# BartvLaatum/GreenLight-Gym2

Hardware: AMD Instinct MI355X
Metric: TomatoEnv env-steps/sec (higher is better)
Workload: dtype f32

## Files before the change

### greenlight-gym2_amd/csrc/glgym.hip

```cpp
#include <hip/hip_runtime.h>

#include <cmath>
#include <cstdio>
#include <cstdlib>
#include <cstring>
#include <new>
#include <string>
#include <vector>

#include "glgym.h"
#include "gl_model.hpp"
#include "gl_model_quad.hpp"
#include "gl_reward.hpp"
#include "glgym_bdf.h"
#include "glgym_rng.h"
#include "glgym_plan.h"

using namespace glm;

namespace {

thread_local std::string g_err;

#define HIPCHK(expr)                                                                                   \
    do {                                                                                               \
        hipError_t e_ = (expr);                                                                        \
        if (e_ != hipSuccess) {                                                                        \
            g_err = std::string(#expr) + ": " + hipGetErrorString(e_);                                 \
            return GLGYM_EHIP;                                                                         \
        }                                                                                              \
    } while (0)

constexpr int WAVE = 64;

#include "gl_default_const.inc"
static_assert(sizeof(ModelConst<float>) == sizeof(kDefaultConstF32_image), "regenerate gl_default_const.inc");
static_assert(sizeof(ModelConst<double>) == sizeof(kDefaultConstF64_image), "regenerate gl_default_const.inc");
template <class T> struct DefaultConst;
template <> struct DefaultConst<float> {
    static constexpr ModelConst<float> value = __builtin_bit_cast(ModelConst<float>, kDefaultConstF32_bits);
};
template <> struct DefaultConst<double> {
    static constexpr ModelConst<double> value = __builtin_bit_cast(ModelConst<double>, kDefaultConstF64_bits);
};
__constant__ const ModelConst<float> g_default_f32 = __builtin_bit_cast(ModelConst<float>, kDefaultConstF32_bits);
__constant__ const ModelConst<double> g_default_f64 = __builtin_bit_cast(ModelConst<double>, kDefaultConstF64_bits);
template <class T> __device__ __forceinline__ const ModelConst<T>& device_default();
template <> __device__ __forceinline__ const ModelConst<float>& device_default<float>() { return g_default_f32; }
template <> __device__ __forceinline__ const ModelConst<double>& device_default<double>() { return g_default_f64; }

template <class T> struct RewardConst : RewardConstBase<T> {};

template <class T> struct StepArgsT {
    int B, ld;
    T* x; T* u;
    const float* action; const T* control;
    const T* weather; int weather_rows;
    const int* w_off; int* timestep;
    const T* crop_p;
    int N;
    T* reward; T* info; unsigned char* done; float* metrics; int* step_flags;
    T dt; int n_sub;
    T gasR, tCanMin;
    int nd;
    float du, u_min[NU], u_max[NU];
    int verify;
    int pipe;
    int window;
};

template <class T> __device__ __forceinline__ T wave_sum(T v)
{
#pragma unroll
    for (int o = 32; o > 0; o >>= 1) v += __shfl_xor(v, o, WAVE);
    return v;
}

constexpr int OBS_NCORE = 23;
__device__ __forceinline__ float obs_core_feature(int j, float prim, float aux, float sday, int ts, double doy_inc, double hod_inc)
{
#pragma clang fp contract(off)
    const float kPpm = (float)(8.3144598 / (101325.0 * 44.01e-3));
    const int k = ts > 0 ? ts - 1 : 0;
    const float sat = 610.78f * __builtin_amdgcn_exp2f(1.44269504f * 17.2694f * aux * __builtin_amdgcn_rcpf(aux + 238.3f));
    const float rh = fminf(fmaxf(100.0f * prim * __builtin_amdgcn_rcpf(sat), 0.0f), 100.0f);
    const float ppm = kPpm * (aux + 273.15f) * prim;
    const int c = j - 18;
    const double rev = (c <= 2) ? __builtin_fma((double)ts, doy_inc, (double)sday) * (1.0 / 365.0)
                                : (double)ts * hod_inc * (1.0 / 24.0);
    const float fr = (float)(rev - floor(rev));
    const float clk = (c == 1 || c == 3) ? __builtin_amdgcn_sinf(fr) : __builtin_amdgcn_cosf(fr);
    float v = prim;
    v = (j == 0 || j == 16) ? ppm : v;
    v = (j == 2 || j == 15) ? rh : v;
    v = (j == 18) ? (float)k : v;
    v = (j > 18) ? clk : v;
    return v;
}
__device__ __forceinline__ constexpr int obs_core_module(int j) { return j < 4 ? 0 : j < 7 ? 1 : j < 13 ? 2 : j < 18 ? 3 : 4; }
__device__ __forceinline__ constexpr int obs_core_col(int j) { return j < 4 ? j : j < 7 ? j - 4 : j < 13 ? j - 7 : j < 18 ? j - 13 : j - 18; }

#ifndef GL_OBS_ROWS
#define GL_OBS_ROWS 16
#endif
constexpr int OBS_ROWS = GL_OBS_ROWS, OBS_MAX_NP = 128;
struct StepObsArgs {
    float* obs; const float* start_day;
    double doy_inc, hod_inc;
    int Np, dim, moff[6];
};
constexpr int STEP_OBS_MAX_DIM_OCC2 = WAVE * ((2 * NX + GL_N_SLOW) | 1) / OBS_ROWS, STEP_OBS_MAX_DIM_OCC1 = 512;
struct StepNoObs {};
constexpr int GL_SCH_OBS = 8;
template <bool OBS> struct StepObsSel { using type = StepNoObs; };
template <> struct StepObsSel<true> { using type = StepObsArgs; };

#ifndef GL_STEP_WAVES_PER_SIMD
#define GL_STEP_WAVES_PER_SIMD 1
#endif
#ifndef GL_RK4_WIN_F32
#define GL_RK4_WIN_F32 4
#endif
#ifndef GL_RK4_WIN_F64
#define GL_RK4_WIN_F64 4
#endif
template <class T> struct RK4_WINDOW { static constexpr int value = sizeof(T) == 4 ? GL_RK4_WIN_F32 : GL_RK4_WIN_F64; };
constexpr int gl_order(int sch) { return sch == 0 ? 4 : sch == 1 ? 2 : sch == 2 ? 3 : 5; }
template <class T, int SCH> struct SchemeWin { static constexpr int value = SCH == 0 ? RK4_WINDOW<T>::value : SCH == 1 ? 4 : SCH == 2 ? 3 : 2; };

template <class T, bool PER_ENV_CROP, bool DEFAULT_P, bool PIPE = false, int SCHX = 0, int OCC = GL_STEP_WAVES_PER_SIMD>
__global__ __launch_bounds__(WAVE, OCC) void step_kernel(StepArgsT<T> a, ModelConst<T> m_arg, RewardConst<T> rw,
                                                         typename StepObsSel<(SCHX & GL_SCH_OBS) != 0>::type o)
{
    constexpr bool OBS = (SCHX & GL_SCH_OBS) != 0;
    constexpr int SCH = SCHX & (GL_SCH_OBS - 1);
    static_assert(!OBS || (sizeof(T) == 4 && !PIPE), "observation epilogue: fp32, default ODE");
    const ModelConst<T>& m = DEFAULT_P ? device_default<T>() : m_arg;
    constexpr bool WBUF = OCC == 2;
    constexpr int WSTRIDE = (2 * NX + GL_N_SLOW) | 1;
    alignas(16) __shared__ float sh_w[WBUF ? WAVE * WSTRIDE : WAVE * NU];
    float* sh_act = sh_w;
    const int lane = threadIdx.x;
    const int b0 = blockIdx.x * WAVE;
    const int b = b0 + lane;
    const bool live = b < a.B;
    const int bb = live ? b : a.B - 1;

    T u[NU];
    if (a.action) {
        const int n_tile = min(WAVE, a.B - b0) * NU;
        for (int i = lane; i < n_tile; i += WAVE) sh_act[i] = a.action[(size_t)b0 * NU + i];
        __syncthreads();
        const int l = live ? lane : (a.B - 1 - b0);
#pragma unroll
        for (int j = 0; j < NU; ++j) {
            const float inc = sh_act[l * NU + j] * a.du;
            const T v = a.u[(size_t)j * a.ld + bb] + T(inc);
            u[j] = Math<T>::min(Math<T>::max(v, T(a.u_min[j])), T(a.u_max[j]));
        }
    } else {
#pragma unroll
        for (int j = 0; j < NU; ++j) u[j] = a.control[(size_t)j * a.ld + bb];
    }

    T x0[NX];
#pragma unroll
    for (int i = 0; i < NX; ++i) x0[i] = a.x[(size_t)i * a.ld + bb];
    const int ts = a.timestep[bb];
    int row = a.w_off[bb] + ts;
    row = row < 0 ? 0 : (row >= a.weather_rows ? a.weather_rows - 1 : row);
    T d[7];
#pragma unroll
    for (int j = 0; j < 7; ++j) d[j] = a.weather[(size_t)row * a.nd + j];

    CropConst<T> crLocal;
    if (PER_ENV_CROP) {
        T pc[NCROP];
#pragma unroll
        for (int i = 0; i < NCROP; ++i) pc[i] = a.crop_p[(size_t)i * a.ld + bb];
        make_crop_const<T, T>(pc, a.gasR, a.tCanMin, crLocal);
    }
    const CropConst<T>& cr = PER_ENV_CROP ? crLocal : m.crop;
    StepCoef<T> s_reg;
    precompute(u, d, m, cr, s_reg);
    if (PIPE) {
        const T tPipe = a.weather[(size_t)row * a.nd + 10], swOff = a.weather[(size_t)row * a.nd + 12];
        s_reg.pipeTrack = ((tPipe < T(1)) || (swOff > T(0))) ? T(0) : T(1);
        s_reg.tPipeSet = tPipe;
    }
    const StepCoef<T>& s = s_reg;
    if (live) {
#pragma unroll
        for (int j = 0; j < NU; ++j) a.u[(size_t)j * a.ld + b] = u[j];
    }
    T del_reg[WBUF ? 1 : NX];
    T* wb = reinterpret_cast<T*>(sh_w) + (size_t)lane * WSTRIDE;
    T* del = WBUF ? wb + NX + GL_N_SLOW : del_reg;
    if (WBUF) {
        __syncthreads();
#pragma unroll
        for (int i = 0; i < NX; ++i) wb[i] = x0[i];
        wb[5] = x0[3] - x0[5]; wb[7] = x0[2] - x0[7]; wb[20] = x0[2] - x0[20]; wb[6] = x0[5] - x0[6];
    }
    bool bad;
    int extra_steps, first_flags = 0;
    const int retries = rk4_delta_guarded<T, PIPE, gl_order(SCH), SchemeWin<T, SCH>::value, WBUF>(x0, s, m, cr, a.dt, a.n_sub, del, &bad, &extra_steps, a.verify != 0, &first_flags, a.window, wb);
    const T uBoil = a.u[(size_t)0 * a.ld + bb], uCo2 = a.u[(size_t)1 * a.ld + bb], uLamp = a.u[(size_t)4 * a.ld + bb];
    if (WBUF) {
#pragma unroll
        for (int i = 0; i < NX; ++i) x0[i] = a.x[(size_t)i * a.ld + bb];
    }

    T x1[NX];
#pragma unroll
    for (int i = 0; i < NX; ++i) x1[i] = bad ? x0[i] : x0[i] + del[i];
    {
        const double per_step = (double)a.dt / 86400.0;
        double t_start = (double)x0[NX - 1] - (double)ts * per_step;
        if (fabs(t_start) < 5e-4) t_start = 0.0;
        if (!bad) x1[NX - 1] = T(t_start + ((double)ts + 1.0) * per_step);
    }

    const T co2ppm = rw.kPpm * (x1[2] + T(273.15)) * x1[0];
    const T rh = Math<T>::min(Math<T>::max(T(100) * x1[15] / sat_vp_exact(x1[2]), T(0)), T(100));
    const T o3[3] = {co2ppm, x1[2], rh};
    T viol[3], pen = T(0);
#pragma unroll
    for (int i = 0; i < 3; ++i) {
        viol[i] = Math<T>::max(rw.lo[i] - o3[i], T(0)) + Math<T>::max(o3[i] - rw.hi[i], T(0));
        pen += viol[i] * rw.invMaxViol[i];
    }
    const T heat = uBoil * rw.heatK, elec = uLamp * rw.elecK, co2c = uCo2 * rw.co2K;
    const T varc = heat + co2c + elec;
    const T gains = (bad ? T(0) : del[25]) * rw.gainK;
    const T profit = gains - varc;
    const T reward = (profit - rw.minProfit) * rw.invRange - pen;
    const bool term = bad || (ts >= a.N);

    if (live) {
#pragma unroll
        for (int i = 0; i < NX; ++i) a.x[(size_t)i * a.ld + b] = x1[i];
        a.timestep[b] = ts + 1;
        a.reward[b] = reward;
        a.done[b] = term ? 1 : 0;
        if (a.step_flags) a.step_flags[b] = first_flags | (retries << 8) | (bad ? GLGYM_SF_FAILED : 0) | (min(extra_steps, 32767) << 16);
        if (a.info) {
            const T inf[GLGYM_NINFO] = {profit, gains, varc, rw.fixedCosts, co2c, heat, elec, viol[1], viol[0], viol[2], T(0)};
#pragma unroll
            for (int i = 0; i < GLGYM_NINFO; ++i) a.info[(size_t)i * a.ld + b] = inf[i];
        }
    }
    if (a.metrics) {
        const float w = live ? 1.f : 0.f;
        float mv[GLGYM_NMETRIC] = {w * (float)reward, w * (float)profit, (live && term) ? 1.f : 0.f,
                                   (live && bad) ? 1.f : 0.f, w * (float)viol[0], w * (float)viol[1],
                                   w * (float)viol[2], w, w * (float)retries, w * (float)extra_steps,
                                   (live && (first_flags & SC_FLAG_ERR)) ? 1.f : 0.f, (live && (first_flags & SC_FLAG_BRANCH)) ? 1.f : 0.f,
                                   (live && (first_flags & (SC_FLAG_CAP | SC_FLAG_NONFINITE))) ? 1.f : 0.f,
                                   (live && (first_flags & 16)) ? 1.f : 0.f};
        float* mrep = a.metrics + (size_t)(blockIdx.x % GLGYM_METRIC_REPLICAS) * GLGYM_METRIC_STRIDE;
#pragma unroll
        for (int i = 0; i < GLGYM_NMETRIC; ++i) {
            const float sum = wave_sum(mv[i]);
            if (lane == 0) atomicAdd(mrep + i, sum);
        }
    }
    if constexpr (OBS) {
        typedef float v4f __attribute__((ext_vector_type(4)));
        float* span;
        if constexpr (WBUF) {
            span = sh_w;
        } else {
            __shared__ float4 sh_obs4[OBS_ROWS * STEP_OBS_MAX_DIM_OCC1 / 4];
            span = reinterpret_cast<float*>(sh_obs4);
        }
        const int dim = o.dim;
        const int ts1 = ts + 1;
        const int base = a.w_off[bb] + (ts1 > 0 ? ts1 - 1 : 0);
        const int basec = base >= a.weather_rows ? a.weather_rows - 1 : (base < 0 ? 0 : base);
        const T* wrow = a.weather + (size_t)basec * a.nd;
        float wv[5];
#pragma unroll
        for (int j = 0; j < 5; ++j) wv[j] = wrow[j];
        const float sday = o.start_day[bb];
        const float uo[NU] = {uBoil, uCo2, a.u[(size_t)2 * a.ld + bb], a.u[(size_t)3 * a.ld + bb], uLamp, a.u[(size_t)5 * a.ld + bb]};
        float f[OBS_NCORE];
#pragma unroll
        for (int j = 0; j < OBS_NCORE; ++j) {
            const int xi = j == 0 ? 0 : j == 1 ? 2 : j == 2 ? 15 : j == 3 ? 9 : j == 4 ? 21 : j == 5 ? 25 : 26;
            const float prim = j < 7 ? x1[xi] : (j < 13 ? uo[(j >= 7 && j < 13) ? j - 7 : 0] : wv[j < 18 ? j - 13 : 0]);
            const float aux = j < 13 ? x1[2] : wv[1];
            f[j] = obs_core_feature(j, prim, aux, sday, ts1, o.doy_inc, o.hod_inc);
        }
        const int n_live = min(WAVE, a.B - b0);
        const int nf = o.moff[5] >= 0 ? 5 * o.Np : 0;
        __syncthreads();
        for (int s0 = 0; s0 < n_live; s0 += OBS_ROWS) {
            const int nrows = min(OBS_ROWS, n_live - s0);
            const int r_me = lane - s0;
            if (r_me >= 0 && r_me < nrows) {
#pragma unroll
                for (int j = 0; j < OBS_NCORE; ++j) {
                    const int mo = o.moff[obs_core_module(j)];
                    if (mo >= 0) span[r_me * dim + mo + obs_core_col(j)] = f[j];
                }
            }
            int base_r[OBS_ROWS];
#pragma unroll
            for (int r = 0; r < OBS_ROWS; ++r) base_r[r] = __builtin_amdgcn_readlane(base, s0 + r);
            for (int q = lane; q < nf; q += WAVE) {
                const int i = q / 5, c = q - i * 5;
                float v[OBS_ROWS];
#pragma unroll
                for (int r = 0; r < OBS_ROWS; ++r) {
                    int row = base_r[r] + 1 + i;
                    row = row >= a.weather_rows ? a.weather_rows - 1 : (row < 0 ? 0 : row);
                    v[r] = (float)a.weather[(size_t)row * a.nd + c];
                }
#pragma unroll
                for (int r = 0; r < OBS_ROWS; ++r)
                    if (r < nrows) span[r * dim + o.moff[5] + q] = v[r];
            }
            __syncthreads();
            float* out = o.obs + (size_t)(b0 + s0) * dim;
            if (nrows == OBS_ROWS) {
                const int n4 = (OBS_ROWS * dim) >> 2;
                const v4f* src4 = reinterpret_cast<const v4f*>(span);
                v4f* dst4 = reinterpret_cast<v4f*>(out);
                for (int e = lane; e < n4; e += WAVE) __builtin_nontemporal_store(src4[e], &dst4[e]);
            } else {
                for (int r = 0; r < nrows; ++r)
                    for (int jj = lane; jj < dim; jj += WAVE) out[(size_t)r * dim + jj] = span[(size_t)r * dim + jj];
            }
            __syncthreads();
        }
    }
}


template <class T, bool DEFAULT_P, int SCH = 0, bool PIPE = false, bool CROP = false, bool PAIR = false>
__global__ __launch_bounds__(WAVE) void step_kernel_quad(StepArgsT<T> a, ModelConst<T> m_arg, RewardConst<T> rw)
{
    static_assert(!(PAIR && CROP), "the two-rungs ladder is instantiated for shared crop constants only");
    constexpr bool LDSM = sizeof(T) == 8 && !DEFAULT_P;
    __shared__ ModelConst<T> sh_m[1];
    if (LDSM) {
        static_assert(sizeof(ModelConst<T>) % 4 == 0, "word copy");
        const unsigned* src = reinterpret_cast<const unsigned*>(&m_arg);
        unsigned* dst = reinterpret_cast<unsigned*>(&sh_m[0]);
        for (int i = threadIdx.x; i < (int)(sizeof(ModelConst<T>) / 4); i += WAVE) dst[i] = src[i];
        __syncthreads();
    }
    const ModelConst<T>& m = LDSM ? sh_m[0] : DEFAULT_P ? device_default<T>() : m_arg;
    const int gl = blockIdx.x * WAVE + threadIdx.x, role = gl & 3;
    const int b = PAIR ? gl >> 3 : gl >> 2, half = PAIR ? (gl >> 2) & 1 : 0;
    const bool live = b < a.B;
    const int bb = live ? b : a.B - 1;
    T u[NU];
    if (a.action) {
#pragma unroll
        for (int j = 0; j < NU; ++j) {
            const float inc = a.action[(size_t)bb * NU + j] * a.du;
            const T v = a.u[(size_t)j * a.ld + bb] + T(inc);
            u[j] = Math<T>::min(Math<T>::max(v, T(a.u_min[j])), T(a.u_max[j]));
        }
    } else {
#pragma unroll
        for (int j = 0; j < NU; ++j) u[j] = a.control[(size_t)j * a.ld + bb];
    }
    const int ts = a.timestep[bb];
    int row = a.w_off[bb] + ts;
    row = row < 0 ? 0 : (row >= a.weather_rows ? a.weather_rows - 1 : row);
    T d[7];
#pragma unroll
    for (int j = 0; j < 7; ++j) d[j] = a.weather[(size_t)row * a.nd + j];
    constexpr bool LDSQ = sizeof(T) == 8;
    struct SRec { StepCoef<T> s; T pad[(sizeof(StepCoef<T>) / sizeof(T)) % 2 == 0 ? 1 : 2]; };
    struct KRec { LaneK<T> k; T pad[(sizeof(LaneK<T>) / sizeof(T)) % 2 == 0 ? 1 : 2]; };
    struct CRec { CropConst<T> c; T pad[(sizeof(CropConst<T>) / sizeof(T)) % 2 == 0 ? 1 : 2]; };
    __shared__ SRec sh_s[LDSQ ? WAVE / 4 : 1];
    __shared__ KRec sh_k[LDSQ ? WAVE : 1];
    __shared__ CRec sh_c[(LDSQ && CROP) ? WAVE / 4 : 1];
    StepCoef<T> s_reg;
    LaneK<T> k_reg;
    CropConst<T> cr_reg;
    if (CROP && (!LDSQ || role == 0)) {
        T pc[NCROP];
#pragma unroll
        for (int i = 0; i < NCROP; ++i) pc[i] = a.crop_p[(size_t)i * a.ld + bb];
        make_crop_const<T, T>(pc, a.gasR, a.tCanMin, cr_reg);
    }
    if (!LDSQ || role == 0) {
        precompute(u, d, m, CROP ? cr_reg : m.crop, s_reg);
        if (PIPE && a.pipe) {
            const T tPipe = a.weather[(size_t)row * a.nd + 10], swOff = a.weather[(size_t)row * a.nd + 12];
            s_reg.pipeTrack = ((tPipe < T(1)) || (swOff > T(0))) ? T(0) : T(1);
            s_reg.tPipeSet = tPipe;
            s_reg.pipeOde = T(1);
        }
    }
    if (LDSQ) {
        if (role == 0) { sh_s[threadIdx.x >> 2].s = s_reg; if (CROP) sh_c[threadIdx.x >> 2].c = cr_reg; }
        __syncthreads();
    }
    const CropConst<T>& cr = !CROP ? m.crop : LDSQ ? sh_c[threadIdx.x >> 2].c : cr_reg;
    const StepCoef<T>& s = LDSQ ? sh_s[threadIdx.x >> 2].s : s_reg;
    LaneK<T>& K = LDSQ ? sh_k[threadIdx.x].k : k_reg;
    auto X = [&](int i) { return a.x[(size_t)i * a.ld + bb]; };
    QVec<T> x0, z0, del;
#pragma unroll
    for (int i = 0; i < 6; ++i) x0.sh[i] = X(role == 0 ? gq_sh_ix(i) : role == 1 ? gq_sh_ix(i) : role == 2 ? gq_sh_ix(i) : gq_sh_ix(i));
    x0.p = gq_mk<T>(X(role == 0 ? 4 : role == 1 ? 8 : role == 2 ? 7 : 5), X(role == 0 ? 9 : role == 1 ? 17 : role == 2 ? 20 : 6));
#pragma unroll
    for (int j = 0; j < 4; ++j) {
        const int ix = role == 0 ? gq_other_ix(0, j) : role == 1 ? gq_other_ix(1, j) : role == 2 ? gq_other_ix(2, j) : gq_other_ix(3, j < 2 ? j : 1);
        x0.o[j] = X(ix);
    }
    z0 = x0;
    z0.p = gq_mk<T>(role == 2 ? x0.sh[2] - x0.p.x : role == 3 ? x0.sh[3] - x0.p.x : x0.p.x,
                    role == 2 ? x0.sh[2] - x0.p.y : role == 3 ? x0.p.x - x0.p.y : x0.p.y);
    if (live && role == 0 && half == 0) {
#pragma unroll
        for (int j = 0; j < NU; ++j) a.u[(size_t)j * a.ld + b] = u[j];
    }
    bool bad;
    int extra_steps = 0, first_flags = 0, retries = 0, mine = 1;
    constexpr bool HVU = sizeof(T) == 8 || DEFAULT_P;
    if (PAIR) {
        int bad_i;
        rk4_delta_guarded_quad_pair<T, gl_order(SCH), SchemeWin<T, SCH>::value, LDSQ, PIPE, false, true, HVU>(role, half, z0, s, K, m, cr, a.dt, a.n_sub, del, &bad_i, &mine,
                                                                                                         a.window, &retries, &extra_steps, &first_flags);
        asm volatile("" : "+v"(bad_i), "+v"(mine));
        bad = bad_i != 0;
    } else {
        retries = rk4_delta_guarded_quad<T, gl_order(SCH), SchemeWin<T, SCH>::value, LDSQ, PIPE, LDSQ && CROP, HVU>(role, z0, s, K, m, cr, a.dt, a.n_sub, del, &bad,
                                                                                                    &extra_steps, a.verify != 0, &first_flags, a.window);
    }
    P2<T> dP;
    gq_phys_pair<T>(role, del, dP);
    asm volatile("" ::: "memory");
    int gl2 = blockIdx.x * WAVE + threadIdx.x;
    asm volatile("" : "+v"(gl2));
    const int role2 = gl2 & 3, b2 = PAIR ? gl2 >> 3 : gl2 >> 2;
    const bool live2 = b2 < a.B && mine != 0;
    const int bb2 = (b2 < a.B) ? b2 : a.B - 1;
    const int ts2 = a.timestep[bb2];
    auto X2 = [&](int i) { return a.x[(size_t)i * a.ld + bb2]; };
#pragma unroll
    for (int i = 0; i < 6; ++i) x0.sh[i] = X2(gq_sh_ix(i));
    x0.p = gq_mk<T>(X2(role2 == 0 ? 4 : role2 == 1 ? 8 : role2 == 2 ? 7 : 5), X2(role2 == 0 ? 9 : role2 == 1 ? 17 : role2 == 2 ? 20 : 6));
#pragma unroll
    for (int j = 0; j < 4; ++j) {
        const int ix = role2 == 0 ? gq_other_ix(0, j) : role2 == 1 ? gq_other_ix(1, j) : role2 == 2 ? gq_other_ix(2, j) : gq_other_ix(3, j < 2 ? j : 1);
        x0.o[j] = X2(ix);
    }
#pragma unroll
    for (int j = 0; j < NU; ++j) u[j] = a.u[(size_t)j * a.ld + bb2];
    QVec<T> x1;
    x1.p = gq_mk<T>(bad ? x0.p.x : x0.p.x + dP.x, bad ? x0.p.y : x0.p.y + dP.y);
#pragma unroll
    for (int i = 0; i < 6; ++i) x1.sh[i] = bad ? x0.sh[i] : x0.sh[i] + del.sh[i];
#pragma unroll
    for (int j = 0; j < 4; ++j) x1.o[j] = bad ? x0.o[j] : x0.o[j] + del.o[j];
    if (role2 == 3) {
        const double per_step = (double)a.dt / 86400.0;
        double t_start = (double)x0.o[1] - (double)ts2 * per_step;
        if (fabs(t_start) < 5e-4) t_start = 0.0;
        if (!bad) x1.o[1] = T(t_start + ((double)ts2 + 1.0) * per_step);
    }
    const T dFruit = gq_bcast<2>(del.o[3]);
    const T co2ppm = rw.kPpm * (x1.sh[2] + T(273.15)) * x1.sh[0];
    const T rh = Math<T>::min(Math<T>::max(T(100) * x1.sh[4] / sat_vp_exact(x1.sh[2]), T(0)), T(100));
    const T o3[3] = {co2ppm, x1.sh[2], rh};
    T viol[3], pen = T(0);
#pragma unroll
    for (int i = 0; i < 3; ++i) {
        viol[i] = Math<T>::max(rw.lo[i] - o3[i], T(0)) + Math<T>::max(o3[i] - rw.hi[i], T(0));
        pen += viol[i] * rw.invMaxViol[i];
    }
    const T heat = u[0] * rw.heatK, elec = u[4] * rw.elecK, co2c = u[1] * rw.co2K;
    const T varc = heat + co2c + elec;
    const T gains = (bad ? T(0) : dFruit) * rw.gainK;
    const T profit = gains - varc;
    const T reward = (profit - rw.minProfit) * rw.invRange - pen;
    const bool term = bad || (ts2 >= a.N);
    if (live2) {
        auto W = [&](int i, T v) { a.x[(size_t)i * a.ld + b2] = v; };
        W(role2 == 0 ? 4 : role2 == 1 ? 8 : role2 == 2 ? 7 : 5, x1.p.x);
        W(role2 == 0 ? 9 : role2 == 1 ? 17 : role2 == 2 ? 20 : 6, x1.p.y);
#pragma unroll
        for (int j = 0; j < 4; ++j)
            if (role2 != 3 || j < 2) W(role2 == 0 ? gq_other_ix(0, j) : role2 == 1 ? gq_other_ix(1, j) : role2 == 2 ? gq_other_ix(2, j) : gq_other_ix(3, j < 2 ? j : 1), x1.o[j]);
        if (role2 == 0) {
#pragma unroll
            for (int i = 0; i < 6; ++i) W(gq_sh_ix(i), x1.sh[i]);
            a.timestep[b2] = ts2 + 1;
            a.reward[b2] = reward;
            a.done[b2] = term ? 1 : 0;
            if (a.step_flags) a.step_flags[b2] = first_flags | (retries << 8) | (bad ? GLGYM_SF_FAILED : 0) | (min(extra_steps, 32767) << 16);
            if (a.info) {
                const T inf[GLGYM_NINFO] = {profit, gains, varc, rw.fixedCosts, co2c, heat, elec, viol[1], viol[0], viol[2], T(0)};
#pragma unroll
                for (int i = 0; i < GLGYM_NINFO; ++i) a.info[(size_t)i * a.ld + b2] = inf[i];
            }
        }
    }
    if (a.metrics) {
        const bool cnt = live2 && role2 == 0;
        const float w = cnt ? 1.f : 0.f;
        float mv[GLGYM_NMETRIC] = {w * (float)reward, w * (float)profit, (cnt && term) ? 1.f : 0.f,
                                   (cnt && bad) ? 1.f : 0.f, w * (float)viol[0], w * (float)viol[1],
                                   w * (float)viol[2], w, w * (float)retries, w * (float)extra_steps,
                                   (cnt && (first_flags & SC_FLAG_ERR)) ? 1.f : 0.f, (cnt && (first_flags & SC_FLAG_BRANCH)) ? 1.f : 0.f,
                                   (cnt && (first_flags & (SC_FLAG_CAP | SC_FLAG_NONFINITE))) ? 1.f : 0.f,
                                   (cnt && (first_flags & 16)) ? 1.f : 0.f};
        float* mrep = a.metrics + (size_t)(blockIdx.x % GLGYM_METRIC_REPLICAS) * GLGYM_METRIC_STRIDE;
#pragma unroll
        for (int i = 0; i < GLGYM_NMETRIC; ++i) {
            const float sum = wave_sum(mv[i]);
            if (threadIdx.x == 0) atomicAdd(mrep + i, sum);
        }
    }
}

template <class T, int SCH, bool PIPE, bool CROP, bool PAIR = false>
__global__ __launch_bounds__(WAVE) void evalf_kernel_quad(const double* x, const double* u, const double* d, const double* crop, int B, T dt,
                                                          int n_sub, T gasR, T tCanMin, ModelConst<T> m_arg, double* x_next, int nd,
                                                          int* n_failed, int verify, int pipe, int window)
{
    constexpr bool LDSM = sizeof(T) == 8;
    __shared__ ModelConst<T> sh_m[1];
    if (LDSM) {
        const unsigned* src = reinterpret_cast<const unsigned*>(&m_arg);
        unsigned* dst = reinterpret_cast<unsigned*>(&sh_m[0]);
        for (int i = threadIdx.x; i < (int)(sizeof(ModelConst<T>) / 4); i += WAVE) dst[i] = src[i];
        __syncthreads();
    }
    const ModelConst<T>& m = LDSM ? sh_m[0] : m_arg;
    const int gl = blockIdx.x * WAVE + threadIdx.x, role = gl & 3, b = PAIR ? gl >> 3 : gl >> 2, half = PAIR ? (gl >> 2) & 1 : 0;
    const bool live = b < B;
    const int bb = live ? b : B - 1;
    T uu[NU], dd[7];
#pragma unroll
    for (int i = 0; i < NU; ++i) uu[i] = T(u[(size_t)bb * NU + i]);
#pragma unroll
    for (int i = 0; i < 7; ++i) dd[i] = T(d[(size_t)bb * nd + i]);
    constexpr bool LDSQ = sizeof(T) == 8;
    struct SRec { StepCoef<T> s; T pad[(sizeof(StepCoef<T>) / sizeof(T)) % 2 == 0 ? 1 : 2]; };
    struct KRec { LaneK<T> k; T pad[(sizeof(LaneK<T>) / sizeof(T)) % 2 == 0 ? 1 : 2]; };
    struct CRec { CropConst<T> c; T pad[(sizeof(CropConst<T>) / sizeof(T)) % 2 == 0 ? 1 : 2]; };
    __shared__ SRec sh_s[LDSQ ? WAVE / 4 : 1];
    __shared__ KRec sh_k[LDSQ ? WAVE : 1];
    __shared__ CRec sh_c[(LDSQ && CROP) ? WAVE / 4 : 1];
    StepCoef<T> s_reg;
    LaneK<T> k_reg;
    CropConst<T> cr_reg;
    if (CROP && (!LDSQ || role == 0)) {
        T pc[NCROP];
#pragma unroll
        for (int i = 0; i < NCROP; ++i) pc[i] = T(crop[(size_t)bb * NCROP + i]);
        make_crop_const<T, T>(pc, gasR, tCanMin, cr_reg);
    }
    if (!LDSQ || role == 0) {
        precompute(uu, dd, m, CROP ? cr_reg : m.crop, s_reg);
        if (PIPE && pipe) {
            const T tPipe = T(d[(size_t)bb * nd + 10]), swOff = T(d[(size_t)bb * nd + 12]);
            s_reg.pipeTrack = ((tPipe < T(1)) || (swOff > T(0))) ? T(0) : T(1);
            s_reg.tPipeSet = tPipe;
            s_reg.pipeOde = T(1);
        }
    }
    if (LDSQ) {
        if (role == 0) { sh_s[threadIdx.x >> 2].s = s_reg; if (CROP) sh_c[threadIdx.x >> 2].c = cr_reg; }
        __syncthreads();
    }
    const CropConst<T>& cr = !CROP ? m.crop : LDSQ ? sh_c[threadIdx.x >> 2].c : cr_reg;
    const StepCoef<T>& s = LDSQ ? sh_s[threadIdx.x >> 2].s : s_reg;
    LaneK<T>& K = LDSQ ? sh_k[threadIdx.x].k : k_reg;
    auto X = [&](int i) { return T(x[(size_t)bb * NX + i]); };
    QVec<T> x0, z0, del;
#pragma unroll
    for (int i = 0; i < 6; ++i) x0.sh[i] = X(gq_sh_ix(i));
    x0.p = gq_mk<T>(X(role == 0 ? 4 : role == 1 ? 8 : role == 2 ? 7 : 5), X(role == 0 ? 9 : role == 1 ? 17 : role == 2 ? 20 : 6));
#pragma unroll
    for (int j = 0; j < 4; ++j)
        x0.o[j] = X(role == 0 ? gq_other_ix(0, j) : role == 1 ? gq_other_ix(1, j) : role == 2 ? gq_other_ix(2, j) : gq_other_ix(3, j < 2 ? j : 1));
    z0 = x0;
    z0.p = gq_mk<T>(role == 2 ? x0.sh[2] - x0.p.x : role == 3 ? x0.sh[3] - x0.p.x : x0.p.x,
                    role == 2 ? x0.sh[2] - x0.p.y : role == 3 ? x0.p.x - x0.p.y : x0.p.y);
    bool bad;
    constexpr bool HVU = sizeof(T) == 8;
    int mine = 1;
    if (PAIR) {
        int bad_i;
        rk4_delta_guarded_quad_pair<T, gl_order(SCH), SchemeWin<T, SCH>::value, LDSQ, PIPE, LDSQ && CROP, false, HVU>(role, half, z0, s, K, m, cr, dt, n_sub, del, &bad_i, &mine, window);
        asm volatile("" : "+v"(bad_i), "+v"(mine));
        bad = bad_i != 0;
    } else {
        int extra_steps, first_flags = 0;
        rk4_delta_guarded_quad<T, gl_order(SCH), SchemeWin<T, SCH>::value, LDSQ, PIPE, LDSQ && CROP, HVU>(role, z0, s, K, m, cr, dt, n_sub, del, &bad, &extra_steps, verify != 0,
                                                                                      &first_flags, window);
    }
    P2<T> dP;
    gq_phys_pair<T>(role, del, dP);
    asm volatile("" ::: "memory");
    int gl2 = blockIdx.x * WAVE + threadIdx.x;
    asm volatile("" : "+v"(gl2));
    const int role2 = gl2 & 3, b2 = PAIR ? gl2 >> 3 : gl2 >> 2;
    if (b2 < B && mine != 0) {
        const double nan = __builtin_nan("");
        auto X2 = [&](int i) { return x[(size_t)b2 * NX + i]; };
        auto W = [&](int i, T dv) { x_next[(size_t)b2 * NX + i] = bad ? nan : X2(i) + (double)dv; };
        W(role2 == 0 ? 4 : role2 == 1 ? 8 : role2 == 2 ? 7 : 5, dP.x);
        W(role2 == 0 ? 9 : role2 == 1 ? 17 : role2 == 2 ? 20 : 6, dP.y);
#pragma unroll
        for (int j = 0; j < 4; ++j)
            if (role2 != 3 || j < 2)
                W(role2 == 0 ? gq_other_ix(0, j) : role2 == 1 ? gq_other_ix(1, j) : role2 == 2 ? gq_other_ix(2, j) : gq_other_ix(3, j < 2 ? j : 1), del.o[j]);
        if (role2 == 0) {
#pragma unroll
            for (int i = 0; i < 6; ++i) W(gq_sh_ix(i), del.sh[i]);
            if (bad) atomicAdd(n_failed, 1);
        }
    }
}

template <class T, bool PER_ENV_CROP, bool PIPE>
__global__ __launch_bounds__(WAVE) void rhs_kernel(const double* x, const double* u, const double* d, const double* crop, int B, T gasR,
                                                   T tCanMin, ModelConst<T> m, double* dx, int nd)
{
    const int b = blockIdx.x * WAVE + threadIdx.x;
    if (b >= B) return;
    T x0[NX], uu[NU], dd[7];
    for (int i = 0; i < NX; ++i) x0[i] = T(x[(size_t)b * NX + i]);
    for (int i = 0; i < NU; ++i) uu[i] = T(u[(size_t)b * NU + i]);
    for (int i = 0; i < 7; ++i) dd[i] = T(d[(size_t)b * nd + i]);
    CropConst<T> crLocal;
    if (PER_ENV_CROP) {
        T pc[NCROP];
        for (int i = 0; i < NCROP; ++i) pc[i] = T(crop[(size_t)b * NCROP + i]);
        make_crop_const<T, T>(pc, gasR, tCanMin, crLocal);
    }
    const CropConst<T>& cr = PER_ENV_CROP ? crLocal : m.crop;
    StepCoef<T> s;
    precompute(uu, dd, m, cr, s);
    if (PIPE) {
        const T tPipe = T(d[(size_t)b * nd + 10]), swOff = T(d[(size_t)b * nd + 12]);
        s.pipeTrack = ((tPipe < T(1)) || (swOff > T(0))) ? T(0) : T(1);
        s.tPipeSet = tPipe;
    }
    T k[NX];
    rhs<T, true, PIPE>(x0, s, m, cr, k);
    for (int i = 0; i < NX; ++i) dx[(size_t)b * NX + i] = (double)k[i];
}

template <class T, bool PER_ENV_CROP, bool PIPE = false, int SCH = 0>
__global__ __launch_bounds__(WAVE) void evalf_kernel(const double* x, const double* u, const double* d,
                                                     const double* crop, int B, T dt, int n_sub, T gasR, T tCanMin,
                                                     ModelConst<T> m, double* x_next, int rhs_only, int nd,
                                                     int* n_failed, int verify, int window)
{
    const int b = blockIdx.x * WAVE + threadIdx.x;
    if (b >= B) return;
    T x0[NX], uu[NU], dd[7];
    for (int i = 0; i < NX; ++i) x0[i] = T(x[(size_t)b * NX + i]);
    for (int i = 0; i < NU; ++i) uu[i] = T(u[(size_t)b * NU + i]);
    for (int i = 0; i < 7; ++i) dd[i] = T(d[(size_t)b * nd + i]);
    CropConst<T> crLocal;
    if (PER_ENV_CROP) {
        T pc[NCROP];
        for (int i = 0; i < NCROP; ++i) pc[i] = T(crop[(size_t)b * NCROP + i]);
        make_crop_const<T, T>(pc, gasR, tCanMin, crLocal);
    }
    const CropConst<T>& cr = PER_ENV_CROP ? crLocal : m.crop;
    StepCoef<T> s;
    precompute(uu, dd, m, cr, s);
    if (PIPE) {
        const T tPipe = T(d[(size_t)b * nd + 10]), swOff = T(d[(size_t)b * nd + 12]);
        s.pipeTrack = ((tPipe < T(1)) || (swOff > T(0))) ? T(0) : T(1);
        s.tPipeSet = tPipe;
    }
    if (rhs_only) {
        T k[NX];
        rhs<T, true, PIPE>(x0, s, m, cr, k);
        for (int i = 0; i < NX; ++i) x_next[(size_t)b * NX + i] = (double)k[i];
        return;
    }
    T del[NX];
    bool failed;
    rk4_delta_guarded<T, PIPE, gl_order(SCH), SchemeWin<T, SCH>::value>(x0, s, m, cr, dt, n_sub, del, &failed, nullptr, verify != 0, nullptr, window);
    for (int i = 0; i < NX; ++i)
        x_next[(size_t)b * NX + i] = failed ? __builtin_nan("") : (double)x0[i] + (double)del[i];
    if (failed) atomicAdd(n_failed, 1);
}

template <class T> struct ObsArgsT {
    int B, ld;
    const T* x; const T* u; const T* weather; int weather_rows;
    const int* w_off; const int* timestep; const float* start_day;
    int Np; float* obs; double doy_inc, hod_inc;
    const unsigned char* mask; float* term_obs;
    int nd;
    int moff[6], dim;
};

template <class T> __global__ __launch_bounds__(256) void obs_kernel(ObsArgsT<T> a)
{
    constexpr int ROWS = OBS_ROWS, NCORE = OBS_NCORE;
    extern __shared__ float4 span4[];
    float* span = reinterpret_cast<float*>(span4);
    const int tid = threadIdx.x;
    const int dim = a.dim;
    for (int rb = blockIdx.x * ROWS; rb < a.B; rb += gridDim.x * ROWS) {
        const int nrows = min(ROWS, a.B - rb);
        if (a.mask) {
            int any = 0;
            for (int r = 0; r < nrows; ++r) any |= a.mask[rb + r];
            if (!any) continue;
        }
        int base_r[ROWS];
#pragma unroll
        for (int r = 0; r < ROWS; ++r) {
            const int b = rb + (r < nrows ? r : 0);
            const int ts = a.timestep[b];
            base_r[r] = a.w_off[b] + (ts > 0 ? ts - 1 : 0);
        }
        for (int e = tid; e < ROWS * NCORE; e += 256) {
            const int r = e / NCORE, j = e - r * NCORE;
            const int b = rb + (r < nrows ? r : 0);
            const int ts = a.timestep[b];
            int base = 0;
#pragma unroll
            for (int rr = 0; rr < ROWS; ++rr) base = (rr == r) ? base_r[rr] : base;
            base = base >= a.weather_rows ? a.weather_rows - 1 : (base < 0 ? 0 : base);
            const T* wrow = a.weather + (size_t)base * a.nd;
            const int xi = j == 0 ? 0 : j == 1 ? 2 : j == 2 ? 15 : j == 3 ? 9 : j == 4 ? 21 : j == 5 ? 25 : 26;
            const T* p1 = j < 7 ? a.x + (size_t)xi * a.ld + b
                                : (j < 13 ? a.u + (size_t)(j - 7) * a.ld + b : wrow + (j < 18 ? j - 13 : 0));
            const T* p2 = j < 13 ? a.x + (size_t)2 * a.ld + b : wrow + 1;
            const float prim = (float)*p1, aux = (float)*p2, sday = a.start_day[b];
            const float v = obs_core_feature(j, prim, aux, sday, ts, a.doy_inc, a.hod_inc);
            const int mo = j < 4 ? a.moff[0] : j < 7 ? a.moff[1] : j < 13 ? a.moff[2] : j < 18 ? a.moff[3] : a.moff[4];
            const int jl = j < 4 ? j : j < 7 ? j - 4 : j < 13 ? j - 7 : j < 18 ? j - 13 : j - 18;
            if (r < nrows && mo >= 0) span[r * dim + mo + jl] = v;
        }
        const int nf = a.moff[5] >= 0 ? 5 * a.Np : 0;
        for (int q = tid; q < nf; q += 256) {
            const int i = q / 5, c = q - i * 5;
            float v[ROWS];
#pragma unroll
            for (int r = 0; r < ROWS; ++r) {
                int row = base_r[r] + 1 + i;
                row = row >= a.weather_rows ? a.weather_rows - 1 : (row < 0 ? 0 : row);
                v[r] = (float)a.weather[(size_t)row * a.nd + c];
            }
#pragma unroll
            for (int r = 0; r < ROWS; ++r)
                if (r < nrows) span[r * dim + a.moff[5] + q] = v[r];
        }
        __syncthreads();
        float* out = a.obs + (size_t)rb * dim;
        if (!a.mask && nrows == ROWS) {
            const int n4 = (ROWS * dim) >> 2;
            float4* out4 = reinterpret_cast<float4*>(out);
            typedef float v4f __attribute__((ext_vector_type(4)));
            const v4f* src4 = reinterpret_cast<const v4f*>(span4);
            v4f* dst4 = reinterpret_cast<v4f*>(out4);
            for (int e = tid; e < n4; e += 256) __builtin_nontemporal_store(src4[e], &dst4[e]);
        } else {
            for (int r = 0; r < nrows; ++r) {
                if (a.mask && !a.mask[rb + r]) continue;
                for (int jj = tid; jj < dim; jj += 256) {
                    const size_t e = (size_t)r * dim + jj;
                    if (a.mask && a.term_obs) a.term_obs[(size_t)rb * dim + e] = out[e];
                    out[e] = span[e];
                }
            }
        }
        __syncthreads();
    }
}

template <class T>
__global__ __launch_bounds__(256) void rule_based_kernel(glgym_rule_cfg c, int B, int ld, const T* __restrict__ x,
                                                         const T* __restrict__ weather, int weather_rows,
                                                         const int* __restrict__ w_off, const int* __restrict__ timestep,
                                                         const float* __restrict__ start_day, const double* hour,
                                                         const double* doy_in, double doy_inc, double hod_inc,
                                                         T* __restrict__ control, int nd)
{
    const int b = blockIdx.x * blockDim.x + threadIdx.x;
    if (b >= B) return;
    const int ts = timestep[b];
    int row = w_off[b] + ts;
    row = row >= weather_rows ? weather_rows - 1 : (row < 0 ? 0 : row);
    const T* w = weather + (size_t)row * nd;
    const double iGlob = (double)w[0], tOut = (double)w[1], dli = (double)w[7], isDay = (double)w[8],
                 isDaySmooth = (double)w[9];
    const double co2Air = (double)x[b], tAir = (double)x[(size_t)2 * ld + b], vpAir = (double)x[(size_t)15 * ld + b];
    const double hod = hour ? hour[b] : fmod((double)ts * hod_inc, 24.0);
    const double doy = doy_in ? doy_in[b] : (double)start_day[b] + (double)ts * doy_inc;
    auto pband = [](double v, double sp, double band, double lo, double hi) {
        return lo + (hi - lo) * (1.0 / (1.0 + exp(-2.0 / band * 4.605170185988092 * (v - sp - band * 0.5))));
    };
    const double tod = c.lamps_on <= c.lamps_off ? (double)(c.lamps_on < hod && hod < c.lamps_off)
                                                 : (double)(c.lamps_on < hod || hod < c.lamps_off);
    const double doy_ok = c.lamps_day_start <= c.lamps_day_stop
                              ? (double)(c.lamps_day_start < doy && doy < c.lamps_day_stop)
                              : (double)(c.lamps_day_start < doy || doy < c.lamps_day_stop);
    const double below_dli = (double)(dli < c.lamp_rad_sum_limit);
    const double lamp_no_cons = (double)(iGlob < c.lamps_off_sun) * below_dli * tod * doy_ok;
    const double sw_on = fmax(0.0, fmin(1.0, hod - c.lamps_on + 1.0));
    const double sw_off = fmax(0.0, fmin(1.0, c.lamps_off - hod + 1.0));
    const double both = c.lamps_on == c.lamps_off ? 0.0
                        : (c.lamps_on < c.lamps_off ? fmin(sw_on, sw_off) : fmax(sw_on, sw_off));
    const double smooth_lamp = both * below_dli * doy_ok;
    const double day_inside = fmax(smooth_lamp, isDay);
    const double heat_sp = day_inside * c.temp_setpoint_day + (1.0 - day_inside) * c.temp_setpoint_night +
                           c.heat_correction * lamp_no_cons;
    const double heat_max = heat_sp + c.heat_deadzone;
    const double co2_sp = day_inside * c.co2_day;
    const double co2_ppm = 1e6 * 8.3144598 * (tAir + 273.15) * (1e-6 * co2Air) / (101325.0 * 44.01e-3);
    const double rh_in = 100.0 * vpAir / (610.78 * exp(17.2694 * tAir / (tAir + 238.3)));
    const double vent_heat = pband(tAir, heat_max, c.vent_heat_Pband, 0, 1);
    const double vent_rh = pband(rh_in, c.rh_max + 0.0 * c.mech_dehumid_Pband, c.vent_rh_Pband, 0, 1);
    const double vent_cold = pband(tAir, heat_sp - c.t_vent_off, c.vent_cold_Pband, 1, 0);
    const double th_sp = isDay * c.thScrSpDay + (1.0 - isDay) * c.thScrSpNight;
    const double th_cold = pband(tOut, th_sp, c.thScrPband, 0, 1);
    const double th_heat = pband(tAir, heat_sp + c.thScrDeadZone, -c.thScrPband, 1, 0);
    const double th_rh = fmax(pband(rh_in, c.rhMax + c.thScrRh, c.thScrRhPband, 1, 0), 1.0 - vent_cold);
    const double lamp_on = lamp_no_cons * pband(tAir, heat_max + c.lampExtraHeat, -0.5, 0, 1) *
                           (isDaySmooth + (1.0 - isDaySmooth)) *
                           fmax(pband(rh_in, c.rhMax + c.blScrExtraRh, -0.5, 0, 1), 1.0 - vent_cold);
    control[b] = (T)pband(tAir, heat_sp, c.tHeatBand, 0, 1);
    control[(size_t)1 * ld + b] = (T)pband(co2_ppm, co2_sp, c.co2Band, 0, 1);
    control[(size_t)2 * ld + b] = (T)fmin(th_cold, fmax(th_heat, th_rh));
    control[(size_t)3 * ld + b] = (T)fmin(vent_cold, fmax(vent_heat, vent_rh));
    control[(size_t)4 * ld + b] = (T)lamp_on;
    control[(size_t)5 * ld + b] = (T)(c.useBlScr * (1.0 - isDaySmooth) * lamp_on);
}

__device__ __forceinline__ void philox4x32_10(unsigned c0, unsigned c1, unsigned c2, unsigned c3, unsigned k0,
                                              unsigned k1, unsigned* out)
{
#pragma unroll
    for (int r = 0; r < 10; ++r) {
        const unsigned long long p0 = 0xD2511F53ull * c0, p1 = 0xCD9E8D57ull * c2;
        const unsigned n0 = (unsigned)(p1 >> 32) ^ c1 ^ k0, n1 = (unsigned)p1;
        const unsigned n2 = (unsigned)(p0 >> 32) ^ c3 ^ k1, n3 = (unsigned)p0;
        c0 = n0; c1 = n1; c2 = n2; c3 = n3;
        k0 += 0x9E3779B9u; k1 += 0xBB67AE85u;
    }
    out[0] = c0; out[1] = c1; out[2] = c2; out[3] = c3;
}


template <class T>
__global__ void reset_kernel(int B, int ld, const unsigned char* mask, T* x, T* u, int* timestep, const T* weather,
                             int weather_rows, int* w_off, const int* start_rows, const float* start_days, int n_starts,
                             float* start_day, int* episode, unsigned long long seed, int nd)
{
    const int b = blockIdx.x * blockDim.x + threadIdx.x;
    if (b >= B || (mask && !mask[b])) return;
    if (start_rows && n_starts > 0) {
        const int ep = episode ? episode[b] : 0;
        unsigned rnd[4];
        philox4x32_10((unsigned)b, (unsigned)ep, 0x5eedu, 0u, (unsigned)seed, (unsigned)(seed >> 32), rnd);
        const int j = (int)(rnd[0] % (unsigned)n_starts);
        w_off[b] = start_rows[j];
        if (start_day && start_days) start_day[b] = start_days[j];
        if (episode) episode[b] = ep + 1;
    }
    int r = w_off[b];
    r = r < 0 ? 0 : (r >= weather_rows ? weather_rows - 1 : r);
    const double co2Out = (double)weather[(size_t)r * nd + 3], tSoOut = (double)weather[(size_t)r * nd + 6];
    const double tAir = 16.5;
    double xi[NX];
    xi[0] = xi[1] = co2Out;
    for (int i = 2; i <= 10; ++i) xi[i] = tAir;
    xi[4] = tAir + 4;
    xi[11] = 0.25 * (3.0 * tAir + tSoOut);
    xi[12] = 0.25 * (2.0 * tAir + 2 * tSoOut);
    xi[13] = 0.25 * (tAir + 3 * tSoOut);
    xi[14] = tSoOut;
    xi[15] = xi[16] = 90.0 / 100.0 * (610.78 * exp(17.2694 * tAir / (tAir + 238.3)));
    xi[17] = xi[18] = xi[19] = xi[20] = tAir;
    xi[21] = xi[4];
    xi[22] = 0.0; xi[23] = 9.5283e4; xi[24] = 2.5107e5; xi[25] = 5.5338e4; xi[26] = 3.0978e3; xi[27] = 0.0;
    for (int i = 0; i < NX; ++i) x[(size_t)i * ld + b] = T(xi[i]);
    for (int j = 0; j < NU; ++j) u[(size_t)j * ld + b] = T(0);
    timestep[b] = 0;
}

template <class T>
__global__ void crop_noise_kernel(T* crop_p, int B, int ld, const float* p0, float scale, unsigned long long seed,
                                  unsigned long long draw)
{
    const int b = blockIdx.x * blockDim.x + threadIdx.x;
    if (b >= B) return;
    float pn[NCROP + 2];
    for (int blk = 0; blk < 9; ++blk) {
        unsigned r[4];
        philox4x32_10((unsigned)b, (unsigned)draw, (unsigned)(draw >> 32), (unsigned)blk, (unsigned)seed,
                      (unsigned)(seed >> 32), r);
        for (int q = 0; q < 4; ++q) {
            const int i = blk * 4 + q;
            if (i < NCROP) {
                const float un = ((float)(r[q] >> 8) + 0.5f) * (1.0f / 16777216.0f);
                const float noise = (un - 0.5f) * scale;
                pn[i] = p0[i] + noise * p0[i];
            }
        }
    }
    pn[144 - CROP0] = pn[141 - CROP0] / pn[142 - CROP0];
    for (int i = 0; i < NCROP; ++i) crop_p[(size_t)i * ld + b] = T(pn[i]);
}


constexpr int VN_REP = 16;
__global__ __launch_bounds__(1024) void vecnorm_moments_kernel(const float* __restrict__ obs, int B, int dim,
                                                               double* __restrict__ acc_all)
{
    double* acc = acc_all + (size_t)(blockIdx.x % VN_REP) * 2 * dim;
    const int rows_per_block = (B + gridDim.x - 1) / gridDim.x;
    const int r0 = blockIdx.x * rows_per_block, r1 = min(B, r0 + rows_per_block);
    for (int c = threadIdx.x; c < dim; c += blockDim.x) {
        double s0 = 0.0, q0 = 0.0, s1 = 0.0, q1 = 0.0;
        int r = r0;
        for (; r + 7 < r1; r += 8) {
            float v[8];
#pragma unroll
            for (int j = 0; j < 8; ++j) v[j] = obs[(size_t)(r + j) * dim + c];
#pragma unroll
            for (int j = 0; j < 8; j += 2) {
                const double a = (double)v[j], b = (double)v[j + 1];
                s0 += a; q0 += a * a; s1 += b; q1 += b * b;
            }
        }
        for (; r < r1; ++r) { const double v = (double)obs[(size_t)r * dim + c]; s0 += v; q0 += v * v; }
        if (r1 > r0) { atomicAdd(acc + c, s0 + s1); atomicAdd(acc + dim + c, q0 + q1); }
    }
}

template <class T>
__global__ __launch_bounds__(256) void vecnorm_returns_kernel(const T* __restrict__ reward, double* __restrict__ returns,
                                                              int B, double gamma, double* __restrict__ acc2)
{
    const int b = blockIdx.x * blockDim.x + threadIdx.x;
    double v = 0.0;
    if (b < B) { v = returns[b] * gamma + (double)reward[b]; returns[b] = v; }
    double s = v, q = v * v;
#pragma unroll
    for (int o = 32; o > 0; o >>= 1) { s += __shfl_xor(s, o, WAVE); q += __shfl_xor(q, o, WAVE); }
    __shared__ double part[2][4];
    const int wv = threadIdx.x / WAVE;
    if ((threadIdx.x & (WAVE - 1)) == 0) { part[0][wv] = s; part[1][wv] = q; }
    __syncthreads();
    if (threadIdx.x == 0) {
        atomicAdd(acc2, part[0][0] + part[0][1] + part[0][2] + part[0][3]);
        atomicAdd(acc2 + 1, part[1][0] + part[1][1] + part[1][2] + part[1][3]);
    }
}

__global__ __launch_bounds__(1024) void vecnorm_merge_kernel(double* mean, double* var, double* count, const double* acc, int dim,
                                                            int B, double* ret_stats, const double* acc2, int do_obs,
                                                            int do_ret, double eps, double* scale)
{
    const double n = (double)B;
    const double cnt = *count;
    for (int c = threadIdx.x; c < dim; c += blockDim.x) {
        if (do_obs) {
            double sum = 0.0, sq = 0.0;
            for (int r = 0; r < VN_REP; ++r) { sum += acc[(size_t)r * 2 * dim + c]; sq += acc[(size_t)r * 2 * dim + dim + c]; }
            const double bm = sum / n, bv = fmax(sq / n - bm * bm, 0.0);
            const double tot = cnt + n, delta = bm - mean[c];
            const double m2 = var[c] * cnt + bv * n + delta * delta * cnt * n / tot;
            mean[c] += delta * n / tot;
            var[c] = m2 / tot;
        }
        if (scale) scale[c] = 1.0 / sqrt(var[c] + eps);
    }
    if (do_ret && threadIdx.x == 0) {
        const double bm = acc2[0] / n, bv = fmax(acc2[1] / n - bm * bm, 0.0);
        const double rc = ret_stats[2], tot = rc + n, delta = bm - ret_stats[0];
        const double m2 = ret_stats[1] * rc + bv * n + delta * delta * rc * n / tot;
        ret_stats[0] += delta * n / tot;
        ret_stats[1] = m2 / tot;
        ret_stats[2] = tot;
    }
    __syncthreads();
    if (do_obs && threadIdx.x == 0) *count = cnt + n;
}

__global__ __launch_bounds__(1024) void vecnorm_apply_kernel(const float* __restrict__ obs, float* __restrict__ out,
                                                            int B, int dim, const double* __restrict__ mean,
                                                            const double* __restrict__ scale, float clip)
{
    const int rows_per_block = (B + gridDim.x - 1) / gridDim.x;
    const int r0 = blockIdx.x * rows_per_block, r1 = min(B, r0 + rows_per_block);
    for (int c = threadIdx.x; c < dim; c += blockDim.x) {
        const double mu = mean[c], sc = scale[c];
        for (int r = r0; r < r1; ++r) {
            const size_t i = (size_t)r * dim + c;
            const float v = (float)(((double)obs[i] - mu) * sc);
            out[i] = fminf(fmaxf(v, -clip), clip);
        }
    }
}

template <class T>
__global__ void vecnorm_reward_kernel(const T* __restrict__ reward, float* __restrict__ out, double* __restrict__ returns,
                                      const unsigned char* __restrict__ done, int B, const double* ret_stats, double eps,
                                      float clip, int norm_reward)
{
    const int b = blockIdx.x * blockDim.x + threadIdx.x;
    if (b >= B) return;
    float r = (float)reward[b];
    if (norm_reward) r = fminf(fmaxf((float)((double)reward[b] / sqrt(ret_stats[1] + eps)), -clip), clip);
    out[b] = r;
    if (done && done[b]) returns[b] = 0.0;
}


__device__ __forceinline__ double w_sat_vp(double t) { return 610.78 * exp(17.2694 * t / (t + 238.3)); }

__global__ void weather_convert_kernel(int n, const double* __restrict__ time, const double* __restrict__ i_glob,
                                       const double* __restrict__ t_out, const double* __restrict__ rh,
                                       const double* __restrict__ wind, const double* __restrict__ t_sky, double co2_ppm,
                                       double* __restrict__ W)
{
    const int k = blockIdx.x * blockDim.x + threadIdx.x;
    if (k >= n) return;
    const double R = 8.3144598, C2K = 273.15, M_CO2 = 44.01e-3, M_H2O = 18.01528e-3, P_ATM = 101325.0;
    const double t = t_out[k];
    const double rho_v = (rh[k] / 100.0) * w_sat_vp(t) * M_H2O / (R * (t + C2K));
    const double rho_sat = (100.0 / 100.0) * w_sat_vp(t) * M_H2O / (R * (t + C2K));
    W[0 * (size_t)n + k] = i_glob[k];
    W[1 * (size_t)n + k] = t;
    W[2 * (size_t)n + k] = w_sat_vp(t) * (rho_v / rho_sat);
    W[3 * (size_t)n + k] = (P_ATM * 1e-6 * co2_ppm * M_CO2 / (R * (t + C2K))) * 1e6;
    W[4 * (size_t)n + k] = wind[k];
    W[5 * (size_t)n + k] = t_sky[k];
    const double year = 3600.0 * 24.0 * 365.0;
    W[6 * (size_t)n + k] = 10.0 + 5.0 * sin(2.0 * 3.14159265358979323846 * (time[k] + 0.625 * year) / year);
}

__global__ void weather_scan_kernel(int n, const double* __restrict__ time, double* __restrict__ W)
{
    if (blockIdx.x != 0 || threadIdx.x != 0 || n < 2) return;
    const double* rad = W;
    double* dli = W + 7 * (size_t)n;
    double* is_day = W + 8 * (size_t)n;
    double* smooth = W + 9 * (size_t)n;
    const double c = 86400.0, interval = time[1] - time[0];
    auto next_jump = [&](int from) {
        for (int k = from < 0 ? 0 : from; k + 1 < n; ++k)
            if (floor(time[k + 1] / c) - floor(time[k] / c) == 1.0) return k;
        return -1;
    };
    int before = 0, j = next_jump(0), after = j >= 0 ? j + 1 : n, i = 0;
    while (i < n) {
        const int seg_end = after < n ? after : n;
        double sum = 0.0;
        for (int k = before; k <= after && k < n; ++k) sum += rad[k];
        for (int k = i; k < seg_end; ++k) dli[k] = sum * interval * 1e-6;
        i = seg_end;
        if (i >= n) break;
        before = after;
        j = next_jump(before + 2);
        after = j >= 0 ? j : n;
    }
    double dt_mean = (time[n - 1] - time[0]) / (double)(n - 1);
    for (int k = 0; k < n; ++k) { is_day[k] = rad[k] > 0.0 ? 1.0 : 0.0; smooth[k] = is_day[k]; }
    const int n_tr = (int)(3600.0 / dt_mean), half = n_tr / 2;
    if (n_tr < 2) return;
    const double step = 1.0 / (double)(n_tr - 1);
    bool in_sunset = false;
    for (int k = n_tr; k < n - n_tr; ++k) {
        const double cur = is_day[k], nxt = is_day[k + 1];
        if (cur == 0.0) {
            in_sunset = false;
            if (nxt == 1.0)
                for (int q = 0; q < 2 * half && q < n_tr; ++q) {
                    const double r = (q == n_tr - 1) ? 1.0 : (double)q * step;
                    is_day[k - half + q] = r;
                    smooth[k - half + q] = 1.0 / (1.0 + exp(-10.0 * (r - 0.5)));
                }
        } else if (cur == 1.0 && nxt == 0.0 && !in_sunset) {
            for (int q = 0; q < 2 * half && q < n_tr; ++q) {
                const double r = (q == n_tr - 1) ? 1.0 : (double)q * step;
                is_day[k - half + q] = 1.0 - r;
                smooth[k - half + q] = 1.0 - 1.0 / (1.0 + exp(-10.0 * (r - 0.5)));
            }
            in_sunset = true;
        }
    }
}

__device__ __forceinline__ double w_sign(double v) { return v > 0.0 ? 1.0 : (v < 0.0 ? -1.0 : 0.0); }
__device__ __forceinline__ double pchip_edge(double h0, double h1, double m0, double m1)
{
    double d = ((2.0 * h0 + h1) * m0 - h0 * m1) / (h0 + h1);
    if (w_sign(d) != w_sign(m0)) d = 0.0;
    else if (w_sign(m0) != w_sign(m1) && fabs(d) > 3.0 * fabs(m0)) d = 3.0 * m0;
    return d;
}
__global__ void pchip_slopes_kernel(int n, int n_col, const double* __restrict__ x, const double* __restrict__ W,
                                    double* __restrict__ D)
{
    const int k = blockIdx.x * blockDim.x + threadIdx.x, col = blockIdx.y;
    if (k >= n || col >= n_col) return;
    const double* y = W + (size_t)col * n;
    auto h = [&](int i) { return x[i + 1] - x[i]; };
    auto m = [&](int i) { return (y[i + 1] - y[i]) / h(i); };
    double d;
    if (n == 2) d = m(0);
    else if (k == 0) d = pchip_edge(h(0), h(1), m(0), m(1));
    else if (k == n - 1) d = pchip_edge(h(n - 2), h(n - 3), m(n - 2), m(n - 3));
    else {
        const double m0 = m(k - 1), m1 = m(k), h0 = h(k - 1), h1 = h(k);
        if (w_sign(m0) != w_sign(m1) || m0 == 0.0 || m1 == 0.0) d = 0.0;
        else {
            const double w1 = 2.0 * h1 + h0, w2 = h1 + 2.0 * h0;
            d = 1.0 / ((w1 / m0 + w2 / m1) / (w1 + w2));
        }
    }
    D[(size_t)col * n + k] = d;
}

template <class T>
__global__ void pchip_eval_kernel(int n, int n_col, int n_out, int nd, const double* __restrict__ x,
                                  const double* __restrict__ W, const double* __restrict__ D, T* __restrict__ out)
{
    const int i = blockIdx.x * blockDim.x + threadIdx.x, col = blockIdx.y;
    if (i >= n_out || col >= n_col) return;
    const double start = x[0], stop = x[n - 1];
    const double stepo = n_out > 1 ? (stop - start) / (double)(n_out - 1) : 0.0;
    const double t = (i == n_out - 1 && n_out > 1) ? stop : (double)i * stepo + start;
    int lo = 0, hi = n - 1;
    while (hi - lo > 1) { const int mid = (lo + hi) >> 1; if (x[mid] <= t) lo = mid; else hi = mid; }
    const int k = lo > n - 2 ? n - 2 : lo;
    const double* y = W + (size_t)col * n;
    const double* d = D + (size_t)col * n;
    const double dx = x[k + 1] - x[k], slope = (y[k + 1] - y[k]) / dx;
    const double tt = (d[k] + d[k + 1] - 2.0 * slope) / dx;
    const double c0 = tt / dx, c1 = (slope - d[k]) / dx - tt, c2 = d[k], c3 = y[k];
    const double sdx = t - x[k];
    double res = 0.0, z = 1.0;
    res += c3 * z; z *= sdx;
    res += c2 * z; z *= sdx;
    res += c1 * z; z *= sdx;
    res += c0 * z;
    if (col == 0 && res < 1e-10) res = 0.0;
    out[(size_t)i * nd + col] = T(res);
}

}

struct glgym_handle_s {
    int device = 0;
    int dtype = GLGYM_F32;
    int n_sub = 256;
    double dt = 900.0;
    double p[NP];
    ModelConst<float> mf;
    ModelConst<double> md;
    glgym_reward_cfg rcfg;
    RewardConst<float> rf;
    RewardConst<double> rd;
    double max_profit = 0, min_profit = 0, fixed_costs = 0;
    float* p0_crop_dev = nullptr;
    int* fail_dev = nullptr;
    int nd = ND;
    int variant = GLGYM_ODE;
    int scheme = GLGYM_SCHEME_RK4;
    int verify_mode = GLGYM_VERIFY_AUTO;
    int use_specialised = 1;
    int window = 0;
    int layout = GLGYM_LAYOUT_AUTO;
    int occupancy = 0;
    int ladder_parallel = 1;
    int n_simd = 1024;
    float du = 0.1f, u_min[NU] = {0, 0, 0, 0, 0, 0}, u_max[NU] = {1, 1, 1, 1, 1, 1};
    int obs_modules[6] = {0, 1, 2, 3, 4, 5};
    int n_obs_modules = 6;
    hipEvent_t ev0 = nullptr, ev1 = nullptr;
    int integrator = GLGYM_INTEGRATOR_EXPLICIT;
    int step_integrator = GLGYM_INTEGRATOR_EXPLICIT;
    double rtol = 1e-6, atol = 1e-6;
    int max_steps = 10000;
    int32_t* stats_dev = nullptr;
    int stats_cap = 0;
    std::vector<int32_t> stats;
    int stats_rows = 0;
// ... 170 lines not shown
{
    if (!h || waves_per_simd < 0 || waves_per_simd > 2) { g_err = "glgym_set_occupancy: 0 (by batch size), 1 or 2 waves per SIMD"; return GLGYM_EINVAL; }
    h->occupancy = waves_per_simd;
    return GLGYM_OK;
}

int glgym_set_ladder_parallel(glgym_handle h, int on)
{
    if (!h || (on != 0 && on != 1)) { g_err = "glgym_set_ladder_parallel: 0 or 1"; return GLGYM_EINVAL; }
    h->ladder_parallel = on;
    return GLGYM_OK;
}

int glgym_set_control_limits(glgym_handle h, const double* u_min, const double* u_max, double delta_u_max)
{
    if (!h || !u_min || !u_max || !(delta_u_max >= 0)) { g_err = "glgym_set_control_limits: bad arguments"; return GLGYM_EINVAL; }
    for (int j = 0; j < NU; ++j)
        if (!(u_min[j] <= u_max[j])) { g_err = "glgym_set_control_limits: u_min > u_max"; return GLGYM_EINVAL; }
    for (int j = 0; j < NU; ++j) { h->u_min[j] = (float)u_min[j]; h->u_max[j] = (float)u_max[j]; }
    h->du = (float)delta_u_max;
    return GLGYM_OK;
}

int glgym_set_integrator(glgym_handle h, int integrator)
{
    if (!h || (integrator != GLGYM_INTEGRATOR_EXPLICIT && integrator != GLGYM_INTEGRATOR_BDF)) {
        g_err = "glgym_set_integrator: GLGYM_INTEGRATOR_EXPLICIT or GLGYM_INTEGRATOR_BDF";
        return GLGYM_EINVAL;
    }
    h->integrator = integrator;
    return GLGYM_OK;
}

int glgym_set_step_integrator(glgym_handle h, int integrator)
{
    if (!h || (integrator != GLGYM_INTEGRATOR_EXPLICIT && integrator != GLGYM_INTEGRATOR_BDF)) {
        g_err = "glgym_set_step_integrator: GLGYM_INTEGRATOR_EXPLICIT or GLGYM_INTEGRATOR_BDF";
        return GLGYM_EINVAL;
    }
    h->step_integrator = integrator;
    return GLGYM_OK;
}

int glgym_set_tolerances(glgym_handle h, double rtol, double atol, int max_steps)
{
    if (!h || !(rtol > 0.0) || !(atol > 0.0) || !std::isfinite(rtol) || !std::isfinite(atol) || max_steps < 1) {
        g_err = "glgym_set_tolerances: rtol > 0, atol > 0 (finite), max_steps >= 1";
        return GLGYM_EINVAL;
    }
    h->rtol = rtol; h->atol = atol; h->max_steps = max_steps;
    return GLGYM_OK;
}

int glgym_get_solver_stats(glgym_handle h, int B, int32_t* stats)
{
    if (!h || !stats || B < 1 || B != h->stats_rows) {
        g_err = "glgym_get_solver_stats: B must be the batch size of the last glgym_evalF with GLGYM_INTEGRATOR_BDF";
        return GLGYM_EINVAL;
    }
    std::memcpy(stats, h->stats.data(), (size_t)B * GLGYM_NSOLVER_STAT * sizeof(int32_t));
    return GLGYM_OK;
}

int glgym_set_verify(glgym_handle h, int mode)
{
    if (!h || (mode != GLGYM_VERIFY_AUTO && mode != GLGYM_VERIFY_ALWAYS && mode != GLGYM_VERIFY_NEVER)) {
        g_err = "glgym_set_verify: GLGYM_VERIFY_AUTO, GLGYM_VERIFY_ALWAYS or GLGYM_VERIFY_NEVER";
        return GLGYM_EINVAL;
    }
    h->verify_mode = mode;
    return GLGYM_OK;
}

int glgym_set_n_sub(glgym_handle h, int n_sub)
{
    if (!h || n_sub < 1) return GLGYM_EINVAL;
    h->n_sub = n_sub;
    return GLGYM_OK;
}

int glgym_set_reward(glgym_handle h, const glgym_reward_cfg* cfg)
{
    if (!h || !cfg) return GLGYM_EINVAL;
    h->rcfg = *cfg;
    return refresh(h);
}

int glgym_get_reward_scale(glgym_handle h, double* max_profit, double* min_profit, double* fixed_costs)
{
    if (!h) return GLGYM_EINVAL;
    if (max_profit) *max_profit = h->max_profit;
    if (min_profit) *min_profit = h->min_profit;
    if (fixed_costs) *fixed_costs = h->fixed_costs;
    return GLGYM_OK;
}

}

static int ensure_scratch(glgym_handle h, size_t elems)
{
    if (h->scratch_elems >= elems) return GLGYM_OK;
    if (h->scratch) (void)hipFree(h->scratch);
    h->scratch = nullptr; h->scratch_elems = 0;
    HIPCHK(hipMalloc(&h->scratch, elems * sizeof(double)));
    h->scratch_elems = elems;
    return GLGYM_OK;
}

template <class T, int SCH>
static void launch_evalf_sch(glgym_handle h, const ModelConst<T>& m, const double* p_used, const double* dx, const double* du,
                             const double* dd, const double* dcrop, int B, double* dout, dim3 grid, dim3 block)
{
    const int verify = h->verify_mode != GLGYM_VERIFY_NEVER;
    const bool pair = verify && h->ladder_parallel && !dcrop && (size_t)8 * B <= (size_t)WAVE * h->n_simd &&
                      (sizeof(T) == 8 || h->layout != GLGYM_LAYOUT_ONE);
    if constexpr (sizeof(T) == 8) {
        const dim3 qgrid((4 * B + WAVE - 1) / WAVE), pgrid((8 * B + WAVE - 1) / WAVE);
        const int pipe = h->variant == GLGYM_ODE_PIPE ? 1 : 0;
        if (pair) hipLaunchKernelGGL((evalf_kernel_quad<T, SCH, true, false, true>), pgrid, block, 0, (hipStream_t)0, dx, du, dd, dcrop, B, T(h->dt), h->n_sub,
                                     T(p_used[39]), T(p_used[162]), m, dout, h->nd, h->fail_dev, verify, pipe, h->window);
        else if (dcrop) hipLaunchKernelGGL((evalf_kernel_quad<T, SCH, true, true>), qgrid, block, 0, (hipStream_t)0, dx, du, dd, dcrop, B, T(h->dt), h->n_sub,
                                      T(p_used[39]), T(p_used[162]), m, dout, h->nd, h->fail_dev, verify, pipe, h->window);
        else hipLaunchKernelGGL((evalf_kernel_quad<T, SCH, true, false>), qgrid, block, 0, (hipStream_t)0, dx, du, dd, dcrop, B, T(h->dt), h->n_sub,
                                T(p_used[39]), T(p_used[162]), m, dout, h->nd, h->fail_dev, verify, pipe, h->window);
    } else {
        const dim3 pgrid((8 * B + WAVE - 1) / WAVE);
        if (pair) hipLaunchKernelGGL((evalf_kernel_quad<T, SCH, false, false, true>), pgrid, block, 0, (hipStream_t)0, dx, du, dd, dcrop, B, T(h->dt), h->n_sub,
                                     T(p_used[39]), T(p_used[162]), m, dout, h->nd, h->fail_dev, verify, 0, h->window);
        else if (!dcrop && (h->layout == GLGYM_LAYOUT_QUAD || (h->layout == GLGYM_LAYOUT_AUTO && B <= 4 * h->n_simd * 4)))
            hipLaunchKernelGGL((evalf_kernel_quad<T, SCH, false, false, false>), dim3((4 * B + WAVE - 1) / WAVE), block, 0, (hipStream_t)0, dx, du, dd, dcrop, B,
                               T(h->dt), h->n_sub, T(p_used[39]), T(p_used[162]), m, dout, h->nd, h->fail_dev, verify, 0, h->window);
        else if (dcrop) hipLaunchKernelGGL((evalf_kernel<T, true, false, SCH>), grid, block, 0, (hipStream_t)0, dx, du, dd, dcrop, B, T(h->dt), h->n_sub,
                                      T(p_used[39]), T(p_used[162]), m, dout, 0, h->nd, h->fail_dev, verify, h->window);
        else hipLaunchKernelGGL((evalf_kernel<T, false, false, SCH>), grid, block, 0, (hipStream_t)0, dx, du, dd, dcrop, B, T(h->dt), h->n_sub,
                                T(p_used[39]), T(p_used[162]), m, dout, 0, h->nd, h->fail_dev, verify, h->window);
    }
}

template <class T>
static int run_evalf(glgym_handle h, const ModelConst<T>& m, const double* p_used, const double* dx, const double* du,
                     const double* dd, const double* dcrop, int B, double* dout, int rhs_only)
{
    const dim3 grid((B + WAVE - 1) / WAVE), block(WAVE);
    const bool pipe = h->variant == GLGYM_ODE_PIPE;
    if (rhs_only) {
        if (pipe) hipLaunchKernelGGL((rhs_kernel<T, false, true>), grid, block, 0, (hipStream_t)0, dx, du, dd, dcrop, B, T(p_used[39]), T(p_used[162]), m, dout, h->nd);
        else if (dcrop) hipLaunchKernelGGL((rhs_kernel<T, true, false>), grid, block, 0, (hipStream_t)0, dx, du, dd, dcrop, B, T(p_used[39]), T(p_used[162]), m, dout, h->nd);
        else hipLaunchKernelGGL((rhs_kernel<T, false, false>), grid, block, 0, (hipStream_t)0, dx, du, dd, dcrop, B, T(p_used[39]), T(p_used[162]), m, dout, h->nd);
        HIPCHK(hipGetLastError());
        return GLGYM_OK;
    }
    if (pipe) {
        if (dcrop || h->scheme != GLGYM_SCHEME_RK4) {
            g_err = "glgym_evalF: GLGYM_ODE_PIPE supports neither per-row parameter blocks nor schemes other than GLGYM_SCHEME_RK4";
            return GLGYM_EINVAL;
        }
        if constexpr (sizeof(T) == 8) {
            launch_evalf_sch<T, GLGYM_SCHEME_RK4>(h, m, p_used, dx, du, dd, dcrop, B, dout, grid, block);
        } else {
            const int verify = h->verify_mode != GLGYM_VERIFY_NEVER;
            hipLaunchKernelGGL((evalf_kernel<T, false, true>), grid, block, 0, (hipStream_t)0, dx, du, dd, dcrop, B, T(h->dt), h->n_sub,
                               T(p_used[39]), T(p_used[162]), m, dout, 0, h->nd, h->fail_dev, verify, h->window);
        }
    } else if (h->scheme == GLGYM_SCHEME_RK2) {
        launch_evalf_sch<T, GLGYM_SCHEME_RK2>(h, m, p_used, dx, du, dd, dcrop, B, dout, grid, block);
    } else if (h->scheme == GLGYM_SCHEME_RK3) {
        launch_evalf_sch<T, GLGYM_SCHEME_RK3>(h, m, p_used, dx, du, dd, dcrop, B, dout, grid, block);
    } else if (h->scheme == GLGYM_SCHEME_LS5) {
        launch_evalf_sch<T, GLGYM_SCHEME_LS5>(h, m, p_used, dx, du, dd, dcrop, B, dout, grid, block);
    } else {
        launch_evalf_sch<T, GLGYM_SCHEME_RK4>(h, m, p_used, dx, du, dd, dcrop, B, dout, grid, block);
    }
    HIPCHK(hipGetLastError());
    return GLGYM_OK;
}

static int evalf_impl(glgym_handle h, const double* x, const double* u, const double* d, const double* p, int p_rows,
                      int B, double* out, int rhs_only)
{
    if (!h || !x || !u || !d || !out || B < 1 || (p && p_rows != 1 && p_rows != B)) {
        g_err = "glgym_evalF: bad arguments";
        return GLGYM_EINVAL;
    }
    HIPCHK(hipSetDevice(h->device));
    const bool bdf = !rhs_only && h->integrator == GLGYM_INTEGRATOR_BDF;
    if (bdf && h->variant == GLGYM_ODE_PIPE) {
        g_err = "glgym_evalF: GLGYM_INTEGRATOR_BDF does not support GLGYM_ODE_PIPE";
        return GLGYM_EINVAL;
    }
    const double* p_used = p ? p : h->p;
    bool per_row = p && p_rows == B && B > 1;
    if (per_row) {
        for (int b = 1; b < B && per_row; ++b)
            for (int i = 0; i < NP; ++i)
                if ((i < CROP0 || i >= CROP0 + NCROP) && p[(size_t)b * NP + i] != p[i]) {
                    std::vector<int32_t> st(bdf ? (size_t)B * GLGYM_NSOLVER_STAT : 0);
                    for (int r = 0; r < B; ++r) {
                        const int rc = evalf_impl(h, x + (size_t)r * NX, u + (size_t)r * NU, d + (size_t)r * h->nd,
                                                  p + (size_t)r * NP, 1, 1, out + (size_t)r * NX, rhs_only);
                        if (bdf && h->stats_rows == 1)
                            std::memcpy(&st[(size_t)r * GLGYM_NSOLVER_STAT], h->stats.data(), sizeof(int32_t) * GLGYM_NSOLVER_STAT);
                        if (rc != GLGYM_OK) return rc;
                    }
                    if (bdf) { h->stats = st; h->stats_rows = B; }
                    return GLGYM_OK;
                }
    }
    const size_t n_in = (size_t)B * (NX + NU + h->nd + (per_row ? NCROP : 0));
    int rc = ensure_scratch(h, n_in + (size_t)B * NX);
    if (rc != GLGYM_OK) return rc;
    double* dx = h->scratch; double* du = dx + (size_t)B * NX; double* dd = du + (size_t)B * NU;
    double* dcrop = per_row ? dd + (size_t)B * h->nd : nullptr;
    double* dout = h->scratch + n_in;
    HIPCHK(hipMemcpy(dx, x, (size_t)B * NX * sizeof(double), hipMemcpyHostToDevice));
    HIPCHK(hipMemcpy(du, u, (size_t)B * NU * sizeof(double), hipMemcpyHostToDevice));
    HIPCHK(hipMemcpy(dd, d, (size_t)B * h->nd * sizeof(double), hipMemcpyHostToDevice));
    if (per_row) {
        std::vector<double> crop((size_t)B * NCROP);
        for (int b = 0; b < B; ++b)
            for (int i = 0; i < NCROP; ++i) crop[(size_t)b * NCROP + i] = p[(size_t)b * NP + CROP0 + i];
        HIPCHK(hipMemcpy(dcrop, crop.data(), crop.size() * sizeof(double), hipMemcpyHostToDevice));
    }
    HIPCHK(hipMemset(h->fail_dev, 0, sizeof(int)));
    HIPCHK(hipMemset(dout, 0xFF, (size_t)B * NX * sizeof(double)));
    if (bdf) {
        if (h->stats_cap < B) {
            if (h->stats_dev) (void)hipFree(h->stats_dev);
            h->stats_dev = nullptr; h->stats_cap = 0;
            HIPCHK(hipMalloc(&h->stats_dev, (size_t)B * GLGYM_NSOLVER_STAT * sizeof(int32_t)));
            h->stats_cap = B;
        }
        h->stats_rows = 0;
        ModelConst<double> m = h->md;
        if (p) make_model_const<double>(p_used, m);
        HIPCHK(bdf_launch(dx, du, dd, dcrop, B, h->nd, h->dt, h->rtol, h->atol, h->max_steps, m, p_used[39], p_used[162], dout,
                          h->stats_dev, h->fail_dev));
        h->stats.resize((size_t)B * GLGYM_NSOLVER_STAT);
        HIPCHK(hipMemcpy(h->stats.data(), h->stats_dev, h->stats.size() * sizeof(int32_t), hipMemcpyDeviceToHost));
        h->stats_rows = B;
    } else if (h->dtype == GLGYM_F32) {
        ModelConst<float> m = h->mf;
        if (p) make_model_const<float>(p_used, m);
        rc = run_evalf<float>(h, m, p_used, dx, du, dd, dcrop, B, dout, rhs_only);
    } else {
        ModelConst<double> m = h->md;
        if (p) make_model_const<double>(p_used, m);
        rc = run_evalf<double>(h, m, p_used, dx, du, dd, dcrop, B, dout, rhs_only);
    }
    if (rc != GLGYM_OK) return rc;
    HIPCHK(hipMemcpy(out, dout, (size_t)B * NX * sizeof(double), hipMemcpyDeviceToHost));
    int n_failed = 0;
    HIPCHK(hipMemcpy(&n_failed, h->fail_dev, sizeof(int), hipMemcpyDeviceToHost));
    if (n_failed > 0) {
        g_err = "glgym_evalF: the integration failed for " + std::to_string(n_failed) + " of " + std::to_string(B) +
                (bdf ? " rows (BDF: step limit, right-hand-side limit, step-size underflow or a non-finite value)"
                     : " rows (no two consecutive attempts of the n_sub, 2x, 4x, 8x ladder agreed)") + "; their rows of x_next are NaN";
        return GLGYM_EODE;
    }
    if (!rhs_only) {
        for (int b = 0; b < B; ++b)
            for (int i = 0; i < NX; ++i)
                if (std::isnan(out[(size_t)b * NX + i])) {
                    g_err = "glgym_evalF: row " + std::to_string(b) + " of " + std::to_string(B) + " came back unwritten (state " + std::to_string(i) +
                            " is NaN although no integration was reported as failed): internal error of the kernel's row-writing lane selection";
                    return GLGYM_EHIP;
                }
    }
    return GLGYM_OK;
}

extern "C" {

int glgym_evalF(glgym_handle h, const double* x, const double* u, const double* d, const double* p, int p_rows, int B,
                double* x_next)
{
    return evalf_impl(h, x, u, d, p, p_rows, B, x_next, 0);
}

int glgym_rhs(glgym_handle h, const double* x, const double* u, const double* d, int B, double* dx)
{
    return evalf_impl(h, x, u, d, nullptr, 1, B, dx, 1);
}

}

static const int OBS_MODULE_SIZE[6] = {4, 3, 6, 5, 5, 0};
static void obs_layout(glgym_handle h, int Np, int moff[6], int* dim)
{
    for (int m = 0; m < 6; ++m) moff[m] = -1;
    *dim = 0;
    for (int i = 0; i < h->n_obs_modules; ++i) {
        const int m = h->obs_modules[i];
        moff[m] = *dim;
        *dim += m == GLGYM_OBS_FORECAST ? 5 * Np : OBS_MODULE_SIZE[m];
    }
}
static void obs_clock_increments(glgym_handle h, double* doy_inc, double* hod_inc)
{
    *doy_inc = std::fmod(h->dt / 86400.0, 365.0);
    *hod_inc = h->dt / 3600.0;
}
template <int SCH>
static void launch_step_sch(const glgym_step_args* a, const StepArgsT<float>& k, const ModelConst<float>& m, const RewardConst<float>& rw,
                            dim3 grid, dim3 block, hipStream_t st, bool def, bool occ2, const StepObsArgs* o)
{
    using T = float;
    const StepNoObs no;
    constexpr int SCHO = SCH | GL_SCH_OBS;
    if (o) {
        if (occ2) hipLaunchKernelGGL((step_kernel<T, false, true, false, SCHO, 2>), grid, block, 0, st, k, m, rw, *o);
        else if (a->crop_p && def) hipLaunchKernelGGL((step_kernel<T, true, true, false, SCHO>), grid, block, 0, st, k, m, rw, *o);
        else if (a->crop_p) hipLaunchKernelGGL((step_kernel<T, true, false, false, SCHO>), grid, block, 0, st, k, m, rw, *o);
        else if (def) hipLaunchKernelGGL((step_kernel<T, false, true, false, SCHO>), grid, block, 0, st, k, m, rw, *o);
        else hipLaunchKernelGGL((step_kernel<T, false, false, false, SCHO>), grid, block, 0, st, k, m, rw, *o);
        return;
    }
    if (occ2) {
        hipLaunchKernelGGL((step_kernel<T, false, true, false, SCH, 2>), grid, block, 0, st, k, m, rw, no);
        return;
    }
    if (a->crop_p) {
        if (def) hipLaunchKernelGGL((step_kernel<T, true, true, false, SCH>), grid, block, 0, st, k, m, rw, no);
        else hipLaunchKernelGGL((step_kernel<T, true, false, false, SCH>), grid, block, 0, st, k, m, rw, no);
    } else {
        if (def) hipLaunchKernelGGL((step_kernel<T, false, true, false, SCH>), grid, block, 0, st, k, m, rw, no);
        else hipLaunchKernelGGL((step_kernel<T, false, false, false, SCH>), grid, block, 0, st, k, m, rw, no);
    }
}

template <class T, int SCH>
static void launch_quad_sch(const glgym_step_args* a, const StepArgsT<T>& k, const ModelConst<T>& m, const RewardConst<T>& rw,
                            dim3 qgrid, dim3 block, hipStream_t st, bool def, bool pair)
{
    const dim3 pgrid((8 * (size_t)a->B + WAVE - 1) / WAVE);
    if constexpr (sizeof(T) == 8) {
        if (pair) hipLaunchKernelGGL((step_kernel_quad<T, false, SCH, true, false, true>), pgrid, block, 0, st, k, m, rw);
        else if (a->crop_p) hipLaunchKernelGGL((step_kernel_quad<T, false, SCH, true, true>), qgrid, block, 0, st, k, m, rw);
        else hipLaunchKernelGGL((step_kernel_quad<T, false, SCH, true, false>), qgrid, block, 0, st, k, m, rw);
    } else {
        if (pair && def) hipLaunchKernelGGL((step_kernel_quad<T, true, SCH, false, false, true>), pgrid, block, 0, st, k, m, rw);
        else if (pair) hipLaunchKernelGGL((step_kernel_quad<T, false, SCH, false, false, true>), pgrid, block, 0, st, k, m, rw);
        else if (def) hipLaunchKernelGGL((step_kernel_quad<T, true, SCH, false, false>), qgrid, block, 0, st, k, m, rw);
        else hipLaunchKernelGGL((step_kernel_quad<T, false, SCH, false, false>), qgrid, block, 0, st, k, m, rw);
    }
}

template <class T>
static int launch_step(glgym_handle h, const glgym_step_args* a, const ModelConst<T>& m, const RewardConst<T>& rw,
                       hipStream_t st, const glgym_obs_args* oa = nullptr, bool* fused = nullptr)
{
    StepArgsT<T> k;
    k.B = a->B; k.ld = a->ld;
    k.x = (T*)a->x; k.u = (T*)a->u; k.action = a->action; k.control = (const T*)a->control;
    k.weather = (const T*)a->weather; k.weather_rows = a->weather_rows;
    k.w_off = a->w_off; k.timestep = a->timestep; k.crop_p = (const T*)a->crop_p; k.N = a->N;
    k.reward = (T*)a->reward; k.info = (T*)a->info; k.done = a->done; k.metrics = a->metrics; k.step_flags = a->step_flags;
    k.dt = T(h->dt); k.n_sub = h->n_sub; k.gasR = T(h->p[39]); k.tCanMin = T(h->p[162]); k.nd = h->nd;
    k.du = h->du;
    for (int j = 0; j < NU; ++j) { k.u_min[j] = h->u_min[j]; k.u_max[j] = h->u_max[j]; }
    k.pipe = h->variant == GLGYM_ODE_PIPE ? 1 : 0;
    k.window = h->window;
    k.verify = h->verify_mode == GLGYM_VERIFY_ALWAYS || (h->verify_mode == GLGYM_VERIFY_AUTO && (!a->action || h->du > 0.1001f));
    const dim3 grid((a->B + WAVE - 1) / WAVE), block(WAVE), qgrid((4 * a->B + WAVE - 1) / WAVE);
    const bool pipe = h->variant == GLGYM_ODE_PIPE;
    if (pipe && (a->crop_p || h->scheme != GLGYM_SCHEME_RK4)) {
        g_err = "glgym_step: GLGYM_ODE_PIPE supports neither per-env crop parameters nor schemes other than GLGYM_SCHEME_RK4";
        return GLGYM_EINVAL;
    }
    const bool def = h->use_specialised && std::memcmp(&m, &DefaultConst<T>::value, sizeof m) == 0;
    const bool pair = k.verify && h->ladder_parallel && !a->crop_p && (size_t)8 * a->B <= (size_t)WAVE * h->n_simd;
    if constexpr (sizeof(T) == 8) {
        if (h->scheme == GLGYM_SCHEME_RK2) launch_quad_sch<T, GLGYM_SCHEME_RK2>(a, k, m, rw, qgrid, block, st, def, pair);
        else if (h->scheme == GLGYM_SCHEME_RK3) launch_quad_sch<T, GLGYM_SCHEME_RK3>(a, k, m, rw, qgrid, block, st, def, pair);
        else if (h->scheme == GLGYM_SCHEME_LS5) launch_quad_sch<T, GLGYM_SCHEME_LS5>(a, k, m, rw, qgrid, block, st, def, pair);
        else launch_quad_sch<T, GLGYM_SCHEME_RK4>(a, k, m, rw, qgrid, block, st, def, pair);
        HIPCHK(hipGetLastError());
        return GLGYM_OK;
    } else {
        const int layout_env = h->layout;
        const bool quad_ok = !pipe && !a->crop_p;
        const int b_small = 4 * h->n_simd * 4;
        if (quad_ok && (layout_env == 2 || (layout_env == 0 && a->B <= b_small))) {
            if (h->scheme == GLGYM_SCHEME_RK2) launch_quad_sch<T, GLGYM_SCHEME_RK2>(a, k, m, rw, qgrid, block, st, def, pair);
            else if (h->scheme == GLGYM_SCHEME_RK3) launch_quad_sch<T, GLGYM_SCHEME_RK3>(a, k, m, rw, qgrid, block, st, def, pair);
            else if (h->scheme == GLGYM_SCHEME_LS5) launch_quad_sch<T, GLGYM_SCHEME_LS5>(a, k, m, rw, qgrid, block, st, def, pair);
            else launch_quad_sch<T, GLGYM_SCHEME_RK4>(a, k, m, rw, qgrid, block, st, def, pair);
            HIPCHK(hipGetLastError());
            return GLGYM_OK;
        }
        if (pipe) {
            hipLaunchKernelGGL((step_kernel<T, false, false, true>), grid, block, 0, st, k, m, rw, StepNoObs{});
            HIPCHK(hipGetLastError());
            return GLGYM_OK;
        }
        const bool occ2 = def && !a->crop_p && (h->occupancy == 2 || (h->occupancy == 0 && (size_t)a->B >= (size_t)2 * WAVE * h->n_simd));
        StepObsArgs ob;
        const StepObsArgs* o = nullptr;
        if (oa && !oa->mask && oa->B == a->B && oa->ld == a->ld && oa->x == a->x && oa->u == a->u && oa->weather == a->weather &&
            oa->weather_rows == a->weather_rows && oa->w_off == a->w_off && oa->timestep == a->timestep &&
            ((uintptr_t)oa->obs & 15) == 0) {
            ob.obs = oa->obs; ob.start_day = oa->start_day; ob.Np = oa->Np;
            obs_clock_increments(h, &ob.doy_inc, &ob.hod_inc);
            obs_layout(h, oa->Np, ob.moff, &ob.dim);
            if (ob.dim > 0 && ob.dim <= (occ2 ? STEP_OBS_MAX_DIM_OCC2 : STEP_OBS_MAX_DIM_OCC1)) o = &ob;
        }
        if (h->scheme == GLGYM_SCHEME_RK2) launch_step_sch<GLGYM_SCHEME_RK2>(a, k, m, rw, grid, block, st, def, occ2, o);
        else if (h->scheme == GLGYM_SCHEME_RK3) launch_step_sch<GLGYM_SCHEME_RK3>(a, k, m, rw, grid, block, st, def, occ2, o);
        else if (h->scheme == GLGYM_SCHEME_LS5) launch_step_sch<GLGYM_SCHEME_LS5>(a, k, m, rw, grid, block, st, def, occ2, o);
        else launch_step_sch<GLGYM_SCHEME_RK4>(a, k, m, rw, grid, block, st, def, occ2, o);
        HIPCHK(hipGetLastError());
        if (o && fused) *fused = true;
        return GLGYM_OK;
    }
}

template <class T>
static int launch_step_bdf(glgym_handle h, const glgym_step_args* a, const RewardConst<T>& rw, hipStream_t st)
{
    if (h->variant == GLGYM_ODE_PIPE) {
        g_err = "glgym_step: GLGYM_INTEGRATOR_BDF does not support GLGYM_ODE_PIPE";
        return GLGYM_EINVAL;
    }
    glbdf::BdfEnvArgs<T> k;
    k.ld = a->ld;
    k.x = (T*)a->x; k.u = (T*)a->u; k.action = a->action; k.control = (const T*)a->control;
    k.weather = (const T*)a->weather; k.weather_rows = a->weather_rows; k.nd = h->nd;
    k.w_off = a->w_off; k.timestep = a->timestep; k.crop_p = (const T*)a->crop_p; k.N = a->N;
    k.reward = (T*)a->reward; k.info = (T*)a->info; k.done = a->done; k.step_flags = a->step_flags;
    k.dt = h->dt; k.rtol = h->rtol; k.atol = h->atol; k.max_steps = h->max_steps;
    k.gasR = h->p[39]; k.tCanMin = h->p[162];
    k.du = h->du;
    for (int j = 0; j < NU; ++j) { k.u_min[j] = h->u_min[j]; k.u_max[j] = h->u_max[j]; }
    HIPCHK(bdf_env_launch<T>(k, a->B, h->md, rw, a->metrics, st));
    return GLGYM_OK;
}

static int step_impl(glgym_handle h, const glgym_step_args* a, void* stream, const glgym_obs_args* oa, bool* fused)
{
    if (!h || !a) { g_err = "glgym_step: null handle / arguments"; return GLGYM_EINVAL; }
    if (a->struct_size != (int32_t)sizeof(glgym_step_args)) {
        g_err = "glgym_step: glgym_step_args.struct_size is " + std::to_string(a->struct_size) + ", this library expects " +
                std::to_string(sizeof(glgym_step_args)) + " (ABI " + std::to_string(GLGYM_ABI_VERSION) + "): rebuild against include/glgym.h";
        return GLGYM_EINVAL;
    }
    if (a->B < 1 || a->ld < a->B || !a->x || !a->u || !a->weather || !a->w_off || !a->timestep ||
        !a->reward || !a->done || (!a->action) == (!a->control) || a->weather_rows < 1) {
        g_err = "glgym_step: bad arguments (exactly one of action/control, ld >= B, non-null state/outputs)";
        return GLGYM_EINVAL;
    }
    if (h->step_integrator == GLGYM_INTEGRATOR_BDF) {
        DeviceGuard dev_guard(h);
        return h->dtype == GLGYM_F32 ? launch_step_bdf<float>(h, a, h->rf, (hipStream_t)stream)
                                     : launch_step_bdf<double>(h, a, h->rd, (hipStream_t)stream);
    }
    if (h->integrator != GLGYM_INTEGRATOR_EXPLICIT) {
        g_err = "glgym_step: GLGYM_INTEGRATOR_BDF is available to glgym_evalF only; set GLGYM_INTEGRATOR_EXPLICIT for env-steps";
        return GLGYM_EINVAL;
    }
    DeviceGuard dev_guard(h);
    hipStream_t st = (hipStream_t)stream;
    return h->dtype == GLGYM_F32 ? launch_step<float>(h, a, h->mf, h->rf, st, oa, fused)
                                 : launch_step<double>(h, a, h->md, h->rd, st);
}

extern "C" int glgym_step(glgym_handle h, const glgym_step_args* a, void* stream)
{
    return step_impl(h, a, stream, nullptr, nullptr);
}

template <class T> static int launch_obs(glgym_handle h, const glgym_obs_args* a, hipStream_t st)
{
    ObsArgsT<T> k;
    k.B = a->B; k.ld = a->ld; k.x = (const T*)a->x; k.u = (const T*)a->u; k.weather = (const T*)a->weather;
    k.weather_rows = a->weather_rows; k.w_off = a->w_off; k.timestep = a->timestep; k.start_day = a->start_day;
    k.Np = a->Np; k.obs = a->obs; k.mask = a->mask; k.term_obs = a->term_obs; k.nd = h->nd;
    obs_clock_increments(h, &k.doy_inc, &k.hod_inc);
    int blocks = (a->B + OBS_ROWS - 1) / OBS_ROWS;
    static const int cap = [] { const char* e = std::getenv("GLGYM_OBS_BLOCKS"); return e ? std::atoi(e) : 4096; }();
    if (blocks > cap) blocks = cap;
    obs_layout(h, a->Np, k.moff, &k.dim);
    const size_t lds = (size_t)OBS_ROWS * k.dim * sizeof(float);
    hipLaunchKernelGGL((obs_kernel<T>), dim3(blocks), dim3(256), lds, st, k);
    HIPCHK(hipGetLastError());
    return GLGYM_OK;
}



extern "C" int glgym_weather(glgym_handle h, const glgym_weather_args* a, void* stream)
{
    DeviceGuard dev_guard(h);
    if (!h || !a || a->n_raw < 3 || a->n_out < 1 || a->nd < ND || !a->time || !a->i_glob || !a->t_out || !a->rh || !a->wind ||
        !a->t_sky || !a->out || !a->workspace) {
        g_err = "glgym_weather: bad arguments (>= 3 raw samples, nd >= 10, non-null device pointers)";
        return GLGYM_EINVAL;
    }
    hipStream_t st = (hipStream_t)stream;
    const int n = a->n_raw;
    double* W = a->workspace;
    double* D = a->workspace + (size_t)10 * n;
    hipLaunchKernelGGL(weather_convert_kernel, dim3((n + 255) / 256), dim3(256), 0, st, n, a->time, a->i_glob, a->t_out,
                       a->rh, a->wind, a->t_sky, a->co2_ppm, W);
    hipLaunchKernelGGL(weather_scan_kernel, dim3(1), dim3(64), 0, st, n, a->time, W);
    hipLaunchKernelGGL(pchip_slopes_kernel, dim3((n + 255) / 256, 10), dim3(256), 0, st, n, 10, a->time, W, D);
    if (a->nd > ND) {
        HIPCHK(hipMemsetAsync(a->out, 0, (size_t)a->n_out * a->nd * (h->dtype == GLGYM_F32 ? 4 : 8), st));
    }
    const dim3 grid((a->n_out + 255) / 256, 10);
    if (h->dtype == GLGYM_F32)
        hipLaunchKernelGGL((pchip_eval_kernel<float>), grid, dim3(256), 0, st, n, 10, a->n_out, a->nd, a->time, W, D,
                           (float*)a->out);
    else
        hipLaunchKernelGGL((pchip_eval_kernel<double>), grid, dim3(256), 0, st, n, 10, a->n_out, a->nd, a->time, W, D,
                           (double*)a->out);
    HIPCHK(hipGetLastError());
    return GLGYM_OK;
}

extern "C" int glgym_vecnorm(glgym_handle h, const glgym_vecnorm_args* a, void* stream)
{
    DeviceGuard dev_guard(h);
    if (!h || !a || a->B < 1 || a->dim < 1 || !a->obs || !a->obs_out || !a->obs_mean || !a->obs_var || !a->obs_count ||
        !a->workspace || (a->reward && (!a->reward_out || !a->ret_stats || !a->returns))) {
        g_err = "glgym_vecnorm: bad arguments";
        return GLGYM_EINVAL;
    }
    hipStream_t st = (hipStream_t)stream;
    const int B = a->B, dim = a->dim;
    double* acc = a->workspace;
    double* acc2 = a->workspace + (size_t)VN_REP * 2 * dim;
    HIPCHK(hipMemsetAsync(a->workspace, 0, ((size_t)VN_REP * 2 * dim + 2) * sizeof(double), st));
    const int do_obs = a->training && a->norm_obs, do_ret = a->training && a->reward != nullptr;
    int col_threads = (dim + WAVE - 1) / WAVE * WAVE;
    if (col_threads > 1024) col_threads = 1024;
    if (do_obs) {
        int blocks = (B + 63) / 64;
        if (blocks > 1024) blocks = 1024;
        hipLaunchKernelGGL(vecnorm_moments_kernel, dim3(blocks), dim3(col_threads), 0, st, a->obs, B, dim, acc);
    }
    if (do_ret) {
        if (h->dtype == GLGYM_F32)
            hipLaunchKernelGGL((vecnorm_returns_kernel<float>), dim3((B + 255) / 256), dim3(256), 0, st,
                               (const float*)a->reward, a->returns, B, a->gamma, acc2);
        else
            hipLaunchKernelGGL((vecnorm_returns_kernel<double>), dim3((B + 255) / 256), dim3(256), 0, st,
                               (const double*)a->reward, a->returns, B, a->gamma, acc2);
    }
    double* scale = acc;
    if (do_obs || do_ret || a->norm_obs)
        hipLaunchKernelGGL(vecnorm_merge_kernel, dim3(1), dim3(1024), 0, st, a->obs_mean, a->obs_var, a->obs_count, acc, dim, B,
                           a->ret_stats, acc2, do_obs, do_ret, a->epsilon, a->norm_obs ? scale : nullptr);
    const size_t total = (size_t)B * dim;
    if (a->norm_obs) {
        int blocks = (B + 15) / 16;
        if (blocks > 8192) blocks = 8192;
        hipLaunchKernelGGL(vecnorm_apply_kernel, dim3(blocks), dim3(col_threads), 0, st, a->obs, a->obs_out, B, dim,
                           a->obs_mean, scale, a->clip_obs);
    } else if (a->obs_out != a->obs) {
        HIPCHK(hipMemcpyAsync(a->obs_out, a->obs, total * sizeof(float), hipMemcpyDeviceToDevice, st));
    }
    if (a->reward) {
        if (h->dtype == GLGYM_F32)
            hipLaunchKernelGGL((vecnorm_reward_kernel<float>), dim3((B + 255) / 256), dim3(256), 0, st,
                               (const float*)a->reward, a->reward_out, a->returns, a->done, B, a->ret_stats, a->epsilon,
                               a->clip_reward, a->norm_reward);
        else
            hipLaunchKernelGGL((vecnorm_reward_kernel<double>), dim3((B + 255) / 256), dim3(256), 0, st,
                               (const double*)a->reward, a->reward_out, a->returns, a->done, B, a->ret_stats, a->epsilon,
                               a->clip_reward, a->norm_reward);
    }
    HIPCHK(hipGetLastError());
    return GLGYM_OK;
}

extern "C" {

static bool obs_args_ok(glgym_handle h, const glgym_obs_args* a)
{
    return h && a && a->B >= 1 && a->ld >= a->B && a->x && a->u && a->weather && a->w_off && a->timestep && a->start_day && a->obs &&
           a->Np >= 0 && a->Np <= OBS_MAX_NP;
}

int glgym_obs(glgym_handle h, const glgym_obs_args* a, void* stream)
{
    DeviceGuard dev_guard(h);
    if (!obs_args_ok(h, a)) {
        g_err = "glgym_obs: bad arguments (null pointer, ld < B, or Np outside 0..128)";
        return GLGYM_EINVAL;
    }
    hipStream_t st = (hipStream_t)stream;
    return h->dtype == GLGYM_F32 ? launch_obs<float>(h, a, st) : launch_obs<double>(h, a, st);
}

int glgym_step_obs(glgym_handle h, const glgym_step_args* a, const glgym_obs_args* oa, void* stream)
{
    if (!h || !a || !oa) { g_err = "glgym_step_obs: null handle / arguments"; return GLGYM_EINVAL; }
    if (oa->mask) { g_err = "glgym_step_obs: full-mode observations only (glgym_obs_args.mask must be NULL)"; return GLGYM_EINVAL; }
    if (!obs_args_ok(h, oa)) {
        g_err = "glgym_step_obs: bad observation arguments (null pointer, ld < B, or Np outside 0..128)";
        return GLGYM_EINVAL;
    }
    bool fused = false;
    const int rc = step_impl(h, a, stream, oa, &fused);
    if (rc != GLGYM_OK || fused) return rc;
    return glgym_obs(h, oa, stream);
}

int glgym_set_obs_modules(glgym_handle h, const int32_t* modules, int n)
{
    if (!h || !modules || n < 1 || n > 6) { g_err = "glgym_set_obs_modules: 1..6 module ids expected"; return GLGYM_EINVAL; }
    int seen = 0;
    for (int i = 0; i < n; ++i) {
        if (modules[i] < 0 || modules[i] > 5 || (seen >> modules[i] & 1)) {
            g_err = "glgym_set_obs_modules: ids must be distinct GLGYM_OBS_* values";
            return GLGYM_EINVAL;
        }
        seen |= 1 << modules[i];
    }
    for (int i = 0; i < n; ++i) h->obs_modules[i] = modules[i];
    h->n_obs_modules = n;
    return GLGYM_OK;
}

int glgym_obs_dim(glgym_handle h, int Np)
{
    if (!h || Np < 0 || Np > OBS_MAX_NP) return GLGYM_EINVAL;
    int dim = 0;
    for (int i = 0; i < h->n_obs_modules; ++i)
        dim += h->obs_modules[i] == GLGYM_OBS_FORECAST ? 5 * Np : OBS_MODULE_SIZE[h->obs_modules[i]];
    return dim;
}

int glgym_reset(glgym_handle h, const glgym_reset_args* a, void* stream)
{
    DeviceGuard dev_guard(h);
    if (!h || !a || a->B < 1 || a->ld < a->B || !a->x || !a->u || !a->timestep || !a->weather || !a->w_off) {
        g_err = "glgym_reset: bad arguments";
        return GLGYM_EINVAL;
    }
    hipStream_t st = (hipStream_t)stream;
    const dim3 grid((a->B + 255) / 256), block(256);
    if (h->dtype == GLGYM_F32)
        hipLaunchKernelGGL((reset_kernel<float>), grid, block, 0, st, a->B, a->ld, a->mask, (float*)a->x, (float*)a->u,
                           a->timestep, (const float*)a->weather, a->weather_rows, a->w_off, a->start_rows, a->start_days,
                           a->n_starts, a->start_day, a->episode, (unsigned long long)a->seed, h->nd);
    else
        hipLaunchKernelGGL((reset_kernel<double>), grid, block, 0, st, a->B, a->ld, a->mask, (double*)a->x,
                           (double*)a->u, a->timestep, (const double*)a->weather, a->weather_rows, a->w_off,
                           a->start_rows, a->start_days, a->n_starts, a->start_day, a->episode,
                           (unsigned long long)a->seed, h->nd);
    HIPCHK(hipGetLastError());
    return GLGYM_OK;
}

int glgym_crop_noise(glgym_handle h, void* crop_p, int B, int ld, double scale, uint64_t seed, uint64_t draw_index,
                     void* stream)
{
    DeviceGuard dev_guard(h);
    if (!h || !crop_p || B < 1 || ld < B) return GLGYM_EINVAL;
    hipStream_t st = (hipStream_t)stream;
    const dim3 grid((B + 255) / 256), block(256);
    if (h->dtype == GLGYM_F32)
        hipLaunchKernelGGL((crop_noise_kernel<float>), grid, block, 0, st, (float*)crop_p, B, ld, h->p0_crop_dev,
                           (float)scale, (unsigned long long)seed, (unsigned long long)draw_index);
    else
        hipLaunchKernelGGL((crop_noise_kernel<double>), grid, block, 0, st, (double*)crop_p, B, ld, h->p0_crop_dev,
                           (float)scale, (unsigned long long)seed, (unsigned long long)draw_index);
    HIPCHK(hipGetLastError());
    return GLGYM_OK;
}

int glgym_rng_crop_noise(glgym_handle h, void* crop_p, int B, int ld, double scale, uint64_t* rng_state, void* stream)
{
    DeviceGuard dev_guard(h);
    if (!h || !rng_state || B < 1 || ld < B || !(scale >= 0.0)) {
        g_err = "glgym_rng_crop_noise: bad arguments (null handle or stream buffer, ld < B, or a negative scale)";
        return GLGYM_EINVAL;
    }
    hipStream_t st = (hipStream_t)stream;
    if (h->dtype == GLGYM_F32) HIPCHK(rng_crop_noise_launch<float>((float*)crop_p, B, ld, h->p0_crop_dev, scale, rng_state, st));
    else HIPCHK(rng_crop_noise_launch<double>((double*)crop_p, B, ld, h->p0_crop_dev, scale, rng_state, st));
    return GLGYM_OK;
}

int glgym_rng_reset_draw(glgym_handle h, int B, int ld, const unsigned char* mask, uint64_t* rng_state, int n_years, int n_days,
                         const int32_t* start_rows, const float* start_days, int32_t* w_off, float* start_day, void* stream)
{
    DeviceGuard dev_guard(h);
    if (!h || !rng_state || B < 1 || ld < B || n_years < 1 || n_days < 1 || !start_rows || !w_off) {
        g_err = "glgym_rng_reset_draw: bad arguments (null pointer, ld < B, or an empty start grid)";
        return GLGYM_EINVAL;
    }
    HIPCHK(rng_reset_draw_launch(B, ld, mask, rng_state, n_years, n_days, start_rows, start_days, w_off, start_day, (hipStream_t)stream));
    return GLGYM_OK;
}

static bool plan_size_ok(const char* who, int32_t got, size_t want)
{
    if (got == (int32_t)want) return true;
    g_err = std::string(who) + ": struct_size is " + std::to_string(got) + ", this library expects " + std::to_string(want) +
            " (ABI " + std::to_string(GLGYM_ABI_VERSION) + "): rebuild against include/glgym.h";
    return false;
}

int glgym_plan_fork(glgym_handle h, const glgym_plan_fork_args* a, void* stream)
{
    if (!h || !a) { g_err = "glgym_plan_fork: null handle / arguments"; return GLGYM_EINVAL; }
    if (!plan_size_ok("glgym_plan_fork", a->struct_size, sizeof *a)) return GLGYM_EINVAL;
    if (a->n_children < 1 || a->n_parents < 1 || a->ld_parent < a->n_parents || a->ld_child < a->n_children ||
        (!a->parent && (a->K < 1 || (int64_t)a->n_parents * a->K < a->n_children)) ||
        !a->x_parent || !a->u_parent || !a->timestep_parent || !a->w_off_parent || !a->x || !a->u || !a->timestep || !a->w_off ||
        !a->ret || !a->viol || !a->n_steps || !a->alive || !a->failed) {
        g_err = "glgym_plan_fork: bad arguments (null pointer, ld < batch, or without a parent table K < 1 or fewer than C = P * K slots)";
        return GLGYM_EINVAL;
    }
    DeviceGuard dev_guard(h);
    hipStream_t st = (hipStream_t)stream;
    if (h->dtype == GLGYM_F32) HIPCHK(plan_fork_launch<float>(*a, st));
    else HIPCHK(plan_fork_launch<double>(*a, st));
    return GLGYM_OK;
}

int glgym_plan_accumulate(glgym_handle h, const glgym_plan_accumulate_args* a, void* stream)
{
    if (!h || !a) { g_err = "glgym_plan_accumulate: null handle / arguments"; return GLGYM_EINVAL; }
    if (!plan_size_ok("glgym_plan_accumulate", a->struct_size, sizeof *a)) return GLGYM_EINVAL;
    if (a->B < 1 || a->ld < a->B || !a->reward || !a->info || !a->done || !a->ret || !a->viol || !a->n_steps || !a->alive || !a->failed) {
        g_err = "glgym_plan_accumulate: bad arguments (null pointer or ld < B)";
        return GLGYM_EINVAL;
    }
    DeviceGuard dev_guard(h);
    hipStream_t st = (hipStream_t)stream;
    if (h->dtype == GLGYM_F32) HIPCHK(plan_accumulate_launch<float>(*a, st));
    else HIPCHK(plan_accumulate_launch<double>(*a, st));
    return GLGYM_OK;
}

int glgym_plan_rollout(glgym_handle h, const glgym_plan_rollout_args* a, void* stream)
{
    if (!h || !a) { g_err = "glgym_plan_rollout: null handle / arguments"; return GLGYM_EINVAL; }
    if (!plan_size_ok("glgym_plan_rollout", a->struct_size, sizeof *a)) return GLGYM_EINVAL;
    if (a->H < 1 || !(a->gamma >= 0.0) || !std::isfinite(a->gamma) || (!a->actions) == (!a->controls) || a->step.B < 1 ||
        a->step.ld < a->step.B || !a->step.reward || !a->step.info || !a->step.done || !a->ret || !a->viol || !a->n_steps ||
        !a->alive || !a->failed) {
        g_err = "glgym_plan_rollout: bad arguments (H < 1, gamma, exactly one of actions / controls, ld >= B, non-null reward / info / done / accumulators)";
        return GLGYM_EINVAL;
    }
    glgym_step_args s = a->step;
    s.metrics = nullptr;
    glgym_plan_accumulate_args acc;
    acc.struct_size = (int32_t)sizeof acc;
    acc.B = s.B; acc.ld = s.ld; acc.reward = s.reward; acc.info = s.info; acc.done = s.done; acc.step_flags = s.step_flags;
    acc.ret = a->ret; acc.viol = a->viol; acc.n_steps = a->n_steps; acc.alive = a->alive; acc.failed = a->failed;
    const size_t plane = (size_t)NU * (size_t)s.ld * (h->dtype == GLGYM_F32 ? sizeof(float) : sizeof(double));
    double w = 1.0;
    for (int k = 0; k < a->H; ++k) {
        s.action = a->actions ? a->actions + (size_t)k * (size_t)s.B * NU : nullptr;
        s.control = a->controls ? (const void*)((const char*)a->controls + (size_t)k * plane) : nullptr;
        const int rc = glgym_step(h, &s, stream);
        if (rc != GLGYM_OK) return rc;
        acc.w = w;
        const int ra = glgym_plan_accumulate(h, &acc, stream);
        if (ra != GLGYM_OK) return ra;
        w = w * a->gamma;
    }
    return GLGYM_OK;
}

int glgym_plan_select(glgym_handle h, const glgym_plan_select_args* a, void* stream)
{
    if (!h || !a) { g_err = "glgym_plan_select: null handle / arguments"; return GLGYM_EINVAL; }
    if (!plan_size_ok("glgym_plan_select", a->struct_size, sizeof *a)) return GLGYM_EINVAL;
    const bool wants_actions = a->best_action || a->best_sequence || a->mean_sequence;
    if (a->P < 1 || a->K < 1 || a->H < 1 || a->H > 65535 || (int64_t)a->P * a->K > INT32_MAX || !a->ret || !a->failed || !a->best_k ||
        !a->best_ret || (wants_actions && !a->actions) || (a->mean_sequence && !(a->temperature > 0.0 && std::isfinite(a->temperature)))) {
        g_err = "glgym_plan_select: bad arguments (P, K, H < 1, H > 65 535, null pointer, action outputs without actions, or mean_sequence "
                "without a finite temperature > 0)";
        return GLGYM_EINVAL;
    }
    DeviceGuard dev_guard(h);
    HIPCHK(plan_select_launch(*a, (hipStream_t)stream));
    return GLGYM_OK;
}

int glgym_rule_based(glgym_handle h, const glgym_rule_cfg* cfg, const glgym_rule_args* a, void* stream)
{
    DeviceGuard dev_guard(h);
    if (!h || !cfg || !a || a->B < 1 || a->ld < a->B || !a->x || !a->weather || !a->w_off || !a->timestep || !a->control ||
        a->weather_rows < 1 || (!a->start_day && !a->doy) || cfg->vent_heat_Pband == 0 || cfg->vent_rh_Pband == 0 ||
        cfg->vent_cold_Pband == 0 || cfg->thScrPband == 0 || cfg->thScrRhPband == 0 || cfg->tHeatBand == 0 ||
        cfg->co2Band == 0) {
        g_err = "glgym_rule_based: bad arguments (null pointer, ld < B, or a zero proportional band)";
        return GLGYM_EINVAL;
    }
    hipStream_t st = (hipStream_t)stream;
    const dim3 grid((a->B + 255) / 256), block(256);
    const double doy_inc = std::fmod(h->dt / 86400.0, 365.0), hod_inc = h->dt / 3600.0;
    if (h->dtype == GLGYM_F32)
        hipLaunchKernelGGL((rule_based_kernel<float>), grid, block, 0, st, *cfg, a->B, a->ld, (const float*)a->x,
                           (const float*)a->weather, a->weather_rows, a->w_off, a->timestep, a->start_day, a->hour, a->doy,
                           doy_inc, hod_inc, (float*)a->control, h->nd);
    else
        hipLaunchKernelGGL((rule_based_kernel<double>), grid, block, 0, st, *cfg, a->B, a->ld, (const double*)a->x,
                           (const double*)a->weather, a->weather_rows, a->w_off, a->timestep, a->start_day, a->hour,
                           a->doy, doy_inc, hod_inc, (double*)a->control, h->nd);
    HIPCHK(hipGetLastError());
    return GLGYM_OK;
}

int glgym_timer_start(glgym_handle h, void* stream)
{
    DeviceGuard dev_guard(h);
    if (!h) return GLGYM_EINVAL;
    HIPCHK(hipEventRecord(h->ev0, (hipStream_t)stream));
    return GLGYM_OK;
}

int glgym_timer_stop(glgym_handle h, void* stream, float* elapsed_ms)
{
    DeviceGuard dev_guard(h);
    if (!h || !elapsed_ms) return GLGYM_EINVAL;
    HIPCHK(hipEventRecord(h->ev1, (hipStream_t)stream));
    HIPCHK(hipEventSynchronize(h->ev1));
    HIPCHK(hipEventElapsedTime(elapsed_ms, h->ev0, h->ev1));
    return GLGYM_OK;
}

}
```

### greenlight-gym2_amd/gl_gym_amd/_lib.py

```python
from __future__ import annotations

import ctypes as C
import os
from pathlib import Path

_HERE = Path(__file__).resolve().parent
LIB_PATH = Path(os.environ.get("GLGYM_LIB", _HERE / "libglgym.so"))

NX, NU, ND, NP, NCROP, NINFO, NMETRIC = 28, 6, 10, 208, 34, 11, 14
METRIC_REPLICAS, METRIC_STRIDE = 64, 32
F32, F64 = 0, 1
ODE, ODE_PIPE = 0, 1
SCHEME_RK4, SCHEME_RK2 = 0, 1
SCHEME_RK3 = 2
SCHEME_LS5 = 3
SCHEMES = {"rk4": SCHEME_RK4, "rk2": SCHEME_RK2, "rk3": SCHEME_RK3, "ls5": SCHEME_LS5}
ABI_VERSION = 7
INTEGRATORS = {"explicit": 0, "bdf": 1}
NSOLVER_STAT = 5
SOLVER_STAT_KEYS = ("steps", "rhs_evals", "jacobians", "factorisations", "order")
LAYOUTS = {"auto": 0, "one": 1, "quad": 2}
DEFAULT_N_SUB = {"rk4": 240, "rk2": 336, "rk3": 270, "ls5": 128}
DEFAULT_SCHEME = "ls5"
VERIFY_MODES = {"auto": 0, "always": 1, "never": 2}
N_SUB_MULTIPLE = {"rk4": 4, "rk2": 4, "rk3": 3, "ls5": 2}
PRESETS = {"throughput": {k: (v, 0) for k, v in DEFAULT_N_SUB.items()},
           "parity": {"ls5": (192, 1), "rk4": (640, 0), "rk3": (720, 0), "rk2": (896, 0)}}


def preset_n_sub(scheme: str, dt: float, preset: str = "throughput"):
    n0, window = PRESETS[preset][scheme]
    n = n0 * float(dt) / 900.0
    mult = window if window > 0 else N_SUB_MULTIPLE[scheme]
    return max(mult, int(-(-n // mult) * mult)), window


def resolve_scheme(scheme, variant: str = "ode") -> str:
    if variant not in ("ode", "ode_pipe"):
        raise ValueError("variant must be 'ode' or 'ode_pipe'")
    if scheme is None:
        return "rk4" if variant == "ode_pipe" else DEFAULT_SCHEME
    if scheme not in SCHEMES:
        raise ValueError("scheme must be 'ls5', 'rk4', 'rk3' or 'rk2'")
    if variant == "ode_pipe" and scheme != "rk4":
        raise ValueError(f"variant 'ode_pipe' is built for scheme 'rk4' only (got {scheme!r}): leave scheme unset or pass scheme='rk4'")
    return scheme


def default_n_sub(scheme: str, dt: float) -> int:
    return preset_n_sub(scheme, dt, "throughput")[0]
OK, EINVAL, ENODEV, EHIP, ENOMEM, EODE = 0, -1, -2, -3, -4, -5

INFO_KEYS = ("EPI", "revenue", "variable_costs", "fixed_costs", "co2_cost", "heat_cost", "elec_cost",
             "temp_violation", "co2_violation", "rh_violation", "lamp_violation")
METRIC_KEYS = ("sum_reward", "sum_EPI", "n_done", "n_ode_fail", "sum_co2_violation", "sum_temp_violation",
               "sum_rh_violation", "n_env_steps", "n_guard_retries", "n_refined_substeps", "n_flag_err", "n_flag_branch",
               "n_flag_cap", "n_flag_heavy")


class GlgymError(RuntimeError):
    pass


class GlgymOdeError(GlgymError):
    """glgym_evalF: the integration failed for at least one row (GLGYM_EODE) -- the counterpart of the RuntimeError the
    reference's evalF raises when CVODES fails (greenlight_model.cpp:110, caught at tomato_env.py:119-123)."""


class RewardCfg(C.Structure):
    _fields_ = [(n, C.c_double) for n in (
        "elec_price", "heating_price", "co2_price", "fruit_price", "dmfm", "fixed_greenhouse_cost", "fixed_co2_cost",
        "fixed_lamp_cost", "fixed_screen_cost", "pen_lamp", "co2_min", "co2_max", "temp_min", "temp_max", "rh_min",
        "rh_max")]


class StepArgs(C.Structure):
    _fields_ = [("struct_size", C.c_int32), ("B", C.c_int32), ("ld", C.c_int32), ("x", C.c_void_p), ("u", C.c_void_p), ("action", C.c_void_p),
                ("control", C.c_void_p), ("weather", C.c_void_p), ("weather_rows", C.c_int32), ("w_off", C.c_void_p),
                ("timestep", C.c_void_p), ("crop_p", C.c_void_p), ("N", C.c_int32), ("reward", C.c_void_p),
                ("info", C.c_void_p), ("done", C.c_void_p), ("metrics", C.c_void_p), ("step_flags", C.c_void_p)]


def make_step_args(*args, **kw):
    return StepArgs(C.sizeof(StepArgs), *args, **kw)


SF_FIRST_MASK, SF_ACCEPT_AGREE_FLAGGED, SF_ACCEPT_LAST_ALONE, SF_FAILED = 31, 32, 64, 128
SF_BDF = 2048
METRIC_BDF = 14
BDF_METRIC_KEYS = ("bdf_steps", "bdf_rhs_evals", "bdf_jacobians", "bdf_factorisations")


class ObsArgs(C.Structure):
    _fields_ = [("B", C.c_int32), ("ld", C.c_int32), ("x", C.c_void_p), ("u", C.c_void_p), ("weather", C.c_void_p),
                ("weather_rows", C.c_int32), ("w_off", C.c_void_p), ("timestep", C.c_void_p), ("start_day", C.c_void_p),
                ("Np", C.c_int32), ("obs", C.c_void_p), ("mask", C.c_void_p), ("term_obs", C.c_void_p)]


class ResetArgs(C.Structure):
    _fields_ = [("B", C.c_int32), ("ld", C.c_int32), ("mask", C.c_void_p), ("x", C.c_void_p), ("u", C.c_void_p),
                ("timestep", C.c_void_p), ("weather", C.c_void_p), ("weather_rows", C.c_int32), ("w_off", C.c_void_p),
                ("start_rows", C.c_void_p), ("start_days", C.c_void_p), ("n_starts", C.c_int32),
                ("start_day", C.c_void_p), ("episode", C.c_void_p), ("seed", C.c_uint64)]


class VecNormArgs(C.Structure):
    _fields_ = [("B", C.c_int32), ("dim", C.c_int32), ("obs", C.c_void_p), ("obs_out", C.c_void_p),
                ("reward", C.c_void_p), ("reward_out", C.c_void_p), ("done", C.c_void_p), ("obs_mean", C.c_void_p),
                ("obs_var", C.c_void_p), ("obs_count", C.c_void_p), ("ret_stats", C.c_void_p), ("returns", C.c_void_p),
                ("workspace", C.c_void_p), ("gamma", C.c_double), ("epsilon", C.c_double), ("clip_obs", C.c_float),
                ("clip_reward", C.c_float), ("training", C.c_int32), ("norm_obs", C.c_int32),
                ("norm_reward", C.c_int32)]


class PlanForkArgs(C.Structure):
    _fields_ = [("struct_size", C.c_int32), ("n_children", C.c_int32), ("n_parents", C.c_int32), ("K", C.c_int32),
                ("ld_parent", C.c_int32), ("ld_child", C.c_int32), ("parent", C.c_void_p), ("x_parent", C.c_void_p),
                ("u_parent", C.c_void_p), ("timestep_parent", C.c_void_p), ("w_off_parent", C.c_void_p),
                ("start_day_parent", C.c_void_p), ("crop_parent", C.c_void_p), ("x", C.c_void_p), ("u", C.c_void_p),
                ("timestep", C.c_void_p), ("w_off", C.c_void_p), ("start_day", C.c_void_p), ("crop", C.c_void_p),
                ("ret", C.c_void_p), ("viol", C.c_void_p), ("n_steps", C.c_void_p), ("alive", C.c_void_p), ("failed", C.c_void_p)]


class PlanAccumulateArgs(C.Structure):
    _fields_ = [("struct_size", C.c_int32), ("B", C.c_int32), ("ld", C.c_int32), ("w", C.c_double), ("reward", C.c_void_p),
                ("info", C.c_void_p), ("done", C.c_void_p), ("step_flags", C.c_void_p), ("ret", C.c_void_p), ("viol", C.c_void_p),
                ("n_steps", C.c_void_p), ("alive", C.c_void_p), ("failed", C.c_void_p)]


class PlanRolloutArgs(C.Structure):
    _fields_ = [("struct_size", C.c_int32), ("H", C.c_int32), ("gamma", C.c_double), ("step", StepArgs), ("actions", C.c_void_p),
                ("controls", C.c_void_p), ("ret", C.c_void_p), ("viol", C.c_void_p), ("n_steps", C.c_void_p), ("alive", C.c_void_p),
                ("failed", C.c_void_p)]


class PlanSelectArgs(C.Structure):
    _fields_ = [("struct_size", C.c_int32), ("P", C.c_int32), ("K", C.c_int32), ("H", C.c_int32), ("ret", C.c_void_p),
                ("failed", C.c_void_p), ("actions", C.c_void_p), ("best_k", C.c_void_p), ("best_ret", C.c_void_p),
                ("best_action", C.c_void_p), ("best_sequence", C.c_void_p), ("temperature", C.c_double),
                ("mean_sequence", C.c_void_p)]


def make_plan_args(cls, *args, **kw):
    return cls(C.sizeof(cls), *args, **kw)


RULE_FIELDS = ("lamps_on", "lamps_off", "lamps_day_start", "lamps_day_stop", "lamps_off_sun", "lamp_rad_sum_limit",
               "temp_setpoint_day", "temp_setpoint_night", "heat_correction", "heat_deadzone", "co2_day",
               "vent_heat_Pband", "rh_max", "mech_dehumid_Pband", "vent_rh_Pband", "t_vent_off", "vent_cold_Pband",
               "thScrSpDay", "thScrSpNight", "thScrPband", "thScrDeadZone", "thScrRh", "thScrRhPband", "lampExtraHeat",
               "blScrExtraRh", "rhMax", "tHeatBand", "co2Band", "useBlScr")


class RuleCfg(C.Structure):
    _fields_ = [(n, C.c_double) for n in RULE_FIELDS]


class RuleArgs(C.Structure):
    _fields_ = [("B", C.c_int32), ("ld", C.c_int32), ("x", C.c_void_p), ("weather", C.c_void_p),
                ("weather_rows", C.c_int32), ("w_off", C.c_void_p), ("timestep", C.c_void_p), ("start_day", C.c_void_p),
                ("hour", C.c_void_p), ("doy", C.c_void_p), ("control", C.c_void_p)]


class WeatherArgs(C.Structure):
    _fields_ = [("n_raw", C.c_int32), ("time", C.c_void_p), ("i_glob", C.c_void_p), ("t_out", C.c_void_p),
                ("rh", C.c_void_p), ("wind", C.c_void_p), ("t_sky", C.c_void_p), ("co2_ppm", C.c_double),
                ("n_out", C.c_int32), ("nd", C.c_int32), ("out", C.c_void_p), ("workspace", C.c_void_p)]


_DP = C.POINTER(C.c_double)
PROTOTYPES = {
    "glgym_version": (C.c_char_p, []),
    "glgym_abi_version": (C.c_int, []),
    "glgym_set_window": (C.c_int, [C.c_void_p, C.c_int]),
    "glgym_set_layout": (C.c_int, [C.c_void_p, C.c_int]),
    "glgym_set_occupancy": (C.c_int, [C.c_void_p, C.c_int]),
    "glgym_set_ladder_parallel": (C.c_int, [C.c_void_p, C.c_int]),
    "glgym_last_error": (C.c_char_p, []),
    "glgym_create": (C.c_int, [C.c_int, C.c_int, C.c_int, C.c_int, C.c_double, _DP, C.c_int, C.c_int, C.c_int,
                               C.POINTER(C.c_void_p)]),
    "glgym_destroy": (C.c_int, [C.c_void_p]),
    "glgym_set_params": (C.c_int, [C.c_void_p, _DP]),
    "glgym_set_params_keep_reward_scale": (C.c_int, [C.c_void_p, _DP]),
    "glgym_set_n_sub": (C.c_int, [C.c_void_p, C.c_int]),
    "glgym_set_model_variant": (C.c_int, [C.c_void_p, C.c_int]),
    "glgym_set_scheme": (C.c_int, [C.c_void_p, C.c_int]),
    "glgym_set_verify": (C.c_int, [C.c_void_p, C.c_int]),
    "glgym_set_reward": (C.c_int, [C.c_void_p, C.POINTER(RewardCfg)]),
    "glgym_get_reward_scale": (C.c_int, [C.c_void_p, _DP, _DP, _DP]),
    "glgym_evalF": (C.c_int, [C.c_void_p, _DP, _DP, _DP, _DP, C.c_int, C.c_int, _DP]),
    "glgym_rhs": (C.c_int, [C.c_void_p, _DP, _DP, _DP, C.c_int, _DP]),
    "glgym_set_integrator": (C.c_int, [C.c_void_p, C.c_int]),
    "glgym_set_tolerances": (C.c_int, [C.c_void_p, C.c_double, C.c_double, C.c_int]),
    "glgym_get_solver_stats": (C.c_int, [C.c_void_p, C.c_int, C.POINTER(C.c_int32)]),
    "glgym_set_step_integrator": (C.c_int, [C.c_void_p, C.c_int]),
    "glgym_step": (C.c_int, [C.c_void_p, C.POINTER(StepArgs), C.c_void_p]),
    "glgym_obs": (C.c_int, [C.c_void_p, C.POINTER(ObsArgs), C.c_void_p]),
    "glgym_step_obs": (C.c_int, [C.c_void_p, C.POINTER(StepArgs), C.POINTER(ObsArgs), C.c_void_p]),
    "glgym_set_obs_modules": (C.c_int, [C.c_void_p, C.POINTER(C.c_int32), C.c_int]),
    "glgym_obs_dim": (C.c_int, [C.c_void_p, C.c_int]),
    "glgym_set_control_limits": (C.c_int, [C.c_void_p, _DP, _DP, C.c_double]),
    "glgym_reset": (C.c_int, [C.c_void_p, C.POINTER(ResetArgs), C.c_void_p]),
    "glgym_crop_noise": (C.c_int, [C.c_void_p, C.c_void_p, C.c_int, C.c_int, C.c_double, C.c_uint64, C.c_uint64,
                                   C.c_void_p]),
    "glgym_rng_crop_noise": (C.c_int, [C.c_void_p, C.c_void_p, C.c_int, C.c_int, C.c_double, C.c_void_p, C.c_void_p]),
    "glgym_rng_reset_draw": (C.c_int, [C.c_void_p, C.c_int, C.c_int, C.c_void_p, C.c_void_p, C.c_int, C.c_int, C.c_void_p,
                                       C.c_void_p, C.c_void_p, C.c_void_p, C.c_void_p]),
    "glgym_plan_fork": (C.c_int, [C.c_void_p, C.POINTER(PlanForkArgs), C.c_void_p]),
    "glgym_plan_accumulate": (C.c_int, [C.c_void_p, C.POINTER(PlanAccumulateArgs), C.c_void_p]),
    "glgym_plan_rollout": (C.c_int, [C.c_void_p, C.POINTER(PlanRolloutArgs), C.c_void_p]),
    "glgym_plan_select": (C.c_int, [C.c_void_p, C.POINTER(PlanSelectArgs), C.c_void_p]),
    "glgym_rule_based": (C.c_int, [C.c_void_p, C.POINTER(RuleCfg), C.POINTER(RuleArgs), C.c_void_p]),
    "glgym_vecnorm": (C.c_int, [C.c_void_p, C.POINTER(VecNormArgs), C.c_void_p]),
    "glgym_weather": (C.c_int, [C.c_void_p, C.POINTER(WeatherArgs), C.c_void_p]),
    "glgym_timer_start": (C.c_int, [C.c_void_p, C.c_void_p]),
    "glgym_timer_stop": (C.c_int, [C.c_void_p, C.c_void_p, C.POINTER(C.c_float)]),
}

_lib = None


def load():
    global _lib
    if _lib is None:
        if not LIB_PATH.exists():
            raise GlgymError(f"{LIB_PATH} not found: build it with `python -c 'import __graft_entry__ as g; g.build()'` "
                             "(hipcc --offload-arch=gfx950).  There is no CPU fallback.")
        try:
            import torch
        except Exception:
            pass
        lib = C.CDLL(str(LIB_PATH))
        for name, (res, args) in PROTOTYPES.items():
            fn = getattr(lib, name)
            fn.restype, fn.argtypes = res, args
        if lib.glgym_abi_version() != ABI_VERSION:
            raise GlgymError(f"{LIB_PATH} has ABI {lib.glgym_abi_version()}, this binding expects {ABI_VERSION}: rebuild the library")
        _lib = lib
    return _lib


def check(rc: int, what: str = "glgym"):
    if rc != OK:
        msg = load().glgym_last_error().decode() or {EINVAL: "invalid argument", ENODEV: "no HIP device",
                                                       EHIP: "HIP error", ENOMEM: "out of memory"}.get(rc, "")
        raise (GlgymOdeError if rc == EODE else GlgymError)(f"{what} failed (status {rc}): {msg}")
```

### greenlight-gym2_amd/gl_gym_amd/tomato_env.py

```python
from __future__ import annotations

import ctypes as C
import os
from typing import Any, Dict, List, Optional, Sequence

import numpy as np

from . import _lib as L
from . import np_stream
from .greenlight_model import _check_integrator, _check_tolerances
from .parameters import init_default_params
from .utils import synthetic_weather

try:
    from gymnasium import spaces as _spaces

    def _box(low, high, shape, dtype=np.float32):
        return _spaces.Box(low=low, high=high, shape=shape, dtype=dtype)
except Exception:
    class _Box:
        def __init__(self, low, high, shape, dtype):
            self.low = np.broadcast_to(np.asarray(low, dtype=dtype), shape).copy()
            self.high = np.broadcast_to(np.asarray(high, dtype=dtype), shape).copy()
            self.shape, self.dtype = tuple(shape), np.dtype(dtype)
            self._rng = np.random.default_rng()

        def seed(self, seed=None):
            self._rng = np.random.default_rng(seed)

        def sample(self):
            return self._rng.uniform(self.low, self.high).astype(self.dtype)

        def contains(self, v):
            v = np.asarray(v)
            return v.shape == self.shape and bool(np.all(v >= self.low) and np.all(v <= self.high))

    def _box(low, high, shape, dtype=np.float32):
        return _Box(low, high, shape, dtype)

DEFAULT_REWARD = dict(fixed_greenhouse_cost=15., fixed_co2_cost=0.015, fixed_lamp_cost=0.07, fixed_screen_cost=2.,
                      elec_price=0.3, heating_price=0.09, co2_price=0.3, fruit_price=1.6, dmfm=0.065,
                      pen_weights=[4.e-4, 5.e-3, 7.e-4], pen_lamp=0.1)
DEFAULT_CONSTRAINTS = dict(co2_min=300., co2_max=1600., temp_min=15., temp_max=34., rh_min=50., rh_max=85.)


def _torch():
    import torch
    return torch


RNGS = ("philox", "numpy")


def _check_rng(rng, start_grid, n_starts):
    if rng not in RNGS:
        raise ValueError("rng must be 'philox' or 'numpy'")
    if start_grid is None:
        return rng, ((1, int(n_starts)) if rng == "numpy" else None)
    grid = tuple(int(v) for v in start_grid)
    if len(grid) != 2 or grid[0] < 1 or grid[1] < 1 or grid[0] * grid[1] != int(n_starts):
        raise ValueError(f"start_grid must be (n_years, n_days) with n_years * n_days = len(start_rows) = {n_starts}, got {start_grid!r}")
    return rng, grid


def _observation_modules(Np, names):
    return observation_modules(Np, names)


class ObservationModule:

    def __init__(self, name, obs_names, low=-1e-4, high=1e4):
        self.name, self.obs_names, self.n_obs, self.low, self.high = name, list(obs_names), len(obs_names), low, high

    def __repr__(self):
        return f"{self.name}({self.n_obs})"


OBSERVATION_MODULE_IDS = {"IndoorClimateObservations": 0, "BasicCropObservations": 1, "ControlObservations": 2,
                          "WeatherObservations": 3, "TimeObservations": 4, "WeatherForecastObservations": 5}
DEFAULT_OBSERVATION_MODULES = ["IndoorClimateObservations", "BasicCropObservations", "ControlObservations",
                               "WeatherObservations", "TimeObservations", "WeatherForecastObservations"]


def observation_modules(Np: int, names: Optional[Sequence[str]] = None):
    wx = ["glob_rad", "temp_out", "rh_out", "co2_out", "wind_speed"]
    table = {"IndoorClimateObservations": (["co2_air", "temp_air", "rh_air", "pipe_temp"],),
             "BasicCropObservations": (["24CanTemp", "cFruit", "tSum"],),
             "ControlObservations": (["uBoil", "uCo2", "uThScr", "uVent", "uLamp", "uBlScr"], 0.0, 1.0),
             "WeatherObservations": (wx,),
             "TimeObservations": (["timestep", "day of year sin", "day of year cos", "hour of day sin",
                                   "hour of day cos"],),
             "WeatherForecastObservations": (wx * Np,)}
    names = DEFAULT_OBSERVATION_MODULES if names is None else list(names)
    for n in names:
        if n == "StateObservations":
            raise NotImplementedError("StateObservations cannot be built by the reference's TomatoEnv either "
                                      "(observations.py:42: __init__ takes no env) and returns random numbers (:57)")
        if n not in table:
            raise KeyError(f"unknown observation module {n!r}; known: {sorted(table)}")
    if len(set(names)) != len(names) or not names:
        raise ValueError("observation_modules must be a non-empty list without repeats")
    return [ObservationModule(n, *table[n]) for n in names]


class LazyInfos:

    def __init__(self, keys, info_rows, controls, dones, term_obs, step_flags=None):
        self._keys, self._rows, self._ctrl, self._dones, self._term = keys, info_rows, controls, dones, term_obs
        self._flags = step_flags
        self._cache = {}

    def __len__(self):
        return len(self._rows)

    def _make(self, b):
        d = dict(zip(self._keys, self._rows[b].tolist()))
        d["controls"] = self._ctrl[b]
        d["TimeLimit.truncated"] = False
        if self._flags is not None:
            d["integration"] = int(self._flags[b])
        if self._term is not None and self._dones[b]:
            d["terminal_observation"] = self._term[b]
        return d

    def __getitem__(self, b):
        if isinstance(b, slice):
            return [self[i] for i in range(*b.indices(len(self)))]
        b = int(b)
        if b < 0:
            b += len(self)
        if b not in self._cache:
            self._cache[b] = self._make(b)
        return self._cache[b]

    def __setitem__(self, b, value):
        self._cache[int(b)] = value

    def __iter__(self):
        return (self[i] for i in range(len(self)))


class _EpochLib:

    def __init__(self, lib, env):
        self.__dict__["_lib"], self.__dict__["_env"] = lib, env

    def __getattr__(self, name):
        fn, env = getattr(self._lib, name), self._env

        def call(*args):
            env._epoch += 1
            return fn(*args)
        self.__dict__[name] = call
        return call


class TomatoVecEnv:
    def __init__(self, num_envs: int, weather: Optional[np.ndarray] = None, params: Optional[np.ndarray] = None,
                 dt: float = 900.0, season_length: float = 60, pred_horizon: float = 0.5, dtype: str = "float32",
                 n_sub: Optional[int] = None, device: str = "cuda:0", seed: int = 0, uncertainty_scale: float = 0.0,
                 start_rows: Optional[Sequence[int]] = None, start_days: Optional[Sequence[float]] = None,
                 reward_params: Optional[Dict[str, Any]] = None, constraints: Optional[Dict[str, float]] = None,
                 auto_reset: bool = True, collect_metrics: bool = True, lazy_infos: Optional[bool] = None,
                 model_variant: str = "ode", scheme: Optional[str] = None, window: Optional[int] = None,
                 preset: Optional[str] = None,
                 observation_modules: Optional[Sequence[str]] = None, u_min: Optional[Sequence[float]] = None,
                 u_max: Optional[Sequence[float]] = None, delta_u_max: float = 0.1, integration_info: bool = True,
                 integrator: str = "explicit", rtol: float = 1e-6, atol: float = 1e-6, max_steps: int = 10000,
                 rng: str = "philox", start_grid: Optional[Sequence[int]] = None, env_index_offset: int = 0):
        _check_integrator(integrator, model_variant)
        _check_tolerances(rtol, atol, max_steps)
        _check_rng(rng, start_grid, 1 if start_rows is None else len(start_rows))
        torch = _torch()
        if not torch.cuda.is_available():
            raise L.GlgymError("TomatoVecEnv needs a HIP device (torch.cuda.is_available() is False); "
                               "there is no CPU fallback")
        self._epoch = 0
        self._obs_token = None
        self._obs_followed = False
        self._stepped = False
        self.n_fused_steps = 0
        self.n_obs_elided = 0
        self._lib = _EpochLib(L.load(), self)
        self.torch = torch
        self.device = torch.device(device)
        torch.cuda.set_device(self.device)
        self.num_envs = self.B = int(num_envs)
        self.ld = (self.B + 63) // 64 * 64
        self.dt = float(dt)
        self.c = 86400
        self.nx, self.nu, self.num_params = L.NX, L.NU, L.NP
        weather_is_tensor = weather is not None and hasattr(weather, "data_ptr")
        self.nd = L.ND if weather is None else int(np.shape(weather)[1])
        if model_variant not in ("ode", "ode_pipe"):
            raise ValueError("model_variant must be 'ode' or 'ode_pipe'")
        self.model_variant = model_variant
        self.season_length = season_length
        self.N = int(season_length * self.c / self.dt)
        self.Np = int(pred_horizon * self.c / self.dt)
        self.observation_modules = _observation_modules(self.Np, observation_modules)
        if self.observation_modules[0].name != "IndoorClimateObservations":
            raise NotImplementedError("observation_modules must start with IndoorClimateObservations: the reference's "
                                      "GreenhouseReward takes co2 / temperature / humidity from obs[0:3]")
        self.obs_dim = sum(m.n_obs for m in self.observation_modules)
        self.f64 = str(dtype) in ("float64", "f64", "double")
        self.tdtype = torch.float64 if self.f64 else torch.float32
        scheme = L.resolve_scheme(scheme, model_variant)
        self.preset = ("parity" if self.f64 else "throughput") if preset is None else preset
        if self.preset not in L.PRESETS:
            raise ValueError("preset must be 'throughput' or 'parity'")
        self.scheme = scheme
        n_def, w_def = L.preset_n_sub(scheme, self.dt, self.preset)
        self.n_sub = int(n_def if n_sub is None else n_sub)
        self.window = int((w_def if n_sub is None else 0) if window is None else window)
        self.uncertainty_scale = float(uncertainty_scale)
        self.auto_reset = auto_reset
        self.lazy_infos = (int(num_envs) > 4096) if lazy_infos is None else bool(lazy_infos)
        self.integration_info = bool(integration_info)
        self.seed_value = int(seed)

        self._p = np.asarray(init_default_params(L.NP) if params is None else params, dtype=np.float32)
        self._h = C.c_void_p()
        p64 = np.ascontiguousarray(self.p, dtype=np.float64)
        L.check(self._lib.glgym_create(L.NX, L.NU, self.nd, L.NP, self.dt, p64.ctypes.data_as(L._DP),
                                       L.F64 if self.f64 else L.F32, self.n_sub, self.device.index or 0,
                                       C.byref(self._h)), "glgym_create")
        self._env_at_create = tuple(os.environ.get(k) for k in ("GLGYM_LAYOUT", "GLGYM_OCC", "GLGYM_VERIFY"))
        if model_variant == "ode_pipe":
            L.check(self._lib.glgym_set_model_variant(self._h, L.ODE_PIPE), "glgym_set_model_variant")
        L.check(self._lib.glgym_set_scheme(self._h, L.SCHEMES[scheme]), "glgym_set_scheme")
        L.check(self._lib.glgym_set_window(self._h, self.window), "glgym_set_window")
        self.rtol, self.atol, self.max_steps = float(rtol), float(atol), int(max_steps)
        self.set_integrator(integrator)
        self.u_min = np.asarray([0.0] * L.NU if u_min is None else u_min, dtype=np.float32)
        self.u_max = np.asarray([1.0] * L.NU if u_max is None else u_max, dtype=np.float32)
        self.delta_u_max = np.ones(L.NU, dtype=np.float32) * np.float32(delta_u_max)
        if self.u_min.shape != (L.NU,) or self.u_max.shape != (L.NU,):
            raise ValueError("u_min / u_max must have 6 entries")
        lo64, hi64 = self.u_min.astype(np.float64), self.u_max.astype(np.float64)
        L.check(self._lib.glgym_set_control_limits(self._h, lo64.ctypes.data_as(L._DP), hi64.ctypes.data_as(L._DP),
                                                   float(delta_u_max)), "glgym_set_control_limits")
        ids = (C.c_int32 * len(self.observation_modules))(*[OBSERVATION_MODULE_IDS[m.name] for m in self.observation_modules])
        L.check(self._lib.glgym_set_obs_modules(self._h, ids, len(ids)), "glgym_set_obs_modules")
        assert self._lib.glgym_obs_dim(self._h, self.Np) == self.obs_dim
        rp = dict(DEFAULT_REWARD, **(reward_params or {}))
        cs = dict(DEFAULT_CONSTRAINTS, **(constraints or {}))
        self.reward_params, self.constraints = rp, cs
        cfg = L.RewardCfg(rp["elec_price"], rp["heating_price"], rp["co2_price"], rp["fruit_price"], rp["dmfm"],
                          rp["fixed_greenhouse_cost"], rp["fixed_co2_cost"], rp["fixed_lamp_cost"],
                          rp["fixed_screen_cost"], rp["pen_lamp"], cs["co2_min"], cs["co2_max"], cs["temp_min"],
                          cs["temp_max"], cs["rh_min"], cs["rh_max"])
        L.check(self._lib.glgym_set_reward(self._h, C.byref(cfg)), "glgym_set_reward")
        mx, mn, fx = C.c_double(), C.c_double(), C.c_double()
        L.check(self._lib.glgym_get_reward_scale(self._h, C.byref(mx), C.byref(mn), C.byref(fx)))
        self.max_profit, self.min_profit, self.fixed_costs = mx.value, mn.value, fx.value

        if weather is None:
            weather = synthetic_weather(dt=self.dt)
        self._weather_data = (weather.detach().double().cpu().numpy() if weather_is_tensor
                              else np.ascontiguousarray(weather, dtype=np.float64))
        self.weather_rows = int(self._weather_data.shape[0])
        need = self.N + 1 + self.Np + 1
        if self.weather_rows < need:
            raise ValueError(f"weather tensor has {self.weather_rows} rows, an episode needs {need}")
        if start_rows is None:
            start_rows = [0]
        self.start_rows = np.asarray(start_rows, dtype=np.int64)
        if np.any(self.start_rows + need > self.weather_rows) or np.any(self.start_rows < 0):
            raise ValueError("start_rows + episode length exceeds the weather tensor")
        self.start_days = np.asarray(start_days if start_days is not None
                                     else self.start_rows * self.dt / self.c, dtype=np.float32)
        self.rng, self.start_grid = _check_rng(rng, start_grid, len(self.start_rows))
        self.env_index_offset = int(env_index_offset)

        dev, T = self.device, self.tdtype
        z = lambda *s, dtype=T: torch.zeros(*s, dtype=dtype, device=dev)
        self.weather_t = (weather.to(device=dev, dtype=T).contiguous() if weather_is_tensor
                          else torch.as_tensor(self.weather_data, dtype=T, device=dev).contiguous())
        self.x_T, self.u_T = z(L.NX, self.ld), z(L.NU, self.ld)
        self.ctrl_T = z(L.NU, self.ld)
        self.info_T = z(L.NINFO, self.ld)
        self.reward_t = z(self.ld)
        self.done_t = z(self.B, dtype=torch.uint8)
        self.timestep_t = z(self.B, dtype=torch.int32)
        self.w_off_t = z(self.B, dtype=torch.int32)
        self.start_day_t = z(self.B, dtype=torch.float32)
        self.action_t = z(self.B, L.NU, dtype=torch.float32)
        self.obs_t = z(self.B, self.obs_dim, dtype=torch.float32)
        self.term_obs_t = z(self.B, self.obs_dim, dtype=torch.float32)
        self.metrics_t = z(L.METRIC_REPLICAS, L.METRIC_STRIDE, dtype=torch.float32) if collect_metrics else None
        self.step_flags_t = z(self.B, dtype=torch.int32)
        self.crop_T = z(L.NCROP, self.ld) if self.uncertainty_scale > 0 else None
        self._start_rows_t = torch.as_tensor(self.start_rows, dtype=torch.int32, device=dev)
        self._start_days_t = torch.as_tensor(self.start_days, dtype=torch.float32, device=dev)
        self.episode_t = z(self.B, dtype=torch.int32)
        self._draw = 0
        self.rng_state_t = z(np_stream.NWORD, self.ld, dtype=torch.int64) if self.rng == "numpy" else None
        if self.rng == "numpy":
            self._seed_streams(self.seed_value)
        self.x, self.u = self.x_T[:, :self.B].t(), self.u_T[:, :self.B].t()

        lo = np.concatenate([np.full(m.n_obs, m.low, np.float32) for m in self.observation_modules])
        hi = np.concatenate([np.full(m.n_obs, m.high, np.float32) for m in self.observation_modules])
        self.observation_space = _box(lo, hi, (self.obs_dim,), np.float32)
        self.action_space = _box(-1.0, 1.0, (L.NU,), np.float32)
        self._actions = None
        self._keep_applied_u, self._u_applied_T = False, None
        self.reset_infos: List[dict] = [{} for _ in range(self.B)]
        self._obs_host = [torch.empty(self.B, self.obs_dim, dtype=torch.float32).pin_memory() for _ in range(2)]
        self._obs_flip = 0

    def _obs_to_host(self, obs_t):
        buf = self._obs_host[self._obs_flip]
        self._obs_flip ^= 1
        buf.copy_(obs_t, non_blocking=True)
        self.torch.cuda.current_stream(self.device).synchronize()
        return buf.numpy()

    def _stream(self):
        return C.c_void_p(self.torch.cuda.current_stream(self.device).cuda_stream)

    def _seed_streams(self, seed: int):
        first = int(seed) + self.env_index_offset
        self.set_rng_state(np_stream.seed_states(range(first, first + self.B)))

    def get_rng_state(self) -> List[dict]:
        if self.rng_state_t is None:
            raise L.GlgymError("get_rng_state: this environment was built with rng='philox' (stateless, keyed by seed and counters)")
        return np_stream.unpack_states(self.rng_state_t[:, :self.B].cpu().numpy().view(np.uint64))

    def set_rng_state(self, states):
        if self.rng_state_t is None:
            raise L.GlgymError("set_rng_state: this environment was built with rng='philox'")
        words = states if isinstance(states, np.ndarray) else np_stream.pack_states(states)
        if words.shape != (np_stream.NWORD, self.B):
            raise ValueError(f"set_rng_state: expected {self.B} states, got an array of shape {words.shape}")
        self.rng_state_t[:, :self.B].copy_(self.torch.as_tensor(np.ascontiguousarray(words, dtype=np.uint64).view(np.int64)))

    _STATE_TENSORS = ("x_T", "u_T", "timestep_t", "w_off_t", "start_day_t", "episode_t", "crop_T", "rng_state_t", "obs_t", "done_t")

    def get_state(self) -> Dict[str, Any]:
        state: Dict[str, Any] = {k: (None if getattr(self, k) is None else getattr(self, k).clone()) for k in self._STATE_TENSORS}
        state.update(_draw=int(self._draw), seed_value=int(self.seed_value), num_envs=self.B, dtype=str(self.tdtype), rng=self.rng)
        return state

    def set_state(self, state: Dict[str, Any]):
        missing = [k for k in self._STATE_TENSORS + ("_draw", "seed_value", "num_envs", "dtype", "rng") if k not in state]
        if missing:
            raise ValueError(f"set_state: not a get_state() snapshot (missing {missing})")
        if state["num_envs"] != self.B or state["dtype"] != str(self.tdtype) or state["rng"] != self.rng:
            raise ValueError(f"set_state: snapshot of {state['num_envs']} envs, {state['dtype']}, rng={state['rng']!r} does not fit "
                             f"this environment ({self.B} envs, {self.tdtype}, rng={self.rng!r})")
        for k in self._STATE_TENSORS:
            mine, theirs = getattr(self, k), state[k]
            if (mine is None) != (theirs is None) or (mine is not None and (mine.shape != theirs.shape or mine.dtype != theirs.dtype)):
                raise ValueError(f"set_state: {k} of the snapshot does not fit this environment")
        for k in self._STATE_TENSORS:
            if getattr(self, k) is not None:
                getattr(self, k).copy_(state[k])
        self._draw, self.seed_value = int(state["_draw"]), int(state["seed_value"])

    def planner(self, n_candidates: int, horizon: int, gamma: float = 1.0, crop: str = "nominal"):
        from .planner import Planner
        return Planner(self, n_candidates, horizon, gamma=gamma, crop=crop)

    def _launch_reset(self, mask_t):
        mask_ptr = mask_t.data_ptr() if mask_t is not None else None
        if self.rng == "numpy":
            L.check(self._lib.glgym_rng_reset_draw(self._h, self.B, self.ld, mask_ptr, self.rng_state_t.data_ptr(), self.start_grid[0],
                                                   self.start_grid[1], self._start_rows_t.data_ptr(), self._start_days_t.data_ptr(),
                                                   self.w_off_t.data_ptr(), self.start_day_t.data_ptr(), self._stream()),
                    "glgym_rng_reset_draw")
            a = L.ResetArgs(self.B, self.ld, mask_ptr, self.x_T.data_ptr(), self.u_T.data_ptr(), self.timestep_t.data_ptr(),
                            self.weather_t.data_ptr(), self.weather_rows, self.w_off_t.data_ptr(), None, None, 0,
                            self.start_day_t.data_ptr(), self.episode_t.data_ptr(), self.seed_value)
            L.check(self._lib.glgym_reset(self._h, C.byref(a), self._stream()), "glgym_reset")
            return
        a = L.ResetArgs(self.B, self.ld, mask_t.data_ptr() if mask_t is not None else None, self.x_T.data_ptr(),
                        self.u_T.data_ptr(), self.timestep_t.data_ptr(), self.weather_t.data_ptr(), self.weather_rows,
                        self.w_off_t.data_ptr(), self._start_rows_t.data_ptr(), self._start_days_t.data_ptr(),
                        len(self.start_rows), self.start_day_t.data_ptr(), self.episode_t.data_ptr(), self.seed_value)
        L.check(self._lib.glgym_reset(self._h, C.byref(a), self._stream()), "glgym_reset")

    def _obs_args(self, out_t, mask_t=None, term_t=None):
        return L.ObsArgs(self.B, self.ld, self.x_T.data_ptr(), self.u_T.data_ptr(), self.weather_t.data_ptr(),
                         self.weather_rows, self.w_off_t.data_ptr(), self.timestep_t.data_ptr(),
                         self.start_day_t.data_ptr(), self.Np, out_t.data_ptr(),
                         mask_t.data_ptr() if mask_t is not None else None,
                         term_t.data_ptr() if term_t is not None else None)

    def _obs_deps(self):
        return tuple((t.data_ptr(), t._version) for t in (self.x_T, self.u_T, self.timestep_t, self.w_off_t, self.start_day_t,
                                                          self.weather_t, self.obs_t))

    def _launch_obs(self, out_t, mask_t=None, term_t=None):
        if mask_t is None:
            token, self._obs_token = self._obs_token, None
            if out_t is self.obs_t:
                self._obs_followed = self._stepped
                if token is not None and token == (id(out_t), self._epoch, self._obs_deps()):
                    self.n_obs_elided += 1
                    return
        L.check(self._lib.glgym_obs(self._h, C.byref(self._obs_args(out_t, mask_t, term_t)), self._stream()), "glgym_obs")

    def _launch_step(self, raw_control: bool, want_obs: Optional[bool] = None):
        if self._env_at_create is not None and tuple(os.environ.get(k) for k in ("GLGYM_LAYOUT", "GLGYM_OCC", "GLGYM_VERIFY")) != self._env_at_create:
            import warnings
            warnings.warn("GLGYM_LAYOUT / GLGYM_OCC / GLGYM_VERIFY changed after this TomatoVecEnv was created: they are read once, at glgym_create, "
                          "and have no effect on an existing handle -- use set_layout() / set_occupancy() / set_verify()", RuntimeWarning, stacklevel=3)
            self._env_at_create = None
        fuse = self._obs_followed if want_obs is None else bool(want_obs)
        self._obs_followed, self._obs_token, self._stepped = False, None, True
        if self.rng == "numpy":
            if not getattr(self, "freeze_crop_noise", False):
                L.check(self._lib.glgym_rng_crop_noise(self._h, self.crop_T.data_ptr() if self.crop_T is not None else None, self.B, self.ld,
                                                       self.uncertainty_scale, self.rng_state_t.data_ptr(), self._stream()),
                        "glgym_rng_crop_noise")
        elif self.crop_T is not None and not getattr(self, "freeze_crop_noise", False):
            L.check(self._lib.glgym_crop_noise(self._h, self.crop_T.data_ptr(), self.B, self.ld,
                                               self.uncertainty_scale, self.seed_value, self._draw, self._stream()),
                    "glgym_crop_noise")
            self._draw += 1
        a = L.make_step_args(self.B, self.ld, self.x_T.data_ptr(), self.u_T.data_ptr(),
                       None if raw_control else getattr(self, "_action_src", self.action_t).data_ptr(),
                       self.ctrl_T.data_ptr() if raw_control else None, self.weather_t.data_ptr(), self.weather_rows,
                       self.w_off_t.data_ptr(), self.timestep_t.data_ptr(),
                       self.crop_T.data_ptr() if self.crop_T is not None else None, self.N,
                       self.reward_t.data_ptr(), self.info_T.data_ptr(), self.done_t.data_ptr(),
                       self.metrics_t.data_ptr() if self.metrics_t is not None else None, self.step_flags_t.data_ptr())
        if not fuse:
            L.check(self._lib.glgym_step(self._h, C.byref(a), self._stream()), "glgym_step")
            return
        L.check(self._lib.glgym_step_obs(self._h, C.byref(a), C.byref(self._obs_args(self.obs_t)), self._stream()), "glgym_step_obs")
        self.n_fused_steps += 1
        self._obs_token = (id(self.obs_t), self._epoch, self._obs_deps())

    def reset_tensor(self, seed: Optional[int] = None):
        if seed is not None:
            self.seed_value = int(seed)
            self.episode_t.zero_()
            if self.rng == "numpy":
                self._seed_streams(self.seed_value)
        self._launch_reset(None)
        self._launch_obs(self.obs_t)
        return self.obs_t

    def _launch_rule_based(self, controller, hour_t=None, doy_t=None):
        cfg = L.RuleCfg(*[float(getattr(controller, n)) for n in L.RULE_FIELDS])
        if hour_t is None and (self.dt / 3600) * 8 != round((self.dt / 3600) * 8):
            hour_t = self.hour_of_day()
        a = L.RuleArgs(self.B, self.ld, self.x_T.data_ptr(), self.weather_t.data_ptr(), self.weather_rows,
                       self.w_off_t.data_ptr(), self.timestep_t.data_ptr(), self.start_day_t.data_ptr(),
                       hour_t.data_ptr() if hour_t is not None else None,
                       doy_t.data_ptr() if doy_t is not None else None, self.ctrl_T.data_ptr())
        L.check(self._lib.glgym_rule_based(self._h, C.byref(cfg), C.byref(a), self._stream()), "glgym_rule_based")

    def step_tensor(self, actions_t=None, controls_t=None, want_obs: bool = True, controller=None):
        if (actions_t is not None) + (controls_t is not None) + (controller is not None) != 1:
            raise ValueError("give exactly one of actions_t / controls_t / controller")
        self._action_src = self.action_t
        if actions_t is not None:
            if (actions_t.dtype == self.torch.float32 and actions_t.is_cuda and actions_t.device == self.device and
                    actions_t.is_contiguous() and actions_t.numel() == self.B * L.NU):
                self._action_src = actions_t
            else:
                self.action_t.copy_(actions_t.reshape(self.B, L.NU))
        elif controls_t is not None:
            self.ctrl_T[:, :self.B].copy_(controls_t.reshape(self.B, L.NU).t())
        else:
            self._launch_rule_based(controller)
        self._launch_step(raw_control=actions_t is None, want_obs=want_obs)
        if want_obs:
            self._launch_obs(self.obs_t)
        if self.auto_reset:
            if self._keep_applied_u:
                if self._u_applied_T is None:
                    self._u_applied_T = self.torch.empty_like(self.u_T)
                self._u_applied_T.copy_(self.u_T)
                self._u_applied_valid = True
            else:
                self._u_applied_valid = False
            self._launch_reset(self.done_t)
            if want_obs:
                self._launch_obs(self.obs_t, self.done_t, self.term_obs_t)
        return self.obs_t, self.reward_t[:self.B], self.done_t, self.info_T[:, :self.B]

    def reset(self):
        return self._obs_to_host(self.reset_tensor())

    def seed(self, seed: Optional[int] = None):
        if seed is not None:
            self.seed_value = int(seed)
            if self.rng == "numpy":
                self._seed_streams(self.seed_value)
        return [seed] * self.B

    def step_async(self, actions):
        self._actions = np.asarray(actions, dtype=np.float32)

    def step_wait(self):
        self._keep_applied_u = True
        try:
            return self._host_result(self.step_tensor(self.torch.as_tensor(self._actions, device=self.device)))
        finally:
            self._keep_applied_u = False

    def _host_result(self, out):
        obs_t, r_t, d_t, info_T = out
        obs, rew = self._obs_to_host(obs_t), r_t.float().cpu().numpy()
        dones, infos = self.host_infos(d_t, info_T)
        return obs, rew, dones, infos

    def host_infos(self, d_t, info_T, term_obs=None):
        dones = d_t.cpu().numpy().astype(bool)
        rows = info_T.double().t().cpu().numpy()
        applied = self._u_applied_T if (self.auto_reset and getattr(self, "_u_applied_valid", False)) else self.u_T
        ctrl = applied[:, :self.B].t().double().cpu().numpy()
        term = None
        if self.auto_reset and dones.any():
            term = self.term_obs_t.cpu().numpy() if term_obs is None else term_obs
        flags = self.step_flags_t.cpu().numpy() if self.integration_info else None
        if self.lazy_infos:
            infos = LazyInfos(L.INFO_KEYS, rows, ctrl, dones, term, flags)
        else:
            infos = [dict(zip(L.INFO_KEYS, row), controls=c) for row, c in zip(rows.tolist(), ctrl)]
            for d in infos:
                d["TimeLimit.truncated"] = False
            if flags is not None:
                for d, f in zip(infos, flags.tolist()):
                    d["integration"] = f
            if term is not None:
                for b in np.nonzero(dones)[0]:
                    infos[b]["terminal_observation"] = term[b]
        return dones, infos

    def step(self, actions):
        self.step_async(actions)
        return self.step_wait()

    def step_raw_control(self, controls):
        torch = self.torch
        obs_t, r_t, d_t, info_T = self.step_tensor(controls_t=torch.as_tensor(np.asarray(controls), dtype=self.tdtype,
                                                                              device=self.device))
        return self._obs_to_host(obs_t), r_t.float().cpu().numpy(), d_t.cpu().numpy().astype(bool), info_T.cpu().numpy()

    def step_raw_control_pipeinput(self, controls):
        torch = self.torch
        _, _, d_t, _ = self.step_tensor(controls_t=torch.as_tensor(np.asarray(controls), dtype=self.tdtype,
                                                                   device=self.device), want_obs=False)
        return self.x.double().cpu().numpy(), d_t.cpu().numpy().astype(bool)

    def _indices(self, indices):
        if indices is None:
            return list(range(self.B))
        return [indices] if isinstance(indices, int) else list(indices)

    def get_attr(self, attr_name: str, indices=None):
        idx = self._indices(indices)
        per_env = {"x": lambda b: self.x[b].double().cpu().numpy(), "u": lambda b: self.u[b].double().cpu().numpy(),
                   "timestep": lambda b: int(self.timestep_t[b]), "start_day": lambda b: float(self.start_day_t[b]),
                   "w_off": lambda b: int(self.w_off_t[b])}
        if attr_name == "growth_year" and getattr(self, "start_years", None) is not None:
            w_off = self.w_off_t.cpu().numpy()
            return [int(self.start_years[int(np.searchsorted(self.start_rows, w_off[b], side="right")) - 1]) for b in idx]
        if attr_name in per_env:
            return [per_env[attr_name](b) for b in idx]
        return [getattr(self, attr_name) for _ in idx]

    def set_attr(self, attr_name: str, value, indices=None):
        setattr(self, attr_name, value)

    def env_method(self, method_name: str, *args, indices=None, **kwargs):
        return [getattr(self, method_name)(*args, **kwargs) for _ in self._indices(indices)]

    def env_is_wrapped(self, wrapper_class, indices=None):
        return [False for _ in self._indices(indices)]

    def get_obs_names(self):
        return [n for m in self.observation_modules for n in m.obs_names]

    def set_seed(self, seed: int):
        self.seed_value = int(seed)
        self.episode_t.zero_()
        if self.rng == "numpy":
            self._seed_streams(self.seed_value)

    def current_weather(self):
        idx = (self.w_off_t + self.timestep_t).long().clamp_(0, self.weather_rows - 1)
        return self.weather_t[idx]

    @property
    def weather_data(self):
        return self._weather_data

    @weather_data.setter
    def weather_data(self, table):
        torch = self.torch
        table = np.ascontiguousarray(table.detach().double().cpu().numpy() if hasattr(table, "detach") else table, dtype=np.float64)
        if table.ndim != 2 or table.shape[1] != self._weather_data.shape[1]:
            raise ValueError(f"weather_data: expected [rows, {self._weather_data.shape[1]}] like the table this env was built with, got {table.shape}")
        need = self.N + 1 + self.Np + 1
        if table.shape[0] < need:
            raise ValueError(f"weather_data has {table.shape[0]} rows, an episode needs {need}")
        self._weather_data = table
        self.weather_rows = int(table.shape[0])
        self._epoch += 1
        self.weather_t = torch.as_tensor(table, dtype=self.tdtype, device=self.device).contiguous()
        self.start_rows = np.zeros(1, dtype=np.int64)
        self.start_days = np.asarray(self.start_days[:1], dtype=np.float32)
        self._start_rows_t = torch.as_tensor(self.start_rows, dtype=torch.int32, device=self.device)
        self._start_days_t = torch.as_tensor(self.start_days, dtype=torch.float32, device=self.device)
        if self.rng == "numpy":
            self.start_grid = (1, 1)
        self.w_off_t.zero_()

    @property
    def p(self):
        return self._p

    @p.setter
    def p(self, value):
        value = np.asarray(value, dtype=np.float32)
        if value.shape != (L.NP,):
            raise ValueError(f"p: expected {L.NP} parameters, got an array of shape {value.shape}")
        p64 = np.ascontiguousarray(value, dtype=np.float64)
        L.check(self._lib.glgym_set_params_keep_reward_scale(self._h, p64.ctypes.data_as(L._DP)), "glgym_set_params_keep_reward_scale")
        self._p = value

    def _hod_table(self):
        if getattr(self, "_hod_table_t", None) is None:
            t = np.empty(self.N + 4, dtype=np.float64)
            h = 0.0
            for k in range(len(t)):
                t[k] = h
                h = (h + self.dt / 3600) % 24
            self._hod_table_t = self.torch.as_tensor(t, device=self.device)
        return self._hod_table_t

    def hour_of_day(self):
        return self._hod_table()[self.timestep_t.long().clamp_(0, self.N + 3)]

    def day_of_year(self):
        return self.start_day_t.double() + self.timestep_t.double() * ((self.dt / self.c) % 365)

    def rule_based_controls(self, controller):
        self._launch_rule_based(controller)
        return self.ctrl_T[:, :self.B].t().clone()

    def step_rule_based(self, controller):
        return self._host_result(self.step_tensor(controller=controller))

    def metrics(self) -> Dict[str, float]:
        if self.metrics_t is None:
            return {}
        v = self.metrics_t.double().sum(dim=0)[:L.NMETRIC].cpu().numpy()
        return {k: float(v[i]) for i, k in enumerate(L.METRIC_KEYS)}

    def capture_step_graph(self, want_obs: bool = True):
        if self.crop_T is not None and self.rng != "numpy":
            raise L.GlgymError("capture_step_graph: per-step crop noise carries a host-side draw counter; use step_tensor")
        torch = self.torch
        static_a = torch.zeros(self.B, L.NU, dtype=torch.float32, device=self.device)

        def seq():
            self.action_t.copy_(static_a)
            self._action_src = self.action_t
            self._launch_step(raw_control=False, want_obs=want_obs)
            if want_obs:
                self._launch_obs(self.obs_t)
            if self.auto_reset:
                self._launch_reset(self.done_t)
                if want_obs:
                    self._launch_obs(self.obs_t, self.done_t, self.term_obs_t)

        state = [self.x_T, self.u_T, self.timestep_t, self.w_off_t, self.start_day_t, self.episode_t, self.obs_t]
        if self.rng == "numpy":
            state += [self.rng_state_t] + ([self.crop_T] if self.crop_T is not None else [])
        keep = [b.clone() for b in state]
        metrics = None if self.metrics_t is None else self.metrics_t.clone()
        side = torch.cuda.Stream(device=self.device)
        side.wait_stream(torch.cuda.current_stream(self.device))
        with torch.cuda.stream(side):
            seq()
        torch.cuda.current_stream(self.device).wait_stream(side)
        for b, k in zip(state, keep):
            b.copy_(k)
        if metrics is not None:
            self.metrics_t.copy_(metrics)
        graph = torch.cuda.CUDAGraph()
        with torch.cuda.graph(graph):
            seq()
        for b, k in zip(state, keep):
            b.copy_(k)
        if metrics is not None:
            self.metrics_t.copy_(metrics)

        def replay(actions_t):
            static_a.copy_(actions_t.reshape(self.B, L.NU))
            graph.replay()
            return self.obs_t, self.reward_t[:self.B], self.done_t, self.info_T[:, :self.B]
        replay.graph = graph
        return replay

    def set_scheme(self, scheme: str, n_sub: Optional[int] = None, window: Optional[int] = None):
        if scheme not in L.SCHEMES:
            raise ValueError("scheme must be 'ls5', 'rk4', 'rk3' or 'rk2'")
        L.check(self._lib.glgym_set_scheme(self._h, L.SCHEMES[scheme]), "glgym_set_scheme")
        self.scheme = scheme
        n_def, w_def = L.preset_n_sub(scheme, self.dt, self.preset)
        self.set_n_sub(n_def if n_sub is None else n_sub)
        self.set_window((w_def if n_sub is None else 0) if window is None else window)

    def set_integrator(self, name: str, rtol: Optional[float] = None, atol: Optional[float] = None,
                       max_steps: Optional[int] = None):
        rtol = self.rtol if rtol is None else rtol
        atol = self.atol if atol is None else atol
        max_steps = self.max_steps if max_steps is None else max_steps
        _check_integrator(name, self.model_variant)
        _check_tolerances(rtol, atol, max_steps)
        L.check(self._lib.glgym_set_tolerances(self._h, float(rtol), float(atol), int(max_steps)), "glgym_set_tolerances")
        L.check(self._lib.glgym_set_step_integrator(self._h, L.INTEGRATORS[name]), "glgym_set_step_integrator")
        self.integrator, self.rtol, self.atol, self.max_steps = name, float(rtol), float(atol), int(max_steps)

    def solver_metrics(self) -> Dict[str, float]:
        if self.metrics_t is None:
            return {}
        v = self.metrics_t.double().sum(dim=0)[L.METRIC_BDF:L.METRIC_BDF + len(L.BDF_METRIC_KEYS)].cpu().numpy()
        return {k: float(v[i]) for i, k in enumerate(L.BDF_METRIC_KEYS)}

    def set_window(self, window: int):
        self.window = int(window)
        L.check(self._lib.glgym_set_window(self._h, self.window), "glgym_set_window")

    def set_layout(self, layout: str):
        L.check(self._lib.glgym_set_layout(self._h, L.LAYOUTS[layout]), "glgym_set_layout")

    def set_occupancy(self, waves_per_simd: int):
        L.check(self._lib.glgym_set_occupancy(self._h, int(waves_per_simd)), "glgym_set_occupancy")

    def set_ladder_parallel(self, on: bool):
        L.check(self._lib.glgym_set_ladder_parallel(self._h, int(bool(on))), "glgym_set_ladder_parallel")

    def set_n_sub(self, n_sub: int):
        self.n_sub = int(n_sub)
        L.check(self._lib.glgym_set_n_sub(self._h, self.n_sub), "glgym_set_n_sub")

    def set_verify(self, mode: str):
        L.check(self._lib.glgym_set_verify(self._h, L.VERIFY_MODES[mode]), "glgym_set_verify")

    def timer_start(self):
        L.check(self._lib.glgym_timer_start(self._h, self._stream()))

    def timer_stop(self) -> float:
        ms = C.c_float()
        L.check(self._lib.glgym_timer_stop(self._h, self._stream(), C.byref(ms)))
        return float(ms.value)

    def close(self):
        if getattr(self, "_h", None) is not None and self._h.value:
            self.torch.cuda.synchronize(self.device)
            self._lib.glgym_destroy(self._h)
            self._h = C.c_void_p()

    def __del__(self):
        try:
            self.close()
        except Exception:
            pass


class TomatoEnv:

    def __init__(self, weather=None, params=None, dt=900.0, season_length=60, pred_horizon=0.5, dtype="float64",
                 n_sub=None, device="cuda:0", uncertainty_scale=0.0, start_day=0.0, growth_year=2010,
                 reward_params=None, constraints=None, location="synthetic", training=True, model_variant="ode",
                 scheme="rk4", observation_modules=None, u_min=None, u_max=None, delta_u_max=0.1, integrator="explicit", rtol=1e-6,
                 atol=1e-6, max_steps=10000, rng="philox"):
        self.vec = TomatoVecEnv(1, rng=rng, model_variant=model_variant, scheme=scheme, observation_modules=observation_modules,
                                u_min=u_min, u_max=u_max, delta_u_max=delta_u_max, integrator=integrator, rtol=rtol, atol=atol,
                                max_steps=max_steps,
                                weather=weather, params=params, dt=dt, season_length=season_length,
                                pred_horizon=pred_horizon, dtype=dtype, n_sub=n_sub, device=device,
                                uncertainty_scale=uncertainty_scale, start_rows=[0], start_days=[start_day],
                                reward_params=reward_params, constraints=constraints, auto_reset=False)
        v = self.vec
        self.nx, self.nu, self.nd, self.num_params, self.dt, self.c = v.nx, v.nu, v.nd, v.num_params, v.dt, v.c
        self.N, self.Np = v.N, v.Np
        self.observation_space, self.action_space = v.observation_space, v.action_space
        self.start_day, self.growth_year, self.location, self.training = start_day, growth_year, location, training
        self.u_min, self.u_max, self.delta_u_max = v.u_min, v.u_max, v.delta_u_max
        self.terminated = False

    def _set_x(self, value):
        value = np.asarray(value, dtype=np.float64).reshape(L.NX)
        self.vec.x_T[:, 0] = self.vec.torch.as_tensor(value, dtype=self.vec.tdtype, device=self.vec.device)

    x = property(lambda self: self.vec.x[0].double().cpu().numpy(), _set_x)
    weather_data = property(lambda self: self.vec.weather_data, lambda self, table: setattr(self.vec, "weather_data", table))
    u = property(lambda self: self.vec.u[0].double().cpu().numpy())
    p = property(lambda self: self.vec.p, lambda self, value: setattr(self.vec, "p", value))
    timestep = property(lambda self: int(self.vec.timestep_t[0]))
    day_of_year = property(lambda self: self.start_day + self.timestep * ((self.dt / self.c) % 365))
    hour_of_day = property(lambda self: float(self.vec.hour_of_day()[0]))

    def reset(self, seed: Optional[int] = None):
        obs = self.vec.reset_tensor(seed)
        self.terminated = False
        return obs[0].double().cpu().numpy(), {}

    def action_to_control(self, action):
        return np.clip(self.u + np.asarray(action) * self.delta_u_max, self.u_min, self.u_max)

    def _finish(self, out):
        obs_t, r_t, d_t, info_T = out
        info = {k: float(info_T[i, 0]) for i, k in enumerate(L.INFO_KEYS)}
        info["controls"] = self.u
        self.terminated = bool(d_t[0])
        return obs_t[0].double().cpu().numpy(), float(r_t[0]), self.terminated, False, info

    def step(self, action):
        t = self.vec.torch
        return self._finish(self.vec.step_tensor(t.as_tensor(np.asarray(action, dtype=np.float32).reshape(1, 6),
                                                             device=self.vec.device)))

    def step_raw_control(self, control):
        t = self.vec.torch
        return self._finish(self.vec.step_tensor(controls_t=t.as_tensor(np.asarray(control).reshape(1, 6),
                                                                        dtype=self.vec.tdtype, device=self.vec.device)))

    def step_raw_control_pipeinput(self, control):
        x, term = self.vec.step_raw_control_pipeinput(np.asarray(control).reshape(1, 6))
        self.terminated = bool(term[0])
        return x[0], self.terminated

    def set_crop_state(self, cBuf, cLeaf, cStem, cFruit, tCanSum):
        for i, v in zip((22, 23, 24, 25, 26), (cBuf, cLeaf, cStem, cFruit, tCanSum)):
            self.vec.x_T[i, 0] = v

    def get_state(self):
        return dict(self.vec.get_state(), terminated=self.terminated)

    def set_state(self, state):
        self.vec.set_state(state)
        self.terminated = bool(state.get("terminated", False))

    def get_obs_names(self):
        return self.vec.get_obs_names()

    def close(self):
        self.vec.close()
```

### include/glgym.h

```cpp
#ifndef GLGYM_H
#define GLGYM_H

#include <stddef.h>
#include <stdint.h>

#ifdef __cplusplus
extern "C" {
#endif

#define GLGYM_NX 28
#define GLGYM_NU 6
#define GLGYM_ND 10
#define GLGYM_NP 208
#define GLGYM_NCROP 34
#define GLGYM_NINFO 11
#define GLGYM_NMETRIC 14
#define GLGYM_METRIC_BDF 14
#define GLGYM_METRIC_REPLICAS 64
#define GLGYM_METRIC_STRIDE 32

typedef struct glgym_handle_s* glgym_handle;

typedef enum { GLGYM_F32 = 0, GLGYM_F64 = 1 } glgym_dtype;

typedef enum { GLGYM_ODE = 0, GLGYM_ODE_PIPE = 1 } glgym_variant;

typedef enum { GLGYM_SCHEME_RK4 = 0, GLGYM_SCHEME_RK2 = 1, GLGYM_SCHEME_RK3 = 2, GLGYM_SCHEME_LS5 = 3 } glgym_scheme;

typedef enum { GLGYM_VERIFY_AUTO = 0, GLGYM_VERIFY_ALWAYS = 1, GLGYM_VERIFY_NEVER = 2 } glgym_verify;

typedef enum {
    GLGYM_OK = 0,
    GLGYM_EINVAL = -1,
    GLGYM_ENODEV = -2,
    GLGYM_EHIP = -3,
    GLGYM_ENOMEM = -4,
    GLGYM_EODE = -5
} glgym_status;

typedef struct {
    double elec_price, heating_price, co2_price, fruit_price, dmfm;
    double fixed_greenhouse_cost, fixed_co2_cost, fixed_lamp_cost, fixed_screen_cost;
    double pen_lamp;
    double co2_min, co2_max, temp_min, temp_max, rh_min, rh_max;
} glgym_reward_cfg;

#define GLGYM_ABI_VERSION 7

typedef struct {
    int32_t struct_size;
    int32_t B;
    int32_t ld;
    void* x;
    void* u;
    const float* action;
    const void* control;
    const void* weather;
    int32_t weather_rows;
    const int32_t* w_off;
    int32_t* timestep;
    const void* crop_p;
    int32_t N;
    void* reward;
    void* info;
    uint8_t* done;
    float* metrics;
    int32_t* step_flags;
} glgym_step_args;

#define GLGYM_SF_ACCEPT_AGREE_FLAGGED 32
#define GLGYM_SF_ACCEPT_LAST_ALONE 64
#define GLGYM_SF_FAILED 128
#define GLGYM_SF_BDF 2048

typedef struct {
    int32_t B, ld;
    const void* x;
    const void* u;
    const void* weather;
    int32_t weather_rows;
    const int32_t* w_off;
    const int32_t* timestep;
    const float* start_day;
    int32_t Np;
    float* obs;
    const uint8_t* mask;
    float* term_obs;
} glgym_obs_args;

typedef struct {
    int32_t B, ld;
    const uint8_t* mask;
    void* x;
    void* u;
    int32_t* timestep;
    const void* weather;
    int32_t weather_rows;
    int32_t* w_off;
    const int32_t* start_rows;
    const float* start_days;
    int32_t n_starts;
    float* start_day;
    int32_t* episode;
    uint64_t seed;
} glgym_reset_args;

const char* glgym_version(void);
int glgym_abi_version(void);
const char* glgym_last_error(void);

int glgym_create(int nx, int nu, int nd, int np, double dt, const double* p, int dtype, int n_sub, int device,
                 glgym_handle* out);
int glgym_destroy(glgym_handle h);
int glgym_set_params(glgym_handle h, const double* p);
int glgym_set_params_keep_reward_scale(glgym_handle h, const double* p);
int glgym_set_n_sub(glgym_handle h, int n_sub);
int glgym_set_scheme(glgym_handle h, int scheme);
int glgym_set_window(glgym_handle h, int window);
typedef enum { GLGYM_LAYOUT_AUTO = 0, GLGYM_LAYOUT_ONE = 1, GLGYM_LAYOUT_QUAD = 2 } glgym_layout;
int glgym_set_layout(glgym_handle h, int layout);
int glgym_set_occupancy(glgym_handle h, int waves_per_simd);
int glgym_set_ladder_parallel(glgym_handle h, int on);
int glgym_set_verify(glgym_handle h, int mode);
int glgym_set_control_limits(glgym_handle h, const double* u_min , const double* u_max , double delta_u_max);
int glgym_set_model_variant(glgym_handle h, int variant);
int glgym_set_reward(glgym_handle h, const glgym_reward_cfg* cfg);
int glgym_get_reward_scale(glgym_handle h, double* max_profit, double* min_profit, double* fixed_costs);

int glgym_evalF(glgym_handle h, const double* x, const double* u, const double* d, const double* p, int p_rows,
                int B, double* x_next);
int glgym_rhs(glgym_handle h, const double* x, const double* u, const double* d, int B, double* dx);

typedef enum { GLGYM_INTEGRATOR_EXPLICIT = 0, GLGYM_INTEGRATOR_BDF = 1 } glgym_integrator;
int glgym_set_integrator(glgym_handle h, int integrator);
int glgym_set_step_integrator(glgym_handle h, int integrator);
int glgym_set_tolerances(glgym_handle h, double rtol, double atol, int max_steps);
#define GLGYM_NSOLVER_STAT 5
int glgym_get_solver_stats(glgym_handle h, int B, int32_t* stats);

enum { GLGYM_OBS_INDOOR = 0,
       GLGYM_OBS_CROP = 1,
       GLGYM_OBS_CONTROL = 2,
       GLGYM_OBS_WEATHER = 3,
       GLGYM_OBS_TIME = 4,
       GLGYM_OBS_FORECAST = 5    };
int glgym_set_obs_modules(glgym_handle h, const int32_t* modules, int n);
int glgym_obs_dim(glgym_handle h, int Np);

int glgym_step(glgym_handle h, const glgym_step_args* a, void* stream);
int glgym_obs(glgym_handle h, const glgym_obs_args* a, void* stream);
int glgym_step_obs(glgym_handle h, const glgym_step_args* step, const glgym_obs_args* obs, void* stream);
int glgym_reset(glgym_handle h, const glgym_reset_args* a, void* stream);
int glgym_crop_noise(glgym_handle h, void* crop_p, int B, int ld, double scale, uint64_t seed, uint64_t draw_index,
                     void* stream);

int glgym_rng_crop_noise(glgym_handle h, void* crop_p, int B, int ld, double scale, uint64_t* rng_state, void* stream);
int glgym_rng_reset_draw(glgym_handle h, int B, int ld, const unsigned char* mask, uint64_t* rng_state, int n_years, int n_days,
                         const int32_t* start_rows, const float* start_days, int32_t* w_off, float* start_day, void* stream);

typedef struct {
    int32_t struct_size;
    int32_t n_children;
    int32_t n_parents;
    int32_t K;
    int32_t ld_parent, ld_child;
    const int32_t* parent;
    const void* x_parent;
    const void* u_parent;
    const int32_t* timestep_parent;
    const int32_t* w_off_parent;
    const float* start_day_parent;
    const void* crop_parent;
    void* x;
    void* u;
    int32_t* timestep;
    int32_t* w_off;
    float* start_day;
    void* crop;
    double* ret;
    double* viol;
    int32_t* n_steps;
    uint8_t* alive;
    uint8_t* failed;
} glgym_plan_fork_args;

typedef struct {
    int32_t struct_size;
    int32_t B, ld;
    double w;
    const void* reward;
    const void* info;
    const uint8_t* done;
    const int32_t* step_flags;
    double* ret;
    double* viol;
    int32_t* n_steps;
    uint8_t* alive;
    uint8_t* failed;
} glgym_plan_accumulate_args;

typedef struct {
    int32_t struct_size;
    int32_t H;
    double gamma;
    glgym_step_args step;
    const float* actions;
    const void* controls;
    double* ret;
    double* viol;
    int32_t* n_steps;
    uint8_t* alive;
    uint8_t* failed;
} glgym_plan_rollout_args;

typedef struct {
    int32_t struct_size;
    int32_t P, K, H;
    const double* ret;
    const uint8_t* failed;
    const float* actions;
    int32_t* best_k;
    double* best_ret;
    float* best_action;
    float* best_sequence;
    double temperature;
    float* mean_sequence;
} glgym_plan_select_args;

int glgym_plan_fork(glgym_handle h, const glgym_plan_fork_args* a, void* stream);
int glgym_plan_accumulate(glgym_handle h, const glgym_plan_accumulate_args* a, void* stream);
int glgym_plan_rollout(glgym_handle h, const glgym_plan_rollout_args* a, void* stream);
int glgym_plan_select(glgym_handle h, const glgym_plan_select_args* a, void* stream);

typedef struct {
    double lamps_on, lamps_off, lamps_day_start, lamps_day_stop, lamps_off_sun, lamp_rad_sum_limit;
    double temp_setpoint_day, temp_setpoint_night, heat_correction, heat_deadzone, co2_day;
    double vent_heat_Pband, rh_max, mech_dehumid_Pband, vent_rh_Pband, t_vent_off, vent_cold_Pband;
    double thScrSpDay, thScrSpNight, thScrPband, thScrDeadZone, thScrRh, thScrRhPband, lampExtraHeat;
    double blScrExtraRh, rhMax, tHeatBand, co2Band, useBlScr;
} glgym_rule_cfg;

typedef struct {
    int32_t B, ld;
    const void* x;
    const void* weather;
    int32_t weather_rows;
    const int32_t* w_off;
    const int32_t* timestep;
    const float* start_day;
    const double* hour;
    const double* doy;
    void* control;
} glgym_rule_args;

int glgym_rule_based(glgym_handle h, const glgym_rule_cfg* cfg, const glgym_rule_args* a, void* stream);

typedef struct {
    int32_t B, dim;
    const float* obs;
    float* obs_out;
    const void* reward;
    float* reward_out;
    const uint8_t* done;
    double* obs_mean;
    double* obs_var;
    double* obs_count;
    double* ret_stats;
    double* returns;
    double* workspace;
    double gamma, epsilon;
    float clip_obs, clip_reward;
    int32_t training, norm_obs, norm_reward;
} glgym_vecnorm_args;

int glgym_vecnorm(glgym_handle h, const glgym_vecnorm_args* a, void* stream);

typedef struct {
    int32_t n_raw;
    const double* time;
    const double* i_glob;
    const double* t_out;
    const double* rh;
    const double* wind;
    const double* t_sky;
    double co2_ppm;
    int32_t n_out;
    int32_t nd;
    void* out;
    double* workspace;
} glgym_weather_args;

int glgym_weather(glgym_handle h, const glgym_weather_args* a, void* stream);

int glgym_timer_start(glgym_handle h, void* stream);
int glgym_timer_stop(glgym_handle h, void* stream, float* elapsed_ms);

#ifdef __cplusplus
}
#endif
#endif
```

Baseline: 102.5 million.

## Fuse auto-reset and terminal-observation capture into the step+obs kernel epilogue

```diff
diff --git a/greenlight-gym2_amd/csrc/glgym.hip b/greenlight-gym2_amd/csrc/glgym.hip
--- a/greenlight-gym2_amd/csrc/glgym.hip
+++ b/greenlight-gym2_amd/csrc/glgym.hip
@@ -100,6 +100,56 @@
 __device__ __forceinline__ constexpr int obs_core_module(int j) { return j < 4 ? 0 : j < 7 ? 1 : j < 13 ? 2 : j < 18 ? 3 : 4; }
 __device__ __forceinline__ constexpr int obs_core_col(int j) { return j < 4 ? j : j < 7 ? j - 4 : j < 13 ? j - 7 : j < 18 ? j - 13 : j - 18; }
 
+__device__ __forceinline__ void philox4x32_10(unsigned c0, unsigned c1, unsigned c2, unsigned c3, unsigned k0,
+                                              unsigned k1, unsigned* out)
+{
+#pragma unroll
+    for (int r = 0; r < 10; ++r) {
+        const unsigned long long p0 = 0xD2511F53ull * c0, p1 = 0xCD9E8D57ull * c2;
+        const unsigned n0 = (unsigned)(p1 >> 32) ^ c1 ^ k0, n1 = (unsigned)p1;
+        const unsigned n2 = (unsigned)(p0 >> 32) ^ c3 ^ k1, n3 = (unsigned)p0;
+        c0 = n0; c1 = n1; c2 = n2; c3 = n3;
+        k0 += 0x9E3779B9u; k1 += 0xBB67AE85u;
+    }
+    out[0] = c0; out[1] = c1; out[2] = c2; out[3] = c3;
+}
+
+template <class T>
+__device__ __forceinline__ void reset_env(int b, int ld, T* x, T* u, int* timestep, const T* weather, int weather_rows, int* w_off,
+                                          const int* start_rows, const float* start_days, int n_starts, float* start_day, int* episode,
+                                          unsigned long long seed, int nd)
+{
+#pragma clang fp contract(off)
+    if (start_rows && n_starts > 0) {
+        const int ep = episode ? episode[b] : 0;
+        unsigned rnd[4];
+        philox4x32_10((unsigned)b, (unsigned)ep, 0x5eedu, 0u, (unsigned)seed, (unsigned)(seed >> 32), rnd);
+        const int j = (int)(rnd[0] % (unsigned)n_starts);
+        w_off[b] = start_rows[j];
+        if (start_day && start_days) start_day[b] = start_days[j];
+        if (episode) episode[b] = ep + 1;
+    }
+    int r = w_off[b];
+    r = r < 0 ? 0 : (r >= weather_rows ? weather_rows - 1 : r);
+    const double co2Out = (double)weather[(size_t)r * nd + 3], tSoOut = (double)weather[(size_t)r * nd + 6];
+    const double tAir = 16.5;
+    double xi[NX];
+    xi[0] = xi[1] = co2Out;
+    for (int i = 2; i <= 10; ++i) xi[i] = tAir;
+    xi[4] = tAir + 4;
+    xi[11] = 0.25 * (3.0 * tAir + tSoOut);
+    xi[12] = 0.25 * __builtin_fma(2.0, tSoOut, 2.0 * tAir);
+    xi[13] = 0.25 * __builtin_fma(3.0, tSoOut, tAir);
+    xi[14] = tSoOut;
+    xi[15] = xi[16] = 90.0 / 100.0 * (610.78 * exp(17.2694 * tAir / (tAir + 238.3)));
+    xi[17] = xi[18] = xi[19] = xi[20] = tAir;
+    xi[21] = xi[4];
+    xi[22] = 0.0; xi[23] = 9.5283e4; xi[24] = 2.5107e5; xi[25] = 5.5338e4; xi[26] = 3.0978e3; xi[27] = 0.0;
+    for (int i = 0; i < NX; ++i) x[(size_t)i * ld + b] = T(xi[i]);
+    for (int j = 0; j < NU; ++j) u[(size_t)j * ld + b] = T(0);
+    timestep[b] = 0;
+}
+
 #ifndef GL_OBS_ROWS
 #define GL_OBS_ROWS 16
 #endif
@@ -111,9 +161,17 @@
 };
 constexpr int STEP_OBS_MAX_DIM_OCC2 = WAVE * ((2 * NX + GL_N_SLOW) | 1) / OBS_ROWS, STEP_OBS_MAX_DIM_OCC1 = 512;
 struct StepNoObs {};
+struct StepObsResetArgs : StepObsArgs {
+    float* term_obs;
+    int* w_off_rw; float* start_day_rw; int* episode;
+    const int* start_rows; const float* start_days; int n_starts;
+    unsigned long long seed;
+};
 constexpr int GL_SCH_OBS = 8;
-template <bool OBS> struct StepObsSel { using type = StepNoObs; };
-template <> struct StepObsSel<true> { using type = StepObsArgs; };
+constexpr int GL_SCH_RESET = 16;
+template <int EPI> struct StepObsSel { using type = StepNoObs; };
+template <> struct StepObsSel<GL_SCH_OBS> { using type = StepObsArgs; };
+template <> struct StepObsSel<GL_SCH_OBS | GL_SCH_RESET> { using type = StepObsResetArgs; };
 
 #ifndef GL_STEP_WAVES_PER_SIMD
 #define GL_STEP_WAVES_PER_SIMD 1
@@ -130,11 +188,12 @@
 
 template <class T, bool PER_ENV_CROP, bool DEFAULT_P, bool PIPE = false, int SCHX = 0, int OCC = GL_STEP_WAVES_PER_SIMD>
 __global__ __launch_bounds__(WAVE, OCC) void step_kernel(StepArgsT<T> a, ModelConst<T> m_arg, RewardConst<T> rw,
-                                                         typename StepObsSel<(SCHX & GL_SCH_OBS) != 0>::type o)
-{
-    constexpr bool OBS = (SCHX & GL_SCH_OBS) != 0;
+                                                         typename StepObsSel<(SCHX & (GL_SCH_OBS | GL_SCH_RESET))>::type o)
+{
+    constexpr bool OBS = (SCHX & GL_SCH_OBS) != 0, RST = (SCHX & GL_SCH_RESET) != 0;
     constexpr int SCH = SCHX & (GL_SCH_OBS - 1);
     static_assert(!OBS || (sizeof(T) == 4 && !PIPE), "observation epilogue: fp32, default ODE");
+    static_assert(!RST || (OBS && !PER_ENV_CROP), "auto-reset epilogue: behind the observation epilogue, shared crop parameters");
     const ModelConst<T>& m = DEFAULT_P ? device_default<T>() : m_arg;
     constexpr bool WBUF = OCC == 2;
     constexpr int WSTRIDE = (2 * NX + GL_N_SLOW) | 1;
@@ -333,6 +392,54 @@
                     for (int jj = lane; jj < dim; jj += WAVE) out[(size_t)r * dim + jj] = span[(size_t)r * dim + jj];
             }
             __syncthreads();
+        }
+        if constexpr (RST) {
+            const bool fin = live && term;
+            const unsigned long long fin_mask = __builtin_amdgcn_ballot_w64(fin);
+            if (fin_mask != 0) {
+                const size_t row0 = (size_t)b0 * dim;
+                __syncthreads();
+                if (o.term_obs) {
+                    for (unsigned long long mk = fin_mask; mk != 0; mk &= mk - 1) {
+                        const size_t e0 = row0 + (size_t)__builtin_ctzll(mk) * dim;
+                        for (int jj = lane; jj < dim; jj += WAVE) o.term_obs[e0 + jj] = o.obs[e0 + jj];
+                    }
+                }
+                __syncthreads();
+                int base_new = 0;
+                if (fin) {
+                    reset_env<T>(b, a.ld, a.x, a.u, a.timestep, a.weather, a.weather_rows, o.w_off_rw, o.start_rows, o.start_days, o.n_starts,
+                                 o.start_day_rw, o.episode, o.seed, a.nd);
+                    base_new = o.w_off_rw[b];
+                    const int basen = base_new >= a.weather_rows ? a.weather_rows - 1 : (base_new < 0 ? 0 : base_new);
+                    const T* wrown = a.weather + (size_t)basen * a.nd;
+                    float wn[5];
+#pragma unroll
+                    for (int j = 0; j < 5; ++j) wn[j] = wrown[j];
+                    const float sdayn = o.start_day_rw[b];
+                    const float tAirn = a.x[(size_t)2 * a.ld + b];
+                    float* orow = o.obs + row0 + (size_t)lane * dim;
+#pragma unroll
+                    for (int j = 0; j < OBS_NCORE; ++j) {
+                        const int xi = j == 0 ? 0 : j == 1 ? 2 : j == 2 ? 15 : j == 3 ? 9 : j == 4 ? 21 : j == 5 ? 25 : 26;
+                        const float prim = j < 7 ? a.x[(size_t)xi * a.ld + b] : (j < 13 ? 0.0f : wn[j < 18 ? j - 13 : 0]);
+                        const float aux = j < 13 ? tAirn : wn[1];
+                        const int mo = o.moff[obs_core_module(j)];
+                        if (mo >= 0) orow[mo + obs_core_col(j)] = obs_core_feature(j, prim, aux, sdayn, 0, o.doy_inc, o.hod_inc);
+                    }
+                }
+                for (unsigned long long mk = fin_mask; mk != 0; mk &= mk - 1) {
+                    const int r = __builtin_ctzll(mk);
+                    const int base_r1 = __builtin_amdgcn_readlane(base_new, r);
+                    float* orow = o.obs + row0 + (size_t)r * dim + o.moff[5];
+                    for (int q = lane; q < nf; q += WAVE) {
+                        const int i = q / 5, c = q - i * 5;
+                        int row = base_r1 + 1 + i;
+                        row = row >= a.weather_rows ? a.weather_rows - 1 : (row < 0 ? 0 : row);
+                        orow[q] = (float)a.weather[(size_t)row * a.nd + c];
+                    }
+                }
+            }
         }
     }
 }
@@ -840,21 +947,6 @@
     control[(size_t)5 * ld + b] = (T)(c.useBlScr * (1.0 - isDaySmooth) * lamp_on);
 }
 
-__device__ __forceinline__ void philox4x32_10(unsigned c0, unsigned c1, unsigned c2, unsigned c3, unsigned k0,
-                                              unsigned k1, unsigned* out)
-{
-#pragma unroll
-    for (int r = 0; r < 10; ++r) {
-        const unsigned long long p0 = 0xD2511F53ull * c0, p1 = 0xCD9E8D57ull * c2;
-        const unsigned n0 = (unsigned)(p1 >> 32) ^ c1 ^ k0, n1 = (unsigned)p1;
-        const unsigned n2 = (unsigned)(p0 >> 32) ^ c3 ^ k1, n3 = (unsigned)p0;
-        c0 = n0; c1 = n1; c2 = n2; c3 = n3;
-        k0 += 0x9E3779B9u; k1 += 0xBB67AE85u;
-    }
-    out[0] = c0; out[1] = c1; out[2] = c2; out[3] = c3;
-}
-
-
 template <class T>
 __global__ void reset_kernel(int B, int ld, const unsigned char* mask, T* x, T* u, int* timestep, const T* weather,
                              int weather_rows, int* w_off, const int* start_rows, const float* start_days, int n_starts,
@@ -862,34 +954,7 @@
 {
     const int b = blockIdx.x * blockDim.x + threadIdx.x;
     if (b >= B || (mask && !mask[b])) return;
-    if (start_rows && n_starts > 0) {
-        const int ep = episode ? episode[b] : 0;
-        unsigned rnd[4];
-        philox4x32_10((unsigned)b, (unsigned)ep, 0x5eedu, 0u, (unsigned)seed, (unsigned)(seed >> 32), rnd);
-        const int j = (int)(rnd[0] % (unsigned)n_starts);
-        w_off[b] = start_rows[j];
-        if (start_day && start_days) start_day[b] = start_days[j];
-        if (episode) episode[b] = ep + 1;
-    }
-    int r = w_off[b];
-    r = r < 0 ? 0 : (r >= weather_rows ? weather_rows - 1 : r);
-    const double co2Out = (double)weather[(size_t)r * nd + 3], tSoOut = (double)weather[(size_t)r * nd + 6];
-    const double tAir = 16.5;
-    double xi[NX];
-    xi[0] = xi[1] = co2Out;
-    for (int i = 2; i <= 10; ++i) xi[i] = tAir;
-    xi[4] = tAir + 4;
-    xi[11] = 0.25 * (3.0 * tAir + tSoOut);
-    xi[12] = 0.25 * (2.0 * tAir + 2 * tSoOut);
-    xi[13] = 0.25 * (tAir + 3 * tSoOut);
-    xi[14] = tSoOut;
-    xi[15] = xi[16] = 90.0 / 100.0 * (610.78 * exp(17.2694 * tAir / (tAir + 238.3)));
-    xi[17] = xi[18] = xi[19] = xi[20] = tAir;
-    xi[21] = xi[4];
-    xi[22] = 0.0; xi[23] = 9.5283e4; xi[24] = 2.5107e5; xi[25] = 5.5338e4; xi[26] = 3.0978e3; xi[27] = 0.0;
-    for (int i = 0; i < NX; ++i) x[(size_t)i * ld + b] = T(xi[i]);
-    for (int j = 0; j < NU; ++j) u[(size_t)j * ld + b] = T(0);
-    timestep[b] = 0;
+    reset_env<T>(b, ld, x, u, timestep, weather, weather_rows, w_off, start_rows, start_days, n_starts, start_day, episode, seed, nd);
 }
 
 template <class T>
@@ -1666,11 +1731,17 @@
 }
 template <int SCH>
 static void launch_step_sch(const glgym_step_args* a, const StepArgsT<float>& k, const ModelConst<float>& m, const RewardConst<float>& rw,
-                            dim3 grid, dim3 block, hipStream_t st, bool def, bool occ2, const StepObsArgs* o)
+                            dim3 grid, dim3 block, hipStream_t st, bool def, bool occ2, const StepObsArgs* o, const StepObsResetArgs* r)
 {
     using T = float;
     const StepNoObs no;
-    constexpr int SCHO = SCH | GL_SCH_OBS;
+    constexpr int SCHO = SCH | GL_SCH_OBS, SCHR = SCHO | GL_SCH_RESET;
+    if (r) {
+        if (occ2) hipLaunchKernelGGL((step_kernel<T, false, true, false, SCHR, 2>), grid, block, 0, st, k, m, rw, *r);
+        else if (def) hipLaunchKernelGGL((step_kernel<T, false, true, false, SCHR>), grid, block, 0, st, k, m, rw, *r);
+        else hipLaunchKernelGGL((step_kernel<T, false, false, false, SCHR>), grid, block, 0, st, k, m, rw, *r);
+        return;
+    }
     if (o) {
         if (occ2) hipLaunchKernelGGL((step_kernel<T, false, true, false, SCHO, 2>), grid, block, 0, st, k, m, rw, *o);
         else if (a->crop_p && def) hipLaunchKernelGGL((step_kernel<T, true, true, false, SCHO>), grid, block, 0, st, k, m, rw, *o);
@@ -1711,7 +1782,7 @@
 
 template <class T>
 static int launch_step(glgym_handle h, const glgym_step_args* a, const ModelConst<T>& m, const RewardConst<T>& rw,
-                       hipStream_t st, const glgym_obs_args* oa = nullptr, bool* fused = nullptr)
+                       hipStream_t st, const glgym_obs_args* oa = nullptr, int* fused = nullptr, const glgym_reset_args* ra = nullptr)
 {
     StepArgsT<T> k;
     k.B = a->B; k.ld = a->ld;
@@ -1758,8 +1829,9 @@
             return GLGYM_OK;
         }
         const bool occ2 = def && !a->crop_p && (h->occupancy == 2 || (h->occupancy == 0 && (size_t)a->B >= (size_t)2 * WAVE * h->n_simd));
-        StepObsArgs ob;
+        StepObsResetArgs ob;
         const StepObsArgs* o = nullptr;
+        const StepObsResetArgs* r = nullptr;
         if (oa && !oa->mask && oa->B == a->B && oa->ld == a->ld && oa->x == a->x && oa->u == a->u && oa->weather == a->weather &&
             oa->weather_rows == a->weather_rows && oa->w_off == a->w_off && oa->timestep == a->timestep &&
             ((uintptr_t)oa->obs & 15) == 0) {
@@ -1768,12 +1840,20 @@
             obs_layout(h, oa->Np, ob.moff, &ob.dim);
             if (ob.dim > 0 && ob.dim <= (occ2 ? STEP_OBS_MAX_DIM_OCC2 : STEP_OBS_MAX_DIM_OCC1)) o = &ob;
         }
-        if (h->scheme == GLGYM_SCHEME_RK2) launch_step_sch<GLGYM_SCHEME_RK2>(a, k, m, rw, grid, block, st, def, occ2, o);
-        else if (h->scheme == GLGYM_SCHEME_RK3) launch_step_sch<GLGYM_SCHEME_RK3>(a, k, m, rw, grid, block, st, def, occ2, o);
-        else if (h->scheme == GLGYM_SCHEME_LS5) launch_step_sch<GLGYM_SCHEME_LS5>(a, k, m, rw, grid, block, st, def, occ2, o);
-        else launch_step_sch<GLGYM_SCHEME_RK4>(a, k, m, rw, grid, block, st, def, occ2, o);
+        if (o && ra && !a->crop_p && ra->B == a->B && ra->ld == a->ld && ra->x == a->x && ra->u == a->u && ra->timestep == a->timestep &&
+            ra->weather == a->weather && ra->weather_rows == a->weather_rows && ra->w_off == a->w_off && ra->start_rows &&
+            ra->start_days && ra->n_starts > 0 && ra->start_day && ra->start_day == oa->start_day && ra->episode) {
+            ob.term_obs = oa->term_obs; ob.w_off_rw = ra->w_off; ob.start_day_rw = ra->start_day; ob.episode = ra->episode;
+            ob.start_rows = ra->start_rows; ob.start_days = ra->start_days; ob.n_starts = ra->n_starts;
+            ob.seed = (unsigned long long)ra->seed;
+            r = &ob;
+        }
+        if (h->scheme == GLGYM_SCHEME_RK2) launch_step_sch<GLGYM_SCHEME_RK2>(a, k, m, rw, grid, block, st, def, occ2, o, r);
+        else if (h->scheme == GLGYM_SCHEME_RK3) launch_step_sch<GLGYM_SCHEME_RK3>(a, k, m, rw, grid, block, st, def, occ2, o, r);
+        else if (h->scheme == GLGYM_SCHEME_LS5) launch_step_sch<GLGYM_SCHEME_LS5>(a, k, m, rw, grid, block, st, def, occ2, o, r);
+        else launch_step_sch<GLGYM_SCHEME_RK4>(a, k, m, rw, grid, block, st, def, occ2, o, r);
         HIPCHK(hipGetLastError());
-        if (o && fused) *fused = true;
+        if (o && fused) *fused = r ? 2 : 1;
         return GLGYM_OK;
     }
 }
@@ -1799,7 +1879,8 @@
     return GLGYM_OK;
 }
 
-static int step_impl(glgym_handle h, const glgym_step_args* a, void* stream, const glgym_obs_args* oa, bool* fused)
+static int step_impl(glgym_handle h, const glgym_step_args* a, void* stream, const glgym_obs_args* oa, int* fused,
+                     const glgym_reset_args* ra = nullptr)
 {
     if (!h || !a) { g_err = "glgym_step: null handle / arguments"; return GLGYM_EINVAL; }
     if (a->struct_size != (int32_t)sizeof(glgym_step_args)) {
@@ -1823,7 +1904,7 @@
     }
     DeviceGuard dev_guard(h);
     hipStream_t st = (hipStream_t)stream;
-    return h->dtype == GLGYM_F32 ? launch_step<float>(h, a, h->mf, h->rf, st, oa, fused)
+    return h->dtype == GLGYM_F32 ? launch_step<float>(h, a, h->mf, h->rf, st, oa, fused, ra)
                                  : launch_step<double>(h, a, h->md, h->rd, st);
 }
 
@@ -1964,7 +2045,7 @@
         g_err = "glgym_step_obs: bad observation arguments (null pointer, ld < B, or Np outside 0..128)";
         return GLGYM_EINVAL;
     }
-    bool fused = false;
+    int fused = 0;
     const int rc = step_impl(h, a, stream, oa, &fused);
     if (rc != GLGYM_OK || fused) return rc;
     return glgym_obs(h, oa, stream);
@@ -2015,6 +2096,34 @@
                            (unsigned long long)a->seed, h->nd);
     HIPCHK(hipGetLastError());
     return GLGYM_OK;
+}
+
+int glgym_step_obs_reset(glgym_handle h, const glgym_step_args* a, const glgym_obs_args* oa, const glgym_reset_args* ra, void* stream,
+                         int32_t* fused_out)
+{
+    if (fused_out) *fused_out = 0;
+    if (!h || !a || !oa || !ra) { g_err = "glgym_step_obs_reset: null handle / arguments"; return GLGYM_EINVAL; }
+    if (a->struct_size != (int32_t)sizeof(glgym_step_args)) return step_impl(h, a, stream, nullptr, nullptr);
+    if ((oa->mask && oa->mask != a->done) || (ra->mask && ra->mask != a->done)) {
+        g_err = "glgym_step_obs_reset: the masks of the observation and reset blocks must be NULL or the step's `done`";
+        return GLGYM_EINVAL;
+    }
+    if (!obs_args_ok(h, oa) || ra->B < 1 || ra->ld < ra->B || !ra->x || !ra->u || !ra->timestep || !ra->weather || !ra->w_off) {
+        g_err = "glgym_step_obs_reset: bad observation or reset arguments";
+        return GLGYM_EINVAL;
+    }
+    glgym_obs_args full = *oa, masked = *oa;
+    full.mask = nullptr; full.term_obs = oa->term_obs;
+    masked.mask = a->done;
+    glgym_reset_args rst = *ra;
+    rst.mask = a->done;
+    int fused = 0;
+    int rc = step_impl(h, a, stream, &full, &fused, &rst);
+    if (rc == GLGYM_OK && fused == 2 && fused_out) *fused_out = 1;
+    if (rc != GLGYM_OK || fused == 2) return rc;
+    if (!fused && (rc = glgym_obs(h, &full, stream)) != GLGYM_OK) return rc;
+    if ((rc = glgym_reset(h, &rst, stream)) != GLGYM_OK) return rc;
+    return glgym_obs(h, &masked, stream);
 }
 
 int glgym_crop_noise(glgym_handle h, void* crop_p, int B, int ld, double scale, uint64_t seed, uint64_t draw_index,
diff --git a/greenlight-gym2_amd/gl_gym_amd/_lib.py b/greenlight-gym2_amd/gl_gym_amd/_lib.py
--- a/greenlight-gym2_amd/gl_gym_amd/_lib.py
+++ b/greenlight-gym2_amd/gl_gym_amd/_lib.py
@@ -197,6 +197,8 @@
     "glgym_step": (C.c_int, [C.c_void_p, C.POINTER(StepArgs), C.c_void_p]),
     "glgym_obs": (C.c_int, [C.c_void_p, C.POINTER(ObsArgs), C.c_void_p]),
     "glgym_step_obs": (C.c_int, [C.c_void_p, C.POINTER(StepArgs), C.POINTER(ObsArgs), C.c_void_p]),
+    "glgym_step_obs_reset": (C.c_int, [C.c_void_p, C.POINTER(StepArgs), C.POINTER(ObsArgs), C.POINTER(ResetArgs), C.c_void_p,
+                             C.POINTER(C.c_int32)]),
     "glgym_set_obs_modules": (C.c_int, [C.c_void_p, C.POINTER(C.c_int32), C.c_int]),
     "glgym_obs_dim": (C.c_int, [C.c_void_p, C.c_int]),
     "glgym_set_control_limits": (C.c_int, [C.c_void_p, _DP, _DP, C.c_double]),
diff --git a/greenlight-gym2_amd/gl_gym_amd/tomato_env.py b/greenlight-gym2_amd/gl_gym_amd/tomato_env.py
--- a/greenlight-gym2_amd/gl_gym_amd/tomato_env.py
+++ b/greenlight-gym2_amd/gl_gym_amd/tomato_env.py
@@ -181,6 +181,11 @@
         self._stepped = False
         self.n_fused_steps = 0
         self.n_obs_elided = 0
+        self._reset_token = None
+        self._pattern = -1
+        self._auto_reset_applied = None
+        self.n_fused_resets = 0
+        self.n_reset_elided = 0
         self._lib = _EpochLib(L.load(), self)
         self.torch = torch
         self.device = torch.device(device)
@@ -365,6 +370,21 @@
         return Planner(self, n_candidates, horizon, gamma=gamma, crop=crop)
 
     def _launch_reset(self, mask_t):
+        token, self._reset_token = self._reset_token, None
+        self._pattern = 2 if (mask_t is self.done_t and self._pattern == 1) else -1
+        if mask_t is self.done_t and self._reset_elided(token):
+            self._reset_token = token
+            return
+        st = self._auto_reset_applied
+        if mask_t is self.done_t and st is not None and not st["reset_seen"]:
+            st["reset_seen"] = True
+            if st["done"] == (self.done_t.data_ptr(), self.done_t._version):
+                return
+            if st["timestep"] != (self.timestep_t.data_ptr(), self.timestep_t._version):
+                raise RuntimeError("done_t and timestep_t were both written between a step with a fused auto-reset and its "
+                                   "_launch_reset(done_t): the environments that step has already reset cannot be told from the ones "
+                                   "added to the mask; reset those through a mask tensor of their own")
+            mask_t = st["added"] = self.done_t * (self.timestep_t != 0).to(self.done_t.dtype)
         mask_ptr = mask_t.data_ptr() if mask_t is not None else None
         if self.rng == "numpy":
             L.check(self._lib.glgym_rng_reset_draw(self._h, self.B, self.ld, mask_ptr, self.rng_state_t.data_ptr(), self.start_grid[0],
@@ -376,11 +396,13 @@
                             self.start_day_t.data_ptr(), self.episode_t.data_ptr(), self.seed_value)
             L.check(self._lib.glgym_reset(self._h, C.byref(a), self._stream()), "glgym_reset")
             return
-        a = L.ResetArgs(self.B, self.ld, mask_t.data_ptr() if mask_t is not None else None, self.x_T.data_ptr(),
-                        self.u_T.data_ptr(), self.timestep_t.data_ptr(), self.weather_t.data_ptr(), self.weather_rows,
-                        self.w_off_t.data_ptr(), self._start_rows_t.data_ptr(), self._start_days_t.data_ptr(),
-                        len(self.start_rows), self.start_day_t.data_ptr(), self.episode_t.data_ptr(), self.seed_value)
-        L.check(self._lib.glgym_reset(self._h, C.byref(a), self._stream()), "glgym_reset")
+        L.check(self._lib.glgym_reset(self._h, C.byref(self._reset_args(mask_t)), self._stream()), "glgym_reset")
+
+    def _reset_args(self, mask_t):
+        return L.ResetArgs(self.B, self.ld, mask_t.data_ptr() if mask_t is not None else None, self.x_T.data_ptr(),
+                           self.u_T.data_ptr(), self.timestep_t.data_ptr(), self.weather_t.data_ptr(), self.weather_rows,
+                           self.w_off_t.data_ptr(), self._start_rows_t.data_ptr(), self._start_days_t.data_ptr(),
+                           len(self.start_rows), self.start_day_t.data_ptr(), self.episode_t.data_ptr(), self.seed_value)
 
     def _obs_args(self, out_t, mask_t=None, term_t=None):
         return L.ObsArgs(self.B, self.ld, self.x_T.data_ptr(), self.u_T.data_ptr(), self.weather_t.data_ptr(),
@@ -393,24 +415,56 @@
         return tuple((t.data_ptr(), t._version) for t in (self.x_T, self.u_T, self.timestep_t, self.w_off_t, self.start_day_t,
                                                           self.weather_t, self.obs_t))
 
+    def _reset_deps(self):
+        return tuple((t.data_ptr(), t._version) for t in (self.x_T, self.u_T, self.timestep_t, self.w_off_t, self.start_day_t, self.episode_t,
+                                                          self.done_t, self.obs_t, self.term_obs_t, self.weather_t))
+
+    def _reset_elided(self, token):
+        if token is None or token != (self._epoch, self._reset_deps()):
+            return False
+        self.n_reset_elided += 1
+        return True
+
     def _launch_obs(self, out_t, mask_t=None, term_t=None):
         if mask_t is None:
             token, self._obs_token = self._obs_token, None
+            self._pattern = 1 if (out_t is self.obs_t and self._pattern == 0) else -1
             if out_t is self.obs_t:
                 self._obs_followed = self._stepped
                 if token is not None and token == (id(out_t), self._epoch, self._obs_deps()):
                     self.n_obs_elided += 1
                     return
+            self._reset_token = None
+        else:
+            token, self._reset_token = self._reset_token, None
+            whole = out_t is self.obs_t and mask_t is self.done_t and term_t is self.term_obs_t
+            elide = whole and self._pattern == 2 and self._reset_elided(token)
+            self._pattern = 3 if (whole and self._pattern == 2) else -1
+            if elide:
+                return
+            st = self._auto_reset_applied
+            if mask_t is self.done_t and term_t is not None and st is not None and not st["obs_seen"]:
+                if not whole:
+                    raise RuntimeError("the terminal observations of a step with a fused auto-reset are in term_obs_t; a masked "
+                                       "_launch_obs over done_t after it takes obs_t and term_obs_t")
+                st["obs_seen"] = True
+                if st["added"] is not None:
+                    L.check(self._lib.glgym_obs(self._h, C.byref(self._obs_args(out_t, st["added"], term_t)), self._stream()), "glgym_obs")
+                term_t = None
         L.check(self._lib.glgym_obs(self._h, C.byref(self._obs_args(out_t, mask_t, term_t)), self._stream()), "glgym_obs")
 
-    def _launch_step(self, raw_control: bool, want_obs: Optional[bool] = None):
+    def _launch_step(self, raw_control: bool, want_obs: Optional[bool] = None, with_reset: Optional[bool] = None):
         if self._env_at_create is not None and tuple(os.environ.get(k) for k in ("GLGYM_LAYOUT", "GLGYM_OCC", "GLGYM_VERIFY")) != self._env_at_create:
             import warnings
             warnings.warn("GLGYM_LAYOUT / GLGYM_OCC / GLGYM_VERIFY changed after this TomatoVecEnv was created: they are read once, at glgym_create, "
                           "and have no effect on an existing handle -- use set_layout() / set_occupancy() / set_verify()", RuntimeWarning, stacklevel=3)
             self._env_at_create = None
         fuse = self._obs_followed if want_obs is None else bool(want_obs)
+        if with_reset is None:
+            with_reset = want_obs is None and self._pattern == 3
+        with_reset = bool(with_reset) and fuse and self.auto_reset and self.rng != "numpy"
         self._obs_followed, self._obs_token, self._stepped = False, None, True
+        self._reset_token, self._pattern, self._auto_reset_applied = None, 0, None
         if self.rng == "numpy":
             if not getattr(self, "freeze_crop_noise", False):
                 L.check(self._lib.glgym_rng_crop_noise(self._h, self.crop_T.data_ptr() if self.crop_T is not None else None, self.B, self.ld,
@@ -431,6 +485,18 @@
         if not fuse:
             L.check(self._lib.glgym_step(self._h, C.byref(a), self._stream()), "glgym_step")
             return
+        if with_reset:
+            one = C.c_int32(0)
+            L.check(self._lib.glgym_step_obs_reset(self._h, C.byref(a), C.byref(self._obs_args(self.obs_t, None, self.term_obs_t)),
+                                                   C.byref(self._reset_args(self.done_t)), self._stream(), C.byref(one)),
+                    "glgym_step_obs_reset")
+            self.n_fused_steps += 1
+            self.n_fused_resets += one.value
+            self._obs_token = (id(self.obs_t), self._epoch, self._obs_deps())
+            self._reset_token = (self._epoch, self._reset_deps())
+            self._auto_reset_applied = dict(done=(self.done_t.data_ptr(), self.done_t._version), reset_seen=False, obs_seen=False, added=None,
+                                            timestep=(self.timestep_t.data_ptr(), self.timestep_t._version))
+            return
         L.check(self._lib.glgym_step_obs(self._h, C.byref(a), C.byref(self._obs_args(self.obs_t)), self._stream()), "glgym_step_obs")
         self.n_fused_steps += 1
         self._obs_token = (id(self.obs_t), self._epoch, self._obs_deps())
@@ -469,7 +535,8 @@
             self.ctrl_T[:, :self.B].copy_(controls_t.reshape(self.B, L.NU).t())
         else:
             self._launch_rule_based(controller)
-        self._launch_step(raw_control=actions_t is None, want_obs=want_obs)
+        self._launch_step(raw_control=actions_t is None, want_obs=want_obs,
+                          with_reset=want_obs and self.auto_reset and not self._keep_applied_u)
         if want_obs:
             self._launch_obs(self.obs_t)
         if self.auto_reset:
@@ -483,6 +550,7 @@
             self._launch_reset(self.done_t)
             if want_obs:
                 self._launch_obs(self.obs_t, self.done_t, self.term_obs_t)
+        self._pattern = -1
         return self.obs_t, self.reward_t[:self.B], self.done_t, self.info_T[:, :self.B]
 
     def reset(self):
@@ -665,13 +733,14 @@
         def seq():
             self.action_t.copy_(static_a)
             self._action_src = self.action_t
-            self._launch_step(raw_control=False, want_obs=want_obs)
+            self._launch_step(raw_control=False, want_obs=want_obs, with_reset=want_obs and self.auto_reset)
             if want_obs:
                 self._launch_obs(self.obs_t)
             if self.auto_reset:
                 self._launch_reset(self.done_t)
                 if want_obs:
                     self._launch_obs(self.obs_t, self.done_t, self.term_obs_t)
+            self._pattern = -1
 
         state = [self.x_T, self.u_T, self.timestep_t, self.w_off_t, self.start_day_t, self.episode_t, self.obs_t]
         if self.rng == "numpy":
diff --git a/include/glgym.h b/include/glgym.h
--- a/include/glgym.h
+++ b/include/glgym.h
@@ -151,6 +151,8 @@
 int glgym_obs(glgym_handle h, const glgym_obs_args* a, void* stream);
 int glgym_step_obs(glgym_handle h, const glgym_step_args* step, const glgym_obs_args* obs, void* stream);
 int glgym_reset(glgym_handle h, const glgym_reset_args* a, void* stream);
+int glgym_step_obs_reset(glgym_handle h, const glgym_step_args* step, const glgym_obs_args* obs, const glgym_reset_args* reset,
+                         void* stream, int32_t* fused);
 int glgym_crop_noise(glgym_handle h, void* crop_p, int B, int ld, double scale, uint64_t seed, uint64_t draw_index,
                      void* stream);
 
```

New measurement: 103.9 million, median of 6. 1.01x the previous value.
